# rampasek/GraphGPS

Measured on NVIDIA H100. Metric: graphs/sec GPSLayer fwd+bwd, higher is better.
Workload: dtype f32

## Files before the change

### graphgps_b200/csrc/attention.cu

```cuda
#include "kernels.cuh"

namespace gps {

namespace {

constexpr int kWarpsPerBlock = 4;

__device__ __forceinline__ int find_graph(const int* __restrict__ gptr, int B, int node) {
  int lo = 0, hi = B;
  while (hi - lo > 1) {
    int mid = (lo + hi) >> 1;
    if (gptr[mid] <= node) lo = mid; else hi = mid;
  }
  return lo;
}

template <int LPR>
__device__ __forceinline__ float group_sum(float v) {
#pragma unroll
  for (int o = LPR / 2; o > 0; o >>= 1) v += __shfl_xor_sync(0xffffffffu, v, o);
  return v;
}

__device__ __forceinline__ int warp_max_i(int v) {
// ... 19 lines not shown
  q.thr = (uint32_t)fminf(p * 4294967296.f, 4294967295.f);
  q.keep_scale = 1.f / (1.f - p);
}

template <int CH, int LPR>
__device__ __forceinline__ void load_slice(float4* dst, const float* row, int sub, int nch, bool ok) {
#pragma unroll
  for (int c = 0; c < CH; ++c) {
    int ch = sub + c * LPR;
    dst[c] = (ok && ch < nch) ? ld4(row + ch * 4) : f4zero();
  }
}
template <int CH, int LPR>
__device__ __forceinline__ void store_slice(const float4* src, float* row, int sub, int nch) {
#pragma unroll
  for (int c = 0; c < CH; ++c) {
    int ch = sub + c * LPR;
    if (ch < nch) st4(row + ch * 4, src[c]);
  }
}
template <int CH, int LPR>
__device__ __forceinline__ void store_slice_planes(const float4* src, const Planes& p, int64_t r, int64_t col0, int sub, int nch) {
  if (!p.hi) return;
#pragma unroll
  for (int c = 0; c < CH; ++c) {
    int ch = sub + c * LPR;
    if (ch < nch) planes_store4(p, r, col0 + ch * 4, src[c]);
  }
}
template <int CH>
__device__ __forceinline__ float dot_slice(const float4* a, const float4* b) {
  float s = 0.f;
#pragma unroll
  for (int c = 0; c < CH; ++c) s += a[c].x * b[c].x + a[c].y * b[c].y + a[c].z * b[c].z + a[c].w * b[c].w;
  return s;
}

struct AttnArgs {
  const int* gptr; int B; int N; int H; int hd;
  const float* Q; const float* K; const float* V; int64_t ld;
  float* O; const float* Oc; const float* dO; int64_t ldo;
  float* lse; const float* lsec; float* delta; const float* deltac;
  float* dQ; float* dK; float* dV; int64_t ldg;
  float scale; float p_drop; uint64_t seed, offset;
  const unsigned long long* offset_dev;
  Planes Op, dQp, dKp, dVp;
  int smem_rows;
};
__device__ __forceinline__ uint64_t eff_offset(const AttnArgs& a) {
  return a.offset + ((a.p_drop > 0.f && a.offset_dev) ? *a.offset_dev : 0ull);
}

struct StagedRows {
  const float* x; int64_t ldx;
  const float* y; int64_t ldy;
};
template <int RPB>
__device__ __forceinline__ StagedRows stage_rows(const AttnArgs& a, const float* X, int64_t ldX, const float* Y, int64_t ldY,
                                                 int h, float* sm) {
  const int64_t hoff = (int64_t)h * a.hd;
  StagedRows r{X + hoff, ldX, Y + hoff, ldY};
  const int r0 = blockIdx.x * RPB;
  if (a.smem_rows <= 0 || r0 >= a.N) return r;
  const int last = min(r0 + RPB, a.N) - 1;
  const int kmin = a.gptr[find_graph(a.gptr, a.B, r0)];
  const int R = a.gptr[find_graph(a.gptr, a.B, last) + 1] - kmin;
  if (R > a.smem_rows) return r;
  const int pitch = a.hd + 4, nch = a.hd >> 2;
  float* sx = sm;
  float* sy = sm + (int64_t)a.smem_rows * pitch;
  for (int idx = threadIdx.x; idx < R * nch; idx += blockDim.x) {
    const int row = idx / nch, c = idx - row * nch;
    st4(sx + row * pitch + c * 4, ld4(X + (int64_t)(kmin + row) * ldX + hoff + c * 4));
    st4(sy + row * pitch + c * 4, ld4(Y + (int64_t)(kmin + row) * ldY + hoff + c * 4));
  }
  __syncthreads();
  r.x = sx - (int64_t)kmin * pitch; r.ldx = pitch;
  r.y = sy - (int64_t)kmin * pitch; r.ldy = pitch;
  return r;
}

template <int CH, int LPR>
__global__ void __launch_bounds__(kWarpsPerBlock * 32) k_attn_fwd(AttnArgs a) {
  extern __shared__ float attn_sm[];
  constexpr int RPW = 32 / LPR;
  const int warp = threadIdx.x >> 5, lane = threadIdx.x & 31;
  const int sub = lane % LPR, rloc = lane / LPR;
  const int h = blockIdx.y;
  const int i = (blockIdx.x * kWarpsPerBlock + warp) * RPW + rloc;
  const bool row_ok = i < a.N;
  const int nch = a.hd / 4;
  const uint64_t offs = eff_offset(a);
  int gs = 0, n = 0;
  if (row_ok) {
    int g = find_graph(a.gptr, a.B, i);
    gs = a.gptr[g];
    n = a.gptr[g + 1] - gs;
  }
  const int nloop = warp_max_i(n);
  const int64_t hoff = (int64_t)h * a.hd;
  float4 q[CH], o[CH];
  load_slice<CH, LPR>(q, a.Q + (int64_t)(row_ok ? i : 0) * a.ld + hoff, sub, nch, row_ok);
#pragma unroll
  for (int c = 0; c < CH; ++c) {
    q[c] = f4scale(q[c], a.scale);
    o[c] = f4zero();
  }
  float m = -INFINITY, l = 0.f;
  const bool use_drop = a.p_drop > 0.f;
  DropQuad dq;
  drop_quad_init(dq, a.p_drop);
  const StagedRows kv = stage_rows<RPW * kWarpsPerBlock>(a, a.K, a.ld, a.V, a.ld, h, attn_sm);
  float4 kc[CH], vc[CH];
  load_slice<CH, LPR>(kc, kv.x + (int64_t)gs * kv.ldx, sub, nch, n > 0);
  load_slice<CH, LPR>(vc, kv.y + (int64_t)gs * kv.ldy, sub, nch, n > 0);
  for (int jl = 0; jl < nloop; ++jl) {
    if (use_drop && (jl & 3) == 0) drop_quad_refresh(dq, a.p_drop, a.seed, offs, h, i, jl);
    const bool valid = jl < n;
    const bool nvalid = jl + 1 < n;
    const int jn = gs + (nvalid ? jl + 1 : 0);
    float4 kn[CH], vn[CH];
    load_slice<CH, LPR>(kn, kv.x + (int64_t)jn * kv.ldx, sub, nch, nvalid);
    load_slice<CH, LPR>(vn, kv.y + (int64_t)jn * kv.ldy, sub, nch, nvalid);
    float s = group_sum<LPR>(dot_slice<CH>(q, kc));
    s = valid ? s : -INFINITY;
    const float m_new = fmaxf(m, s);
    const float corr = (m_new == -INFINITY) ? 1.f : __expf(m - m_new);
    const float p = valid ? __expf(s - m_new) : 0.f;
    l = l * corr + p;
    const float pd = use_drop ? p * drop_quad_scale(dq, jl) : p;
#pragma unroll
    for (int c = 0; c < CH; ++c) {
      o[c].x = o[c].x * corr + pd * vc[c].x;
      o[c].y = o[c].y * corr + pd * vc[c].y;
      o[c].z = o[c].z * corr + pd * vc[c].z;
      o[c].w = o[c].w * corr + pd * vc[c].w;
      kc[c] = kn[c];
      vc[c] = vn[c];
    }
    m = m_new;
  }
  if (row_ok) {
    const float inv = 1.f / l;
#pragma unroll
    for (int c = 0; c < CH; ++c) o[c] = f4scale(o[c], inv);
    store_slice<CH, LPR>(o, a.O + (int64_t)i * a.ldo + hoff, sub, nch);
    store_slice_planes<CH, LPR>(o, a.Op, i, hoff, sub, nch);
    if (sub == 0) a.lse[(int64_t)i * a.H + h] = m + __logf(l);
  }
}

__global__ void k_attn_delta(AttnArgs a) {
  const int64_t t = ((int64_t)blockIdx.x * blockDim.x + threadIdx.x) >> 3;
  const int sub = threadIdx.x & 7;
  const bool ok = t < (int64_t)a.N * a.H;
  const int64_t i = ok ? t / a.H : 0;
  const int h = ok ? (int)(t - i * a.H) : 0;
  const float4* go = reinterpret_cast<const float4*>(a.dO + i * a.ldo + (int64_t)h * a.hd);
  const float4* oo = reinterpret_cast<const float4*>(a.Oc + i * a.ldo + (int64_t)h * a.hd);
  float acc = 0.f;
  if (ok)
    for (int c = sub; c < a.hd / 4; c += 8) {
      const float4 x = __ldg(go + c), y = __ldg(oo + c);
      acc += x.x * y.x + x.y * y.y + x.z * y.z + x.w * y.w;
    }
  acc += __shfl_xor_sync(0xffffffffu, acc, 4);
  acc += __shfl_xor_sync(0xffffffffu, acc, 2);
  acc += __shfl_xor_sync(0xffffffffu, acc, 1);
  if (ok && sub == 0) a.delta[t] = acc;
}

template <int CH, int LPR>
__device__ __forceinline__ void attn_bwd_q_body(const AttnArgs& a, float* attn_sm) {
  constexpr int RPW = 32 / LPR;
  const int warp = threadIdx.x >> 5, lane = threadIdx.x & 31;
  const int sub = lane % LPR, rloc = lane / LPR;
  const int h = blockIdx.y;
  const int i = (blockIdx.x * kWarpsPerBlock + warp) * RPW + rloc;
  const bool row_ok = i < a.N;
  const int nch = a.hd / 4;
  const uint64_t offs = eff_offset(a);
  int gs = 0, n = 0;
  if (row_ok) {
    int g = find_graph(a.gptr, a.B, i);
    gs = a.gptr[g];
    n = a.gptr[g + 1] - gs;
  }
  const int nloop = warp_max_i(n);
  const int64_t hoff = (int64_t)h * a.hd;
  const int ir = row_ok ? i : 0;
  float4 q[CH], go[CH], gq[CH];
  load_slice<CH, LPR>(q, a.Q + (int64_t)ir * a.ld + hoff, sub, nch, row_ok);
  load_slice<CH, LPR>(go, a.dO + (int64_t)ir * a.ldo + hoff, sub, nch, row_ok);
  {
    const float dl = row_ok ? a.deltac[(int64_t)i * a.H + h] : 0.f;
#pragma unroll
    for (int c = 0; c < CH; ++c) gq[c] = f4zero();
    const float lse = row_ok ? a.lsec[(int64_t)i * a.H + h] : 0.f;
#pragma unroll
    for (int c = 0; c < CH; ++c) q[c] = f4scale(q[c], a.scale);
    const bool use_drop = a.p_drop > 0.f;
    DropQuad dq;
    drop_quad_init(dq, a.p_drop);
    const StagedRows kv = stage_rows<RPW * kWarpsPerBlock>(a, a.K, a.ld, a.V, a.ld, h, attn_sm);
    float4 kk[CH], vv[CH];
    load_slice<CH, LPR>(kk, kv.x + (int64_t)gs * kv.ldx, sub, nch, n > 0);
    load_slice<CH, LPR>(vv, kv.y + (int64_t)gs * kv.ldy, sub, nch, n > 0);
    for (int jl = 0; jl < nloop; ++jl) {
      if (use_drop && (jl & 3) == 0) drop_quad_refresh(dq, a.p_drop, a.seed, offs, h, i, jl);
      const bool valid = jl < n;
      const bool nvalid = jl + 1 < n;
      const int jn = gs + (nvalid ? jl + 1 : 0);
      float4 kn[CH], vn[CH];
      load_slice<CH, LPR>(kn, kv.x + (int64_t)jn * kv.ldx, sub, nch, nvalid);
      load_slice<CH, LPR>(vn, kv.y + (int64_t)jn * kv.ldy, sub, nch, nvalid);
      float s = dot_slice<CH>(q, kk), dp = dot_slice<CH>(go, vv);
#pragma unroll
      for (int ofs = LPR / 2; ofs > 0; ofs >>= 1) {
        s += __shfl_xor_sync(0xffffffffu, s, ofs);
        dp += __shfl_xor_sync(0xffffffffu, dp, ofs);
      }
      const float p = valid ? __expf(s - lse) : 0.f;
      const float ds = p * (dp * (use_drop ? drop_quad_scale(dq, jl) : 1.f) - dl);
#pragma unroll
      for (int c = 0; c < CH; ++c) {
        gq[c].x += ds * kk[c].x;
        gq[c].y += ds * kk[c].y;
        gq[c].z += ds * kk[c].z;
        gq[c].w += ds * kk[c].w;
        kk[c] = kn[c];
        vv[c] = vn[c];
      }
    }
  }
  if (row_ok) {
#pragma unroll
    for (int c = 0; c < CH; ++c) gq[c] = f4scale(gq[c], a.scale);
    store_slice<CH, LPR>(gq, a.dQ + (int64_t)i * a.ldg + hoff, sub, nch);
    store_slice_planes<CH, LPR>(gq, a.dQp, i, hoff, sub, nch);
  }
}

template <int CH, int LPR>
__device__ __forceinline__ void attn_bwd_kv_body(const AttnArgs& a, float* attn_sm) {
  constexpr int RPW = 32 / LPR;
  const int warp = threadIdx.x >> 5, lane = threadIdx.x & 31;
  const int sub = lane % LPR, rloc = lane / LPR;
  const int h = blockIdx.y;
  const int j = (blockIdx.x * kWarpsPerBlock + warp) * RPW + rloc;
  const bool row_ok = j < a.N;
  const int nch = a.hd / 4;
  const uint64_t offs = eff_offset(a);
  int gs = 0, n = 0;
  if (row_ok) {
    int g = find_graph(a.gptr, a.B, j);
    gs = a.gptr[g];
    n = a.gptr[g + 1] - gs;
  }
  const int nloop = warp_max_i(n);
  const int jl = j - gs;
  const int64_t hoff = (int64_t)h * a.hd;
  const int jr = row_ok ? j : 0;
  float4 kk[CH], vv[CH], gk[CH], gv[CH];
  load_slice<CH, LPR>(kk, a.K + (int64_t)jr * a.ld + hoff, sub, nch, row_ok);
  load_slice<CH, LPR>(vv, a.V + (int64_t)jr * a.ld + hoff, sub, nch, row_ok);
#pragma unroll
  for (int c = 0; c < CH; ++c) {
    gk[c] = f4zero();
    gv[c] = f4zero();
  }
  const StagedRows qd = stage_rows<RPW * kWarpsPerBlock>(a, a.Q, a.ld, a.dO, a.ldo, h, attn_sm);
  float4 q[CH], go[CH];
  load_slice<CH, LPR>(q, qd.x + (int64_t)gs * qd.ldx, sub, nch, n > 0);
  load_slice<CH, LPR>(go, qd.y + (int64_t)gs * qd.ldy, sub, nch, n > 0);
  for (int il = 0; il < nloop; ++il) {
    const bool valid = il < n;
    const int i = gs + (valid ? il : 0);
    const bool nvalid = il + 1 < n;
    const int in_ = gs + (nvalid ? il + 1 : 0);
    float4 qn[CH], gon[CH];
    load_slice<CH, LPR>(qn, qd.x + (int64_t)in_ * qd.ldx, sub, nch, nvalid);
    load_slice<CH, LPR>(gon, qd.y + (int64_t)in_ * qd.ldy, sub, nch, nvalid);
    float s = dot_slice<CH>(q, kk), dp = dot_slice<CH>(go, vv);
#pragma unroll
    for (int ofs = LPR / 2; ofs > 0; ofs >>= 1) {
      s += __shfl_xor_sync(0xffffffffu, s, ofs);
      dp += __shfl_xor_sync(0xffffffffu, dp, ofs);
    }
    const float lse = valid ? a.lsec[(int64_t)i * a.H + h] : 0.f;
    const float dl = valid ? a.deltac[(int64_t)i * a.H + h] : 0.f;
    const float p = valid ? __expf(s * a.scale - lse) : 0.f;
    float dsc = 1.f;
    if (a.p_drop > 0.f) {
      DropQuad dq;
      drop_quad_init(dq, a.p_drop);
      drop_quad_refresh(dq, a.p_drop, a.seed, offs, h, i, jl);
      dsc = drop_quad_scale(dq, jl);
    }
    const float pd = p * dsc;
    const float ds = p * (dp * dsc - dl) * a.scale;
#pragma unroll
    for (int c = 0; c < CH; ++c) {
      gk[c].x += ds * q[c].x; gk[c].y += ds * q[c].y; gk[c].z += ds * q[c].z; gk[c].w += ds * q[c].w;
      gv[c].x += pd * go[c].x; gv[c].y += pd * go[c].y; gv[c].z += pd * go[c].z; gv[c].w += pd * go[c].w;
      q[c] = qn[c];
      go[c] = gon[c];
    }
  }
  if (row_ok) {
    store_slice<CH, LPR>(gk, a.dK + (int64_t)j * a.ldg + hoff, sub, nch);
    store_slice<CH, LPR>(gv, a.dV + (int64_t)j * a.ldg + hoff, sub, nch);
    store_slice_planes<CH, LPR>(gk, a.dKp, j, hoff, sub, nch);
    store_slice_planes<CH, LPR>(gv, a.dVp, j, hoff, sub, nch);
  }
}

template <int CH, int LPR>
__global__ void __launch_bounds__(kWarpsPerBlock * 32) k_attn_bwd(AttnArgs a) {
  extern __shared__ float attn_sm[];
  if (blockIdx.z == 0) attn_bwd_kv_body<CH, LPR>(a, attn_sm);
  else attn_bwd_q_body<CH, LPR>(a, attn_sm);
}

enum { KFWD = 0, KBWD = 1 };

constexpr int kStageBytes = 72 * 1024;

template <int CH, int LPR>
static void launch_one(int which, const AttnArgs& a0, cudaStream_t stream) {
  constexpr int RPW = 32 / LPR;
  AttnArgs a = a0;
  static const bool stage_on = [] {
    const char* e = getenv("GPS_B200_ATTN_STAGE");
    return e && e[0] == '1';
  }();
  const int pitch = a.hd + 4;
  a.smem_rows = (stage_on && a.B > 0 && a.N < 64LL * a.B) ? kStageBytes / (2 * pitch * 4) : 0;
  const size_t smem = a.smem_rows > 0 ? (size_t)2 * a.smem_rows * pitch * 4 : 0;
  static bool attr_done[2] = {false, false};
  if (smem > 0 && !attr_done[which]) {
    if (which == KFWD) cudaFuncSetAttribute(k_attn_fwd<CH, LPR>, cudaFuncAttributeMaxDynamicSharedMemorySize, kStageBytes);
    else cudaFuncSetAttribute(k_attn_bwd<CH, LPR>, cudaFuncAttributeMaxDynamicSharedMemorySize, kStageBytes);
    attr_done[which] = true;
  }
  dim3 grid((unsigned)ceil_div(a.N, (int64_t)RPW * kWarpsPerBlock), (unsigned)a.H, which == KFWD ? 1 : 2);
  dim3 block(kWarpsPerBlock * 32);
  if (which == KFWD) k_attn_fwd<CH, LPR><<<grid, block, smem, stream>>>(a);
  else k_attn_bwd<CH, LPR><<<grid, block, smem, stream>>>(a);
}

static int dispatch(int which, const AttnArgs& a, cudaStream_t stream) {
  GPS_REQUIRE(a.hd > 0 && a.hd % 4 == 0, GPS_ERR_UNSUPPORTED, "attention: head dim %d must be a multiple of 4", a.hd);
  GPS_REQUIRE(a.ld % 4 == 0 && a.ldo % 4 == 0 && (which == KFWD || a.ldg % 4 == 0), GPS_ERR_UNSUPPORTED,
              "attention: leading dimensions must be multiples of 4");
  const int nch = a.hd / 4;
  GPS_REQUIRE(nch <= 48, GPS_ERR_UNSUPPORTED, "attention: head dim %d > 192 not supported", a.hd);
  if (a.N == 0) return GPS_OK;
  int lpr = 1;
  while ((nch + lpr - 1) / lpr > 6) lpr *= 2;
  const int ch = (nch + lpr - 1) / lpr;
#define GPS_ATTN_CASE(CHV, LPRV)                                  \
  if (ch == CHV && lpr == LPRV) {                                 \
    launch_one<CHV, LPRV>(which, a, stream);                      \
    GPS_LAUNCH_CHECK();                                           \
    return GPS_OK;                                                \
  }
  GPS_ATTN_CASE(1, 1) GPS_ATTN_CASE(2, 1) GPS_ATTN_CASE(3, 1) GPS_ATTN_CASE(4, 1) GPS_ATTN_CASE(5, 1)
  GPS_ATTN_CASE(6, 1) GPS_ATTN_CASE(4, 2) GPS_ATTN_CASE(5, 2) GPS_ATTN_CASE(6, 2) GPS_ATTN_CASE(4, 4)
  GPS_ATTN_CASE(5, 4) GPS_ATTN_CASE(6, 4) GPS_ATTN_CASE(4, 8) GPS_ATTN_CASE(5, 8) GPS_ATTN_CASE(6, 8)
#undef GPS_ATTN_CASE
  set_error("attention: no kernel for head dim %d", a.hd);
  return GPS_ERR_UNSUPPORTED;
}

}

int attention_fwd(const GpsGraph& g, int64_t heads, int64_t hd, const float* Q, const float* K, const float* V,
                  int64_t ld, float* O, int64_t ldo, float* lse, float p_drop, uint64_t seed, uint64_t offset,
                  cudaStream_t stream, const unsigned long long* offset_dev, Planes Op) {
  AttnArgs a{};
  a.offset_dev = offset_dev;
  a.Op = Op;
  a.gptr = g.graph_ptr; a.B = (int)g.B; a.N = (int)g.N; a.H = (int)heads; a.hd = (int)hd;
  a.Q = Q; a.K = K; a.V = V; a.ld = ld; a.O = O; a.ldo = ldo; a.lse = lse;
  a.scale = 1.f / sqrtf((float)hd); a.p_drop = p_drop; a.seed = seed; a.offset = offset;
  return dispatch(KFWD, a, stream);
}

int attention_bwd(const GpsGraph& g, int64_t heads, int64_t hd, const float* Q, const float* K, const float* V,
                  int64_t ld, const float* O, const float* dO, int64_t ldo, const float* lse, float* delta,
                  float* dQ, float* dK, float* dV, int64_t ldg, float p_drop, uint64_t seed, uint64_t offset,
                  cudaStream_t stream, const unsigned long long* offset_dev, Planes dQp, Planes dKp, Planes dVp) {
  AttnArgs a{};
  a.offset_dev = offset_dev;
  a.dQp = dQp; a.dKp = dKp; a.dVp = dVp;
  a.gptr = g.graph_ptr; a.B = (int)g.B; a.N = (int)g.N; a.H = (int)heads; a.hd = (int)hd;
  a.Q = Q; a.K = K; a.V = V; a.ld = ld; a.Oc = O; a.dO = dO; a.ldo = ldo; a.lsec = lse;
  a.delta = delta; a.deltac = delta; a.dQ = dQ; a.dK = dK; a.dV = dV; a.ldg = ldg;
  a.scale = 1.f / sqrtf((float)hd); a.p_drop = p_drop; a.seed = seed; a.offset = offset;
  if (a.N == 0) return GPS_OK;
  const int64_t nt = (int64_t)a.N * a.H * 8;
  k_attn_delta<<<(unsigned)ceil_div(nt, (int64_t)256), 256, 0, stream>>>(a);
  GPS_LAUNCH_CHECK();
  return dispatch(KBWD, a, stream);
}

}
```

### graphgps_b200/csrc/attention_tc.cu

```cuda
#include <cuda.h>
#include <cuda_bf16.h>

#include "gemm.cuh"
#include "kernels.cuh"
#include "tc_ptx.cuh"

namespace gps {

namespace {

using namespace tc;

constexpr int kTile = 128;
constexpr int kSoftWarps = 8;
constexpr int kThreadsA = 256;

struct AttnTcArgs {
  const int* gptr; int B; int N; int H; int hd; int hd_pad; int planes;
  float* O; int64_t ldo; Planes Op; float* lse;
  float scale; float p_drop; uint64_t seed, offset;
  const unsigned long long* offset_dev;
  float* dbg;
};

__device__ __forceinline__ int find_graph_tc(const int* __restrict__ gptr, int B, int node) {
  int lo = 0, hi = B;
  while (hi - lo > 1) {
    int mid = (lo + hi) >> 1;
    if (gptr[mid] <= node) lo = mid; else hi = mid;
  }
  return lo;
}

__device__ __forceinline__ uint32_t pack_bf16x2(float a, float b) {
  __nv_bfloat162 h = __floats2bfloat162_rn(a, b);
  return *reinterpret_cast<uint32_t*>(&h);
}

struct RowState {
  int i, gs, ge;
  float m, l;
  int rq_quad;
  Philox4 rq;
};

template <int NKB, bool SPLIT>
__global__ void __launch_bounds__(kThreadsA, 1)
k_attn_tc_fwd(const __grid_constant__ CUtensorMap tmQK, const __grid_constant__ CUtensorMap tmV, const AttnTcArgs a) {
  extern __shared__ __align__(1024) uint8_t smem_raw[];
  uint8_t* smem = reinterpret_cast<uint8_t*>((reinterpret_cast<uintptr_t>(smem_raw) + 1023) & ~(uintptr_t)1023);
  constexpr int planes = SPLIT ? 2 : 1;
  constexpr int q_bytes = NKB * 16384, k_bytes = NKB * 16384, v_bytes = 2 * NKB * 8192;
  uint8_t* sQ = smem;
  uint8_t* sK = sQ + planes * q_bytes;
  uint8_t* sV = sK + planes * k_bytes;
  uint64_t* bars = reinterpret_cast<uint64_t*>(sV + planes * v_bytes);
  int* range = reinterpret_cast<int*>(bars + 8);

  const int tid = threadIdx.x, warp = tid >> 5, lane = tid & 31;
  const int q0 = blockIdx.x * kTile, h = blockIdx.y;
  const uint32_t b_q = smem_u32(&bars[0]), b_kf = smem_u32(&bars[1]), b_vf = smem_u32(&bars[2]),
                 b_ke = smem_u32(&bars[3]), b_ve = smem_u32(&bars[4]);

  if (tid == 0) {
    mbar_init(b_q, 1); mbar_init(b_kf, 1); mbar_init(b_vf, 1); mbar_init(b_ke, kSoftWarps); mbar_init(b_ve, kSoftWarps);
    fence_barrier_init();
    const int last = min(q0 + kTile, a.N) - 1;
    const int g0 = find_graph_tc(a.gptr, a.B, q0), g1 = find_graph_tc(a.gptr, a.B, last);
    range[0] = a.gptr[g0];
    range[1] = a.gptr[g1 + 1];
  }
  __syncthreads();
  const int kmin = range[0], kmax = range[1];
  const int ntiles = max(1, (kmax - kmin + kTile - 1) / kTile);

  auto load_k = [&](int t) {
    if (t > 0) mbar_wait(b_ke, (uint32_t)(t - 1) & 1u);
    mbar_arrive_expect_tx(b_kf, (uint32_t)(planes * k_bytes));
    for (int pl = 0; pl < planes; ++pl)
      for (int kb = 0; kb < NKB; ++kb)
        tma_tile_3d(smem_u32(sK + pl * k_bytes + kb * 16384), &tmQK, (a.H + h) * a.hd_pad + 64 * kb, kmin + t * kTile, pl,
                    b_kf);
  };
  auto load_v = [&](int t) {
    if (t > 0) mbar_wait(b_ve, (uint32_t)(t - 1) & 1u);
    mbar_arrive_expect_tx(b_vf, (uint32_t)(planes * v_bytes));
    for (int pl = 0; pl < planes; ++pl)
      for (int kk = 0; kk < 2; ++kk)
        for (int nb = 0; nb < NKB; ++nb)
          tma_tile_3d(smem_u32(sV + pl * v_bytes + (kk * NKB + nb) * 8192), &tmV, (2 * a.H + h) * a.hd_pad + 64 * nb,
                      kmin + t * kTile + 64 * kk, pl, b_vf);
  };
  if (tid == 0) {
    tma_prefetch_desc(&tmQK);
    tma_prefetch_desc(&tmV);
    mbar_arrive_expect_tx(b_q, (uint32_t)(planes * q_bytes));
    for (int pl = 0; pl < planes; ++pl)
      for (int kb = 0; kb < NKB; ++kb)
        tma_tile_3d(smem_u32(sQ + pl * q_bytes + kb * 16384), &tmQK, h * a.hd_pad + 64 * kb, q0, pl, b_q);
    load_k(0);
    load_v(0);
  }

  const int wg = warp >> 2;
  const int rloc = wg * 64 + (warp & 3) * 16 + (lane >> 2);
  const int cq = 2 * (lane & 3);
  RowState rs[2];
#pragma unroll
  for (int u = 0; u < 2; ++u) {
    RowState& R = rs[u];
    R.i = q0 + rloc + 8 * u;
    R.gs = 0; R.ge = 0;
    if (R.i < a.N) {
      const int g = find_graph_tc(a.gptr, a.B, R.i);
      R.gs = a.gptr[g];
      R.ge = a.gptr[g + 1];
    }
    R.m = -INFINITY; R.l = 0.f; R.rq_quad = -1;
  }
  const uint64_t offs = a.offset + ((a.p_drop > 0.f && a.offset_dev) ? *a.offset_dev : 0ull);
  const bool use_drop = a.p_drop > 0.f;
  const uint32_t drop_thr = (uint32_t)fminf(a.p_drop * 4294967296.f, 4294967295.f);
  const float keep_scale = use_drop ? 1.f / (1.f - a.p_drop) : 1.f;
  const bool dump = a.dbg && blockIdx.x == 0 && blockIdx.y == 0;

  float o[NKB * 32];
#pragma unroll
  for (int e = 0; e < NKB * 32; ++e) o[e] = 0.f;
  const uint32_t aQ = smem_u32(sQ) + (uint32_t)wg * 8192u, aK = smem_u32(sK), aV = smem_u32(sV);
  const int qk_steps = a.hd_pad >> 4;
  if (lane == 0) mbar_wait(b_q, 0u);
  __syncwarp();
  for (int t = 0; t < ntiles; ++t) {
    const int key0 = kmin + t * kTile;
    float sacc[64];
#pragma unroll
    for (int e = 0; e < 64; ++e) sacc[e] = 0.f;
    if (lane == 0) mbar_wait(b_kf, (uint32_t)t & 1u);
    __syncwarp();
    wgmma_fence();
#pragma unroll
    for (int ks = 0; ks < NKB * 4; ++ks) {
      if (ks < qk_steps) {
        const uint32_t off = (ks >> 2) * 16384 + (ks & 3) * 32;
        const uint64_t dq_hi = make_desc(aQ + off, 16, 1024);
        const uint64_t dk_hi = make_desc(aK + off, 16, 1024);
        if (SPLIT) {
          const uint64_t dq_lo = make_desc(aQ + q_bytes + off, 16, 1024);
          const uint64_t dk_lo = make_desc(aK + k_bytes + off, 16, 1024);
// ... 53 lines not shown
                R.rq = philox4x32(a.seed, offs + (uint64_t)(GPS_SITE_ATTN_P + h), ((uint64_t)R.i << 20) | (uint64_t)R.rq_quad);
              }
              const int k4 = jl & 3;
              const uint32_t bits = k4 == 0 ? R.rq.v[0] : k4 == 1 ? R.rq.v[1] : k4 == 2 ? R.rq.v[2] : R.rq.v[3];
              pr = bits >= drop_thr ? pr * keep_scale : 0.f;
            }
          }
          v = pr;
          if (dump && t == 0) {
            const int r = rloc + 8 * u, c = 8 * j + cq + e;
            a.dbg[r * 128 + c] = sraw;
            a.dbg[16384 + r * 128 + c] = pr;
          }
        }
    }
    uint32_t ph[32], pl[SPLIT ? 32 : 1];
#pragma unroll
    for (int x = 0; x < 32; ++x) {
      const float p0 = sacc[2 * x], p1 = sacc[2 * x + 1];
      __nv_bfloat162 hb = __floats2bfloat162_rn(p0, p1);
      ph[x] = *reinterpret_cast<uint32_t*>(&hb);
      if (SPLIT) pl[x] = pack_bf16x2(p0 - __low2float(hb), p1 - __high2float(hb));
    }
    if (lane == 0) mbar_wait(b_vf, (uint32_t)t & 1u);
    __syncwarp();
    wgmma_fence();
#pragma unroll
    for (int ks = 0; ks < 8; ++ks) {
      const uint32_t voff = ((ks >> 2) * NKB) * 8192 + (ks & 3) * 2048;
      const uint64_t dv_hi = make_desc(aV + voff, 8192, 1024);
      if (SPLIT) {
        const uint64_t dv_lo = make_desc(aV + v_bytes + voff, 8192, 1024);
        wgmma_rs<NKB * 64, 1>(o, pl + 4 * ks, dv_hi, 1u);
        wgmma_rs<NKB * 64, 1>(o, ph + 4 * ks, dv_lo, 1u);
      }
      wgmma_rs<NKB * 64, 1>(o, ph + 4 * ks, dv_hi, 1u);
    }
    wgmma_commit();
    wgmma_wait<0>();
    reg_fence<NKB * 32>(o);
    __syncwarp();
    if (lane == 0) mbar_arrive(b_ve);
    if (tid == 0 && t + 1 < ntiles) load_v(t + 1);
  }
#pragma unroll
  for (int u = 0; u < 2; ++u) {
    RowState& R = rs[u];
    R.l += __shfl_xor_sync(0xffffffffu, R.l, 1);
    R.l += __shfl_xor_sync(0xffffffffu, R.l, 2);
    const float inv = R.l > 0.f ? 1.f / R.l : 0.f;
    const bool row_ok = R.i < a.N;
#pragma unroll
    for (int j = 0; j < NKB * 8; ++j) {
      const int col = 8 * j + cq;
      const float v0 = o[4 * j + 2 * u], v1 = o[4 * j + 2 * u + 1];
      if (dump) {
        a.dbg[32768 + (rloc + 8 * u) * 128 + col] = v0;
        a.dbg[32768 + (rloc + 8 * u) * 128 + col + 1] = v1;
      }
      if (!row_ok || col >= a.hd) continue;
      const float w0 = v0 * inv, w1 = v1 * inv;
      float* dst = a.O + (int64_t)R.i * a.ldo + (int64_t)h * a.hd + col;
      dst[0] = w0;
      dst[1] = w1;
      if (a.Op.hi) {
        const int64_t off = (int64_t)R.i * a.Op.ld + (int64_t)h * a.hd + col;
        __nv_bfloat162 hb = __floats2bfloat162_rn(w0, w1);
        *reinterpret_cast<__nv_bfloat162*>(a.Op.hi + off) = hb;
        if (a.Op.lo) *reinterpret_cast<uint32_t*>(a.Op.lo + off) = pack_bf16x2(w0 - __low2float(hb), w1 - __high2float(hb));
      }
    }
    if (row_ok && (lane & 3) == 0) a.lse[(int64_t)R.i * a.H + h] = R.m + __logf(R.l);
  }
}

template <int NKB, bool SPLIT>
int launch_attn(const CUtensorMap& tQK, const CUtensorMap& tV, const AttnTcArgs& a, dim3 grid, size_t smem,
                cudaStream_t stream) {
  static bool attr_done = false;
  if (!attr_done) {
    GPS_CUDA(cudaFuncSetAttribute(k_attn_tc_fwd<NKB, SPLIT>, cudaFuncAttributeMaxDynamicSharedMemorySize, 227 * 1024));
    attr_done = true;
  }
  k_attn_tc_fwd<NKB, SPLIT><<<grid, kThreadsA, smem, stream>>>(tQK, tV, a);
  GPS_LAUNCH_CHECK();
  return GPS_OK;
}

float* g_attn_dbg = nullptr;
}

void attention_tc_set_debug(float* buf) { g_attn_dbg = buf; }
bool attention_tc_supported(int64_t hd) { return hd > 0 && hd % 4 == 0 && hd <= 128; }
int64_t attention_tc_hd_pad(int64_t hd) { return round_up(hd, 16); }

int attention_tc_fwd(const GpsGraph& g, int64_t heads, int64_t hd, Planes qkv, float* O, int64_t ldo, Planes Op, float* lse,
                     float p_drop, uint64_t seed, uint64_t offset, const unsigned long long* offset_dev, int precision,
                     cudaStream_t stream) {
  if (g.N == 0) return GPS_OK;
  GPS_REQUIRE(attention_tc_supported(hd) && qkv.hi && (precision != GPS_PREC_FP32 || qkv.lo) && qkv.ld % 8 == 0, GPS_ERR_UNSUPPORTED,
              "attention_tc: head dim %lld / planes not supported", (long long)hd);
  AttnTcArgs a{};
  a.gptr = g.graph_ptr; a.B = (int)g.B; a.N = (int)g.N; a.H = (int)heads; a.hd = (int)hd;
  a.hd_pad = (int)attention_tc_hd_pad(hd);
  a.planes = precision == GPS_PREC_FP32 ? 2 : 1;
  a.O = O; a.ldo = ldo; a.Op = Op; a.lse = lse;
  a.scale = 1.f / sqrtf((float)hd); a.p_drop = p_drop; a.seed = seed; a.offset = offset; a.offset_dev = offset_dev;
  a.dbg = g_attn_dbg;
  const int64_t cols = 3 * heads * a.hd_pad;
  CUtensorMap tQK, tV;
  GPS_TRY(make_tensor_map(qkv.hi, qkv.lo, a.planes, g.N, cols, qkv.ld, 128, &tQK));
  GPS_TRY(make_tensor_map(qkv.hi, qkv.lo, a.planes, g.N, cols, qkv.ld, 64, &tV));
  const int nkb = (a.hd_pad + 63) >> 6;
  const size_t smem = (size_t)a.planes * nkb * (16384 + 16384 + 16384) + 1024 + 256;
  dim3 grid((unsigned)ceil_div(g.N, kTile), (unsigned)heads);
  if (nkb == 1) return a.planes == 2 ? launch_attn<1, true>(tQK, tV, a, grid, smem, stream)
                                     : launch_attn<1, false>(tQK, tV, a, grid, smem, stream);
  return a.planes == 2 ? launch_attn<2, true>(tQK, tV, a, grid, smem, stream)
                       : launch_attn<2, false>(tQK, tV, a, grid, smem, stream);
}

}
```

### graphgps_b200/csrc/common.cuh

```cuda
#pragma once

#include <cuda_bf16.h>
#include <cuda_runtime.h>
#include <stdint.h>
#include <stdio.h>
#include <string>

#include "../../include/gps_b200.h"

namespace gps {

void set_error(const char* fmt, ...);
int cuda_fail(cudaError_t e, const char* what, const char* file, int line);
void count_launch();

#define GPS_CUDA(expr)                                                             \
  do {                                                                             \
    cudaError_t _e = (expr);                                                       \
    if (_e != cudaSuccess) return ::gps::cuda_fail(_e, #expr, __FILE__, __LINE__); \
  } while (0)

#define GPS_LAUNCH_CHECK()            \
  do {                                \
    ::gps::count_launch();            \
    GPS_CUDA(cudaGetLastError());     \
  } while (0)

#define GPS_REQUIRE(cond, code, ...)   \
  do {                                 \
    if (!(cond)) {                     \
      ::gps::set_error(__VA_ARGS__);   \
      return (code);                   \
    }                                  \
  } while (0)

#define GPS_TRY(expr)            \
  do {                           \
    int _rc = (expr);            \
    if (_rc != GPS_OK) return _rc; \
  } while (0)

constexpr int kNumSMs = 132;
constexpr float kBnEps = 1e-5f;
constexpr float kBnMomentum = 0.1f;

static inline int64_t round_up(int64_t v, int64_t a) { return (v + a - 1) / a * a; }
static inline int64_t ceil_div(int64_t a, int64_t b) { return (a + b - 1) / b; }

struct Arena {
  char* base;
  int64_t cap;
  int64_t used = 0;
  bool overflow = false;
  Arena(void* b, int64_t c) : base(reinterpret_cast<char*>(b)), cap(c) {}
  template <typename T>
  T* alloc(int64_t n) {
    int64_t bytes = round_up(n * (int64_t)sizeof(T), 256);
    int64_t off = used;
    used += bytes;
    if (base == nullptr) return nullptr;
    if (used > cap) {
      overflow = true;
      return nullptr;
    }
    return reinterpret_cast<T*>(base + off);
  }
};

struct Planes {
  __nv_bfloat16* hi = nullptr;
  __nv_bfloat16* lo = nullptr;
  int64_t ld = 0;
  Planes cols(int64_t c0) const { Planes q = *this; if (q.hi) q.hi += c0; if (q.lo) q.lo += c0; return q; }
  Planes rows(int64_t r0) const { Planes q = *this; if (q.hi) q.hi += r0 * ld; if (q.lo) q.lo += r0 * ld; return q; }
};

#ifdef __CUDACC__

__device__ __forceinline__ void planes_store4(const Planes& p, int64_t r, int64_t c, float4 v) {
  __nv_bfloat162 h0 = __floats2bfloat162_rn(v.x, v.y), h1 = __floats2bfloat162_rn(v.z, v.w);
  uint2 hw = make_uint2(*reinterpret_cast<uint32_t*>(&h0), *reinterpret_cast<uint32_t*>(&h1));
  *reinterpret_cast<uint2*>(p.hi + r * p.ld + c) = hw;
  if (p.lo) {
    __nv_bfloat162 l0 = __floats2bfloat162_rn(v.x - __low2float(h0), v.y - __high2float(h0));
    __nv_bfloat162 l1 = __floats2bfloat162_rn(v.z - __low2float(h1), v.w - __high2float(h1));
    *reinterpret_cast<uint2*>(p.lo + r * p.ld + c) = make_uint2(*reinterpret_cast<uint32_t*>(&l0), *reinterpret_cast<uint32_t*>(&l1));
  }
}

__device__ __forceinline__ float4 ld4(const float* p) { return *reinterpret_cast<const float4*>(p); }
__device__ __forceinline__ void st4(float* p, float4 v) { *reinterpret_cast<float4*>(p) = v; }
__device__ __forceinline__ float4 f4zero() { return make_float4(0.f, 0.f, 0.f, 0.f); }
__device__ __forceinline__ float4 f4add(float4 a, float4 b) {
  return make_float4(a.x + b.x, a.y + b.y, a.z + b.z, a.w + b.w);
}
__device__ __forceinline__ float4 f4mul(float4 a, float4 b) {
  return make_float4(a.x * b.x, a.y * b.y, a.z * b.z, a.w * b.w);
}
__device__ __forceinline__ float4 f4fma(float4 a, float4 b, float4 c) {
  return make_float4(fmaf(a.x, b.x, c.x), fmaf(a.y, b.y, c.y), fmaf(a.z, b.z, c.z), fmaf(a.w, b.w, c.w));
}
__device__ __forceinline__ float4 f4scale(float4 a, float s) {
  return make_float4(a.x * s, a.y * s, a.z * s, a.w * s);
}

__device__ __forceinline__ float sigmoidf_(float v) { return 1.f / (1.f + __expf(-v)); }

template <int ACT>
__device__ __forceinline__ float act_fwd(float v) {
  if (ACT == GPS_ACT_RELU) return v > 0.f ? v : 0.f;
  return 0.5f * v * (1.f + erff(v * 0.70710678118654752f));
}
template <int ACT>
__device__ __forceinline__ float act_bwd(float v) {
  if (ACT == GPS_ACT_RELU) return v > 0.f ? 1.f : 0.f;
  float cdf = 0.5f * (1.f + erff(v * 0.70710678118654752f));
  float pdf = 0.3989422804014327f * __expf(-0.5f * v * v);
  return cdf + v * pdf;
}
__device__ __forceinline__ float act_fwd_rt(int act, float v) {
  return act == GPS_ACT_RELU ? act_fwd<GPS_ACT_RELU>(v) : act_fwd<GPS_ACT_GELU>(v);
}
__device__ __forceinline__ float act_bwd_rt(int act, float v) {
  return act == GPS_ACT_RELU ? act_bwd<GPS_ACT_RELU>(v) : act_bwd<GPS_ACT_GELU>(v);
}

struct Philox4 {
  uint32_t v[4];
};
__device__ __forceinline__ Philox4 philox4x32(uint64_t seed, uint64_t ctr_hi, uint64_t ctr_lo) {
  const uint32_t M0 = 0xD2511F53u, M1 = 0xCD9E8D57u, W0 = 0x9E3779B9u, W1 = 0xBB67AE85u;
  uint32_t c0 = (uint32_t)ctr_lo, c1 = (uint32_t)(ctr_lo >> 32), c2 = (uint32_t)ctr_hi,
           c3 = (uint32_t)(ctr_hi >> 32);
  uint32_t k0 = (uint32_t)seed, k1 = (uint32_t)(seed >> 32);
#pragma unroll
  for (int r = 0; r < 10; ++r) {
    uint32_t hi0 = __umulhi(M0, c0), lo0 = M0 * c0;
    uint32_t hi1 = __umulhi(M1, c2), lo1 = M1 * c2;
    uint32_t n0 = hi1 ^ c1 ^ k0, n1 = lo1, n2 = hi0 ^ c3 ^ k1, n3 = lo0;
    c0 = n0; c1 = n1; c2 = n2; c3 = n3;
    k0 += W0; k1 += W1;
  }
  Philox4 o;
  o.v[0] = c0; o.v[1] = c1; o.v[2] = c2; o.v[3] = c3;
  return o;
}
__device__ __forceinline__ float4 dropout_scale4(float p, uint64_t seed, uint64_t offset, int site,
                                                 uint64_t idx4) {
  Philox4 r = philox4x32(seed, offset + (uint64_t)site, idx4);
  uint32_t thr = (uint32_t)fminf(p * 4294967296.f, 4294967295.f);
  float s = 1.f / (1.f - p);
  return make_float4(r.v[0] >= thr ? s : 0.f, r.v[1] >= thr ? s : 0.f, r.v[2] >= thr ? s : 0.f,
                     r.v[3] >= thr ? s : 0.f);
}

enum {
  GPS_SITE_GCN_X = 1, GPS_SITE_GCN_E = 2, GPS_SITE_LOCAL = 3, GPS_SITE_ATTN_OUT = 4,
  GPS_SITE_FF1 = 5, GPS_SITE_FF2 = 6, GPS_SITE_PERF_OUT = 7, GPS_SITE_ATTN_P = 16
};

__device__ __forceinline__ float warp_sum(float v) {
// ... 11 lines not shown
```

### graphgps_b200/csrc/elementwise.cu

```cuda
#include <cooperative_groups.h>

#include "kernels.cuh"

namespace gps {

namespace {

struct RowGeom {
  dim3 block, grid;
  size_t smem;
};

static int row_geom(int64_t rows, int64_t d, int nstat, RowGeom* g) {
  GPS_REQUIRE(d > 0 && d % 4 == 0 && d / 4 <= 1024, GPS_ERR_UNSUPPORTED,
              "row-wise stage needs d %% 4 == 0 and d <= 4096 (got %lld)", (long long)d);
  int C4 = (int)(d / 4);
  int RY = C4 >= 256 ? 1 : 256 / C4;
  int64_t cap = kNumSMs * 8;
  if (nstat > 0) {
    RY = C4 >= 1024 ? 1 : 1024 / C4;
    if (RY > 16) RY = 16;
    const int smem_cap = (int)(48 * 1024 / ((size_t)nstat * C4 * sizeof(float4)));
    if (RY > smem_cap) RY = smem_cap < 1 ? 1 : smem_cap;
    cap = kNumSMs / 2;
  }
  int64_t blocks = ceil_div(rows > 0 ? rows : 1, (int64_t)RY * 4);
  if (blocks > cap) blocks = cap;
  g->block = dim3(C4, RY, 1);
  g->grid = dim3((unsigned)blocks, 1, 1);
  g->smem = RY > 1 ? (size_t)nstat * RY * C4 * sizeof(float4) : 0;
  return GPS_OK;
}

template <class Op>
__device__ __forceinline__ void rowwise_body(Op& op, int64_t rows, int vb, int vgrid, float4* sm) {
  const int c4 = threadIdx.x, ry = threadIdx.y, RY = blockDim.y, C4 = blockDim.x;
  constexpr int NS = Op::NS;
  float4 acc[NS > 0 ? NS : 1];
#pragma unroll
  for (int s = 0; s < (NS > 0 ? NS : 1); ++s) acc[s] = f4zero();
  op.prepare(c4);
#pragma unroll 4
  for (int64_t r = (int64_t)vb * RY + ry; r < rows; r += (int64_t)vgrid * RY) op.row(r, c4, acc);
  if (NS > 0) {
    if (RY > 1) {
#pragma unroll
      for (int s = 0; s < NS; ++s) sm[(s * RY + ry) * C4 + c4] = acc[s];
      __syncthreads();
      if (ry == 0) {
#pragma unroll
        for (int s = 0; s < NS; ++s)
          for (int y = 1; y < RY; ++y) acc[s] = f4add(acc[s], sm[(s * RY + y) * C4 + c4]);
      }
    }
    if (ry == 0) {
#pragma unroll
      for (int s = 0; s < NS; ++s) {
        double* p = op.stat_ptr(s);
        if (p) {
          atomic_add_f64(p + c4 * 4 + 0, (double)acc[s].x);
          atomic_add_f64(p + c4 * 4 + 1, (double)acc[s].y);
          atomic_add_f64(p + c4 * 4 + 2, (double)acc[s].z);
          atomic_add_f64(p + c4 * 4 + 3, (double)acc[s].w);
        }
      }
    }
  }
  op.finish(c4, ry);
}

template <class Op>
__global__ void __launch_bounds__(1024) k_rowwise(Op op, int64_t rows) {
  extern __shared__ float4 sm[];
  rowwise_body(op, rows, (int)blockIdx.x, (int)gridDim.x, sm);
}

template <class OpA, class OpB>
__global__ void __launch_bounds__(1024) k_rowwise2(OpA a, int64_t rowsA, int ga, OpB b, int64_t rowsB) {
  extern __shared__ float4 sm[];
  if ((int)blockIdx.x < ga) {
    a.vb = (int)blockIdx.x;
    rowwise_body(a, rowsA, (int)blockIdx.x, ga, sm);
  } else {
    b.vb = (int)blockIdx.x - ga;
    rowwise_body(b, rowsB, (int)blockIdx.x - ga, (int)gridDim.x - ga, sm);
  }
}

struct BnRegs {
  float4 mean, invstd, gamma, beta;
  __device__ void load(const BnView& v, int c4, int vb = -1) {
    gamma = ld4(v.gamma + c4 * 4);
    beta = ld4(v.beta + c4 * 4);
    if (v.mode == 0) {
      mean = ld4(v.mean + c4 * 4);
      invstd = ld4(v.invstd + c4 * 4);
    } else if (v.mode == 2) {
      mean = ld4(v.running_mean + c4 * 4);
      const float4 rv = ld4(v.running_var + c4 * 4);
      invstd = make_float4(rsqrtf(rv.x + kBnEps), rsqrtf(rv.y + kBnEps), rsqrtf(rv.z + kBnEps), rsqrtf(rv.w + kBnEps));
    } else {
      float m[4], is[4], var[4];
#pragma unroll
      for (int j = 0; j < 4; ++j) {
        const double mu = v.sums[c4 * 4 + j] * v.inv_n;
        double vv = v.sums[v.d + c4 * 4 + j] * v.inv_n - mu * mu;
        if (vv < 0.0) vv = 0.0;
        m[j] = (float)mu;
        var[j] = (float)(vv * v.unbias);
        is[j] = (float)(1.0 / sqrt(vv + (double)kBnEps));
      }
      mean = make_float4(m[0], m[1], m[2], m[3]);
      invstd = make_float4(is[0], is[1], is[2], is[3]);
      if ((vb < 0 ? (int)blockIdx.x : vb) == 0 && threadIdx.y == 0) {
        st4(v.save_mean + c4 * 4, mean);
        st4(v.save_invstd + c4 * 4, invstd);
        if (v.running_mean) {
          const float4 rm = ld4(v.running_mean + c4 * 4);
          st4(v.running_mean + c4 * 4, make_float4((1.f - kBnMomentum) * rm.x + kBnMomentum * m[0],
                                                   (1.f - kBnMomentum) * rm.y + kBnMomentum * m[1],
                                                   (1.f - kBnMomentum) * rm.z + kBnMomentum * m[2],
                                                   (1.f - kBnMomentum) * rm.w + kBnMomentum * m[3]));
        }
        if (v.running_var) {
          const float4 rv = ld4(v.running_var + c4 * 4);
          st4(v.running_var + c4 * 4, make_float4((1.f - kBnMomentum) * rv.x + kBnMomentum * var[0],
                                                  (1.f - kBnMomentum) * rv.y + kBnMomentum * var[1],
                                                  (1.f - kBnMomentum) * rv.z + kBnMomentum * var[2],
                                                  (1.f - kBnMomentum) * rv.w + kBnMomentum * var[3]));
        }
        if (c4 == 0 && v.nbt) *v.nbt += 1;
      }
    }
  }
  __device__ float4 zhat(float4 z) const {
    return make_float4((z.x - mean.x) * invstd.x, (z.y - mean.y) * invstd.y, (z.z - mean.z) * invstd.z,
                       (z.w - mean.w) * invstd.w);
  }
  __device__ float4 apply(float4 z) const { return f4fma(zhat(z), gamma, beta); }
};

__device__ __forceinline__ float4 act4(int act, float4 v) {
  if (act < 0) return v;
  return make_float4(act_fwd_rt(act, v.x), act_fwd_rt(act, v.y), act_fwd_rt(act, v.z), act_fwd_rt(act, v.w));
}
__device__ __forceinline__ float4 dact4(int act, float4 v) {
  return make_float4(act_bwd_rt(act, v.x), act_bwd_rt(act, v.y), act_bwd_rt(act, v.z), act_bwd_rt(act, v.w));
}

template <bool STATS>
struct OpBnActRes {
  static constexpr int NS = STATS ? 2 : 0;
  const float* z; int64_t ldz;
  const float* R; float* out; int64_t d;
  BnView bn; int act; DropCfg drop; double* stats; Planes outp;
  BnRegs reg;
  int vb = -1;
  __device__ void prepare(int c4) {
    reg.load(bn, c4, vb);
    if (drop.p > 0.f && drop.offset_dev) drop.offset += *drop.offset_dev;
  }
// ... 64 lines not shown
  static constexpr int NS = 0;
  const float* g; int64_t ldg; const float* z; int64_t ldz; int64_t d;
  BnView bn; int act; DropCfg drop; const double* sums; float inv_n;
  float* out; int64_t ldo; float* grad_gamma; float* grad_beta; int accumulate; Planes outp;
  BnRegs reg;
  float4 m1, m2, gs;
  float4 s1raw, s2raw;
  __device__ void prepare(int c4) {
    reg.load(bn, c4);
    if (drop.p > 0.f && drop.offset_dev) drop.offset += *drop.offset_dev;
    const double* a = sums + c4 * 4;
    const double* b = sums + d + c4 * 4;
    s1raw = make_float4((float)a[0], (float)a[1], (float)a[2], (float)a[3]);
    s2raw = make_float4((float)b[0], (float)b[1], (float)b[2], (float)b[3]);
    m1 = f4scale(s1raw, inv_n);
    m2 = f4scale(s2raw, inv_n);
    if (bn.mode == 2) m1 = m2 = f4zero();
    gs = f4mul(reg.gamma, reg.invstd);
  }
  __device__ void row(int64_t r, int c4, float4*) {
    float4 zh = reg.zhat(ld4(z + r * ldz + c4 * 4));
    float4 gp = bn_bwd_gprime(g, ldg, r, c4, zh, reg, act, drop, d);
    float4 v = make_float4(gs.x * (gp.x - m1.x - zh.x * m2.x), gs.y * (gp.y - m1.y - zh.y * m2.y),
                           gs.z * (gp.z - m1.z - zh.z * m2.z), gs.w * (gp.w - m1.w - zh.w * m2.w));
    st4(out + r * ldo + c4 * 4, v);
    if (outp.hi) planes_store4(outp, r, c4 * 4, v);
  }
  __device__ double* stat_ptr(int) { return nullptr; }
  __device__ void finish(int c4, int ry) {
    if (blockIdx.x == 0 && ry == 0) {
      if (grad_gamma) st4(grad_gamma + c4 * 4, accumulate ? f4add(ld4(grad_gamma + c4 * 4), s2raw) : s2raw);
      if (grad_beta) st4(grad_beta + c4 * 4, accumulate ? f4add(ld4(grad_beta + c4 * 4), s1raw) : s1raw);
    }
  }
};

struct OpBnBwdApplyChain {
  static constexpr int NS = 2;
  OpBnBwdApply a;
  const float* z2; int64_t ldz2; BnView bn2; int act2; DropCfg drop2; double* sums2;
  BnRegs reg2;
  __device__ void prepare(int c4) {
    a.prepare(c4);
    reg2.load(bn2, c4);
    if (drop2.p > 0.f && drop2.offset_dev) drop2.offset += *drop2.offset_dev;
  }
  __device__ void row(int64_t r, int c4, float4* acc) {
    float4 zh = a.reg.zhat(ld4(a.z + r * a.ldz + c4 * 4));
    float4 gp = bn_bwd_gprime(a.g, a.ldg, r, c4, zh, a.reg, a.act, a.drop, a.d);
    float4 v = make_float4(a.gs.x * (gp.x - a.m1.x - zh.x * a.m2.x), a.gs.y * (gp.y - a.m1.y - zh.y * a.m2.y),
                           a.gs.z * (gp.z - a.m1.z - zh.z * a.m2.z), a.gs.w * (gp.w - a.m1.w - zh.w * a.m2.w));
    st4(a.out + r * a.ldo + c4 * 4, v);
    if (a.outp.hi) planes_store4(a.outp, r, c4 * 4, v);
    float4 zh2 = reg2.zhat(ld4(z2 + r * ldz2 + c4 * 4));
    float4 g2 = v;
    if (drop2.p > 0.f)
      g2 = f4mul(g2, dropout_scale4(drop2.p, drop2.seed, drop2.offset, drop2.site, (uint64_t)r * (a.d >> 2) + c4));
    if (act2 >= 0) g2 = f4mul(g2, dact4(act2, f4fma(zh2, reg2.gamma, reg2.beta)));
    acc[0] = f4add(acc[0], g2);
    acc[1] = f4fma(g2, zh2, acc[1]);
  }
  __device__ double* stat_ptr(int s) { return sums2 + (int64_t)s * a.d; }
  __device__ void finish(int c4, int ry) { a.finish(c4, ry); }
};

struct OpAdd3 {
  static constexpr int NS = 0;
  const float* a; int64_t lda; const float* b; int64_t ldb; const float* c; int64_t ldc;
  float* out; int64_t ldo;
  __device__ void prepare(int) {}
  __device__ void row(int64_t r, int c4, float4*) {
    float4 v = ld4(a + r * lda + c4 * 4);
    if (b) v = f4add(v, ld4(b + r * ldb + c4 * 4));
    if (c) v = f4add(v, ld4(c + r * ldc + c4 * 4));
    st4(out + r * ldo + c4 * 4, v);
  }
  __device__ double* stat_ptr(int) { return nullptr; }
  __device__ void finish(int, int) {}
};

constexpr int kColsumCtas = 8;
__global__ void __launch_bounds__(1024) k_colsum(const float* __restrict__ a, int64_t lda, int64_t rows, int C4,
                                                 float* __restrict__ out) {
  extern __shared__ float4 sm[];
  const int ry = threadIdx.y, RY = blockDim.y, CB = blockDim.x;
  const int c4 = blockIdx.x * CB + threadIdx.x;
  const bool col_ok = c4 < C4;
  float4 acc = f4zero();
  if (col_ok)
    for (int64_t r = (int64_t)blockIdx.y * RY + ry; r < rows; r += (int64_t)gridDim.y * RY)
      acc = f4add(acc, ld4(a + r * lda + c4 * 4));
  if (RY > 1) {
    sm[ry * CB + threadIdx.x] = acc;
    __syncthreads();
    if (ry == 0)
      for (int y = 1; y < RY; ++y) acc = f4add(acc, sm[y * CB + threadIdx.x]);
  }
  if (ry == 0) sm[threadIdx.x] = acc;
  cooperative_groups::cluster_group cluster = cooperative_groups::this_cluster();
  cluster.sync();
  if (blockIdx.y == 0 && ry == 0 && col_ok) {
    float4 tot = f4zero();
    for (int k = 0; k < (int)gridDim.y; ++k) tot = f4add(tot, cluster.map_shared_rank(sm, k)[threadIdx.x]);
    atomicAdd(out + c4 * 4 + 0, tot.x);
    atomicAdd(out + c4 * 4 + 1, tot.y);
    atomicAdd(out + c4 * 4 + 2, tot.z);
    atomicAdd(out + c4 * 4 + 3, tot.w);
  }
  cluster.sync();
}

template <class Op>
static int launch_rowwise(Op op, int64_t rows, int64_t d, cudaStream_t stream) {
  if (rows == 0) return GPS_OK;
  RowGeom g;
  GPS_TRY(row_geom(rows, d, Op::NS, &g));
  k_rowwise<Op><<<g.grid, g.block, g.smem, stream>>>(op, rows);
  GPS_LAUNCH_CHECK();
  return GPS_OK;
}

}

int bn_act_residual(const float* z, int64_t ldz, const float* R, float* out, int64_t rows, int64_t d, BnView bn,
                    int act, DropCfg drop, double* stats, cudaStream_t stream, Planes outp) {
  if (stats) {
    OpBnActRes<true> op{z, ldz, R, out, d, bn, act, drop, stats, outp};
    return launch_rowwise(op, rows, d, stream);
  }
  OpBnActRes<false> op{z, ldz, R, out, d, bn, act, drop, nullptr, outp};
  return launch_rowwise(op, rows, d, stream);
}

int bn_act_residual2(const float* zx, const float* Rx, float* outx, int64_t N, BnView bnx, DropCfg dropx, double* statsx,
                     const float* ze, const float* Re, float* oute, int64_t E, BnView bne, DropCfg drope, Planes outep,
                     int64_t d, int act, cudaStream_t stream) {
  if (N == 0 || E == 0 || !statsx) {
    GPS_TRY(bn_act_residual(zx, d, Rx, outx, N, d, bnx, act, dropx, statsx, stream));
    return bn_act_residual(ze, d, Re, oute, E, d, bne, act, drope, nullptr, stream, outep);
  }
  RowGeom g;
  GPS_TRY(row_geom(N, d, 2, &g));
  const int RY = (int)g.block.y;
  int64_t gb = ceil_div(E, (int64_t)RY * 4);
  if (gb > kNumSMs * 2) gb = kNumSMs * 2;
  OpBnActRes<true> opx{zx, d, Rx, outx, d, bnx, act, dropx, statsx, Planes()};
  OpBnActRes<false> ope{ze, d, Re, oute, d, bne, act, drope, nullptr, outep};
  k_rowwise2<<<dim3((unsigned)(g.grid.x + gb)), g.block, g.smem, stream>>>(opx, N, (int)g.grid.x, ope, E);
  GPS_LAUNCH_CHECK();
  return GPS_OK;
}

int bn_bwd_apply_chain(const float* g, int64_t ldg, const float* z, int64_t ldz, int64_t rows, int64_t d, BnView bn,
                       const double* sums, float* out, int64_t ldo, float* grad_gamma, float* grad_beta, bool accumulate,
                       Planes outp, const float* z2, int64_t ldz2, BnView bn2, int act2, DropCfg drop2, double* sums2,
                       cudaStream_t stream) {
  GPS_REQUIRE(rows > 0, GPS_ERR_ARG, "bn_bwd_apply_chain: no rows");
  OpBnBwdApply a{g, ldg, z, ldz, d, bn, -1, DropCfg(), sums, 1.f / (float)rows, out, ldo, grad_gamma, grad_beta,
                 accumulate ? 1 : 0, outp};
  OpBnBwdApplyChain op{a, z2, ldz2, bn2, act2, drop2, sums2};
  return launch_rowwise(op, rows, d, stream);
}

int bn_combine(const float* a, BnView bna, const float* b, BnView bnb, float* out, int64_t rows, int64_t d,
               cudaStream_t stream, Planes outp) {
  OpCombine op{a, b, out, d, bna, bnb, outp};
  return launch_rowwise(op, rows, d, stream);
}

int bn_bwd_reduce(const float* g, int64_t ldg, const float* z, int64_t ldz, int64_t rows, int64_t d, BnView bn,
                  int act, DropCfg drop, double* sums, cudaStream_t stream) {
  OpBnBwdReduce op{g, ldg, z, ldz, d, bn, act, drop, sums};
  return launch_rowwise(op, rows, d, stream);
}

int bn_bwd_apply(const float* g, int64_t ldg, const float* z, int64_t ldz, int64_t rows, int64_t d, BnView bn,
                 int act, DropCfg drop, const double* sums, float* out, int64_t ldo, float* grad_gamma,
                 float* grad_beta, cudaStream_t stream, bool accumulate, Planes outp) {
  OpBnBwdApply op{g, ldg, z, ldz, d, bn, act, drop, sums, 1.f / (float)(rows > 0 ? rows : 1),
                  out, ldo, grad_gamma, grad_beta, accumulate ? 1 : 0, outp};
  if (rows == 0) {
    if (grad_gamma && !accumulate) GPS_CUDA(cudaMemsetAsync(grad_gamma, 0, d * sizeof(float), stream));
    if (grad_beta && !accumulate) GPS_CUDA(cudaMemsetAsync(grad_beta, 0, d * sizeof(float), stream));
    return GPS_OK;
  }
  return launch_rowwise(op, rows, d, stream);
}

int add3(const float* a, int64_t lda, const float* b, int64_t ldb, const float* c, int64_t ldc, float* out,
         int64_t ldo, int64_t rows, int64_t d, cudaStream_t stream) {
  OpAdd3 op{a, lda, b, ldb, c, ldc, out, ldo};
  return launch_rowwise(op, rows, d, stream);
}

int colsum(const float* a, int64_t lda, int64_t rows, int64_t d, float* out, cudaStream_t stream) {
  if (rows == 0) return GPS_OK;
  GPS_REQUIRE(d > 0 && d % 4 == 0, GPS_ERR_UNSUPPORTED, "colsum needs d %% 4 == 0 (got %lld)", (long long)d);
  const int C4 = (int)(d / 4);
  const int CB = C4 < 128 ? C4 : 128;
  const int RY = 1024 / CB < 16 ? 1024 / CB : 16;
  cudaLaunchConfig_t cfg = {};
  cfg.gridDim = dim3((unsigned)ceil_div(C4, CB), kColsumCtas);
  cfg.blockDim = dim3(CB, RY);
  cfg.dynamicSmemBytes = (size_t)RY * CB * sizeof(float4);
  cfg.stream = stream;
  cudaLaunchAttribute attr[1];
  attr[0].id = cudaLaunchAttributeClusterDimension;
  attr[0].val.clusterDim.x = 1;
  attr[0].val.clusterDim.y = kColsumCtas;
  attr[0].val.clusterDim.z = 1;
  cfg.attrs = attr;
  cfg.numAttrs = 1;
  GPS_CUDA(cudaLaunchKernelEx(&cfg, k_colsum, a, lda, rows, C4, out));
  GPS_LAUNCH_CHECK();
  return GPS_OK;
}

int copy2d(const float* src, int64_t lds, float* dst, int64_t ldd, int64_t rows, int64_t d, cudaStream_t stream) {
  if (rows == 0) return GPS_OK;
  GPS_CUDA(cudaMemcpy2DAsync(dst, ldd * sizeof(float), src, lds * sizeof(float), d * sizeof(float), rows,
                             cudaMemcpyDeviceToDevice, stream));
  return GPS_OK;
}

}
```

### graphgps_b200/csrc/eslap.cu

```cuda
#include "kernels.cuh"

namespace gps {

namespace {

constexpr int kWarpsPerBlock = 8;

__device__ __forceinline__ float pe_dist2(const float* __restrict__ pe, int64_t k, int64_t a, int64_t b, int lane) {
  float acc = 0.f;
  for (int64_t c = lane; c < k; c += 32) {
    const float t = pe[a * k + c] - pe[b * k + c];
    acc = fmaf(t, t, acc);
  }
  return warp_sum(acc);
}

template <int ACT>
__global__ void k_eslap_fwd(GpsGraph g, const float* __restrict__ pe, int64_t k, int d, const float* __restrict__ w1,
                            const float* __restrict__ b1, const float* __restrict__ w2, const float* __restrict__ b2,
                            float* __restrict__ r_out, float* __restrict__ rho_out) {
  const int lane = threadIdx.x & 31;
  const int64_t i = (int64_t)blockIdx.x * kWarpsPerBlock + (threadIdx.x >> 5);
  if (i >= g.N) return;
  const float bias2 = b2[0];
  for (int q = g.dst_ptr[i]; q < g.dst_ptr[i + 1]; ++q) {
    const int j = g.dst_src[q];
    const int64_t e = g.dst_eid[q];
    const float r = pe_dist2(pe, k, i, j, lane);
    float z = 0.f;
    for (int m = lane; m < d; m += 32) z = fmaf(w2[m], act_fwd<ACT>(fmaf(w1[m], r, b1[m])), z);
    z = warp_sum(z) + bias2;
    if (lane == 0) {
      r_out[e] = r;
      rho_out[e] = sigmoidf_(z);
    }
  }
}

template <int ACT>
__global__ void k_eslap_bwd_edge(GpsGraph g, int d, const float* __restrict__ g_num, const float* __restrict__ g_den,
                                 const float* __restrict__ Bx, int64_t ldy, const float* __restrict__ ehat,
                                 const float* __restrict__ r_in, const float* __restrict__ rho_in,
                                 const float* __restrict__ w1, const float* __restrict__ b1,
                                 const float* __restrict__ w2, float* __restrict__ gz_out, float* __restrict__ gr_out) {
  const int lane = threadIdx.x & 31;
  const int64_t i = (int64_t)blockIdx.x * kWarpsPerBlock + (threadIdx.x >> 5);
  if (i >= g.N) return;
  for (int q = g.dst_ptr[i]; q < g.dst_ptr[i + 1]; ++q) {
    const int64_t j = g.dst_src[q];
    const int64_t e = g.dst_eid[q];
    float acc = 0.f;
    for (int c = lane * 4; c < d; c += 128) {
      const float4 gn = ld4(g_num + i * d + c), gd = ld4(g_den + i * d + c), bx = ld4(Bx + j * ldy + c);
      const float4 eh = ld4(ehat + e * d + c);
      acc = fmaf(fmaf(gn.x, bx.x, gd.x), sigmoidf_(eh.x), acc);
      acc = fmaf(fmaf(gn.y, bx.y, gd.y), sigmoidf_(eh.y), acc);
      acc = fmaf(fmaf(gn.z, bx.z, gd.z), sigmoidf_(eh.z), acc);
      acc = fmaf(fmaf(gn.w, bx.w, gd.w), sigmoidf_(eh.w), acc);
    }
    const float g_rho = warp_sum(acc);
    const float rho = rho_in[e], r = r_in[e];
    const float gz = g_rho * rho * (1.f - rho);
    float s = 0.f;
    for (int m = lane; m < d; m += 32) s = fmaf(w2[m] * act_bwd<ACT>(fmaf(w1[m], r, b1[m])), w1[m], s);
    s = warp_sum(s);
    if (lane == 0) {
      gz_out[e] = gz;
      gr_out[e] = gz * s;
    }
  }
}

__global__ void k_eslap_bwd_pe(GpsGraph g, const float* __restrict__ pe, int64_t k, const float* __restrict__ gr,
                               float* __restrict__ grad_pe) {
  const int lane = threadIdx.x & 31;
  const int64_t n = (int64_t)blockIdx.x * kWarpsPerBlock + (threadIdx.x >> 5);
  if (n >= g.N) return;
  const int db = g.dst_ptr[n], de = g.dst_ptr[n + 1], sb = g.src_ptr[n], se = g.src_ptr[n + 1];
  for (int64_t c = lane; c < k; c += 32) {
    const float p = pe[n * k + c];
    float acc = 0.f;
    for (int q = db; q < de; ++q) acc = fmaf(2.f * gr[g.dst_eid[q]], p - pe[(int64_t)g.dst_src[q] * k + c], acc);
    for (int q = sb; q < se; ++q) acc = fmaf(2.f * gr[g.src_eid[q]], p - pe[(int64_t)g.src_dst[q] * k + c], acc);
    grad_pe[n * k + c] = acc;
  }
}

template <int ACT>
__global__ void k_eslap_wgrad_part(int64_t E, int64_t chunk, int d, const float* __restrict__ r_in,
                                   const float* __restrict__ gz_in, const float* __restrict__ w1,
                                   const float* __restrict__ b1, const float* __restrict__ w2, float* __restrict__ part) {
  const int64_t e0 = (int64_t)blockIdx.x * chunk;
  const int64_t e1 = e0 + chunk < E ? e0 + chunk : E;
  float* out = part + (int64_t)blockIdx.x * (3 * d + 1);
  for (int m = threadIdx.x; m < d; m += blockDim.x) {
    const float a = w1[m], b = b1[m], w = w2[m];
    float gw2 = 0.f, gw1 = 0.f, gb1 = 0.f;
    for (int64_t e = e0; e < e1; ++e) {
      const float r = r_in[e], gz = gz_in[e];
      const float pre = fmaf(a, r, b);
      gw2 = fmaf(gz, act_fwd<ACT>(pre), gw2);
      const float gpre = gz * w * act_bwd<ACT>(pre);
      gw1 = fmaf(gpre, r, gw1);
      gb1 += gpre;
    }
    out[m] = gw2;
    out[d + m] = gw1;
    out[2 * d + m] = gb1;
  }
  if (threadIdx.x == 0) {
    float gb2 = 0.f;
    for (int64_t e = e0; e < e1; ++e) gb2 += gz_in[e];
    out[3 * d] = gb2;
  }
}

__global__ void k_eslap_wgrad_sum(int64_t nparts, int d, const float* __restrict__ part, float* gw2, float* gw1,
                                  float* gb1, float* gb2, int accumulate) {
  const int col = blockIdx.x * blockDim.x + threadIdx.x;
  if (col > 3 * d) return;
  float s = 0.f;
#pragma unroll 8
  for (int64_t b = 0; b < nparts; ++b) s += part[b * (3 * d + 1) + col];
  float* base = col < d ? gw2 : (col < 2 * d ? gw1 : (col < 3 * d ? gb1 : gb2));
  if (!base) return;
  float* dst = base + (col < 3 * d ? col % d : 0);
  *dst = accumulate ? *dst + s : s;
}

}

int64_t eslap_wgrad_chunk(int64_t E) {
  const int64_t c = ceil_div(E, (int64_t)kNumSMs);
  return c > 32 ? c : 32;
}

int eslap_fwd(const GpsGraph& g, const float* pe, int64_t k, int64_t d, int act, const float* w1, const float* b1,
              const float* w2, const float* b2, float* r, float* rho, cudaStream_t stream) {
  if (g.N == 0 || g.E == 0) return GPS_OK;
  const unsigned blocks = (unsigned)ceil_div(g.N, (int64_t)kWarpsPerBlock);
  if (act == GPS_ACT_RELU)
    k_eslap_fwd<GPS_ACT_RELU><<<blocks, 32 * kWarpsPerBlock, 0, stream>>>(g, pe, k, (int)d, w1, b1, w2, b2, r, rho);
  else
    k_eslap_fwd<GPS_ACT_GELU><<<blocks, 32 * kWarpsPerBlock, 0, stream>>>(g, pe, k, (int)d, w1, b1, w2, b2, r, rho);
  GPS_LAUNCH_CHECK();
  return GPS_OK;
}

int eslap_bwd(const GpsGraph& g, const float* pe, int64_t k, int64_t d, int act, const float* g_num, const float* g_den,
              const float* Bx, int64_t ldy, const float* ehat, const float* r, const float* rho, const float* w1,
              const float* b1, const float* w2, float* gz, float* gr, float* part, float* grad_pe, float* gw1,
              float* gb1, float* gw2, float* gb2, bool accumulate, cudaStream_t stream) {
  const unsigned node_blocks = (unsigned)ceil_div(g.N, (int64_t)kWarpsPerBlock);
  const int64_t chunk = eslap_wgrad_chunk(g.E), nparts = ceil_div(g.E, chunk);
  if (g.E > 0) {
    if (act == GPS_ACT_RELU)
      k_eslap_bwd_edge<GPS_ACT_RELU><<<node_blocks, 32 * kWarpsPerBlock, 0, stream>>>(
          g, (int)d, g_num, g_den, Bx, ldy, ehat, r, rho, w1, b1, w2, gz, gr);
    else
      k_eslap_bwd_edge<GPS_ACT_GELU><<<node_blocks, 32 * kWarpsPerBlock, 0, stream>>>(
          g, (int)d, g_num, g_den, Bx, ldy, ehat, r, rho, w1, b1, w2, gz, gr);
    GPS_LAUNCH_CHECK();
    if (act == GPS_ACT_RELU)
      k_eslap_wgrad_part<GPS_ACT_RELU><<<(unsigned)nparts, 256, 0, stream>>>(g.E, chunk, (int)d, r, gz, w1, b1, w2, part);
    else
      k_eslap_wgrad_part<GPS_ACT_GELU><<<(unsigned)nparts, 256, 0, stream>>>(g.E, chunk, (int)d, r, gz, w1, b1, w2, part);
    GPS_LAUNCH_CHECK();
  }
  if (gw1 || gb1 || gw2 || gb2) {
    k_eslap_wgrad_sum<<<(unsigned)ceil_div(3 * d + 1, (int64_t)128), 128, 0, stream>>>(g.E > 0 ? nparts : 0, (int)d, part,
                                                                                     gw2, gw1, gb1, gb2, accumulate ? 1 : 0);
    GPS_LAUNCH_CHECK();
  }
  if (grad_pe && g.N > 0) {
    k_eslap_bwd_pe<<<node_blocks, 32 * kWarpsPerBlock, 0, stream>>>(g, pe, k, gr, grad_pe);
    GPS_LAUNCH_CHECK();
  }
  return GPS_OK;
}

}
```

### graphgps_b200/csrc/gemm_tma.cu

```cuda
#include <cooperative_groups.h>
#include <cuda.h>
#include <cuda_bf16.h>

#include <mutex>
#include <unordered_map>

#include "gemm.cuh"
#include "tc_ptx.cuh"

namespace gps {

namespace {

using namespace tc;
namespace cgrp = cooperative_groups;

constexpr int BM = 128;
constexpr int BK = 64;
constexpr int kEpiWarps = 8;
constexpr int kTmaWarp = 8;
constexpr int kThreads = 288;
constexpr int kATile = BM * BK * 2;
constexpr int kBlock = 64 * BK * 2;
constexpr int kMaxSplits = 8;

struct TmaArgs {
  GemmParams p;
  int BN, nb_blocks, stages, kb_per_split, planes;
  int debug;
  unsigned long long* trace;
};

__device__ __forceinline__ unsigned long long gtimer() {
  unsigned long long t;
  asm volatile("mov.u64 %0, %globaltimer;" : "=l"(t));
  return t;
}
#define GPS_TRACE(slot)                                                                         \
  do {                                                                                          \
    if (a.trace && cta_lin < 256) a.trace[cta_lin * 16 + (slot)] = gtimer();                    \
  } while (0)

template <bool A_MN, bool B_MN, int BN_T, bool SPLIT>
__global__ void __launch_bounds__(kThreads, BN_T == 64 ? 2 : 1)
k_gemm_tma(const __grid_constant__ CUtensorMap tmA, const __grid_constant__ CUtensorMap tmB, const TmaArgs a) {
  extern __shared__ __align__(1024) uint8_t smem_raw[];
  const GemmParams& p = a.p;
  uint8_t* smem = reinterpret_cast<uint8_t*>((reinterpret_cast<uintptr_t>(smem_raw) + 1023) & ~(uintptr_t)1023);
  const int planes = a.planes;
  const int b_tile = B_MN ? a.nb_blocks * kBlock : BN_T * 128;
  const int stage_bytes = planes * (kATile + b_tile);
  const int S = a.stages;
  uint64_t* bars = reinterpret_cast<uint64_t*>(smem + (size_t)S * stage_bytes);
  float* red = reinterpret_cast<float*>(bars + 2 * S + 2);
  float* ctot = red + 16 * 16 * 8;
  const int nsplit = (int)gridDim.z;

  const int tid = threadIdx.x, warp = tid >> 5, lane = tid & 31;
  const int m0 = blockIdx.y * BM, n0 = blockIdx.x * a.BN;
  const int nkb_total = (p.K + BK - 1) / BK;
  const int kb_begin = blockIdx.z * a.kb_per_split;
  const int kb_end = min(nkb_total, kb_begin + a.kb_per_split);
  const int nkb = kb_end - kb_begin;
  const bool do_colsum = A_MN && p.colsum_a != nullptr && blockIdx.x == 0;
  const int cta_lin = (blockIdx.z * gridDim.y + blockIdx.y) * gridDim.x + blockIdx.x;

  if (tid == 0) {
    GPS_TRACE(0);
    if (a.trace && cta_lin < 256) {
      unsigned smid;
      asm volatile("mov.u32 %0, %smid;" : "=r"(smid));
      a.trace[cta_lin * 16 + 8] = smid;
    }
    for (int s = 0; s < S; ++s) {
      mbar_init(smem_u32(&bars[s]), 1);
      mbar_init(smem_u32(&bars[S + s]), kEpiWarps);
    }
    fence_barrier_init();
  }
  if (warp == kTmaWarp && lane == 0) {
    tma_prefetch_desc(&tmA);
    tma_prefetch_desc(&tmB);
  }
  __syncthreads();
  if (tid == 0) GPS_TRACE(1);

  if (warp == kTmaWarp) {
    if (lane == 0 && nkb > 0) {
      int a_blocks = 2, b_blocks = a.nb_blocks;
      if (A_MN) a_blocks = min(2, (p.M - m0 + 63) / 64);
      if (B_MN) b_blocks = min(a.nb_blocks, (p.N - n0 + 63) / 64);
      const uint32_t tx = (uint32_t)planes * ((A_MN ? a_blocks * kBlock : kATile) +
                                              (B_MN ? b_blocks * kBlock : a.BN * 128));
      for (int i = 0; i < nkb; ++i) {
        const int s = i % S;
        if (i >= S) mbar_wait(smem_u32(&bars[S + s]), (uint32_t)((i / S) - 1) & 1u);
        const uint32_t full = smem_u32(&bars[s]);
        mbar_arrive_expect_tx(full, tx);
        const int k0 = (kb_begin + i) * BK;
        const uint32_t sa = smem_u32(smem + (size_t)s * stage_bytes);
        const uint32_t sb = sa + planes * kATile;
        for (int pl = 0; pl < planes; ++pl) {
          if (!A_MN) {
            tma_tile_3d(sa + pl * kATile, &tmA, k0, m0, pl, full);
          } else {
            for (int b = 0; b < a_blocks; ++b) tma_tile_3d(sa + pl * kATile + b * kBlock, &tmA, m0 + 64 * b, k0, pl, full);
          }
          if (!B_MN) {
            tma_tile_3d(sb + pl * b_tile, &tmB, k0, n0, pl, full);
          } else {
            for (int b = 0; b < b_blocks; ++b) tma_tile_3d(sb + pl * b_tile + b * kBlock, &tmB, n0 + 64 * b, k0, pl, full);
          }
        }
        if (i == 0) GPS_TRACE(2);
      }
      GPS_TRACE(9);
    }
    __syncwarp();
    if (nsplit > 1) {
      cgrp::this_cluster().sync();
      cgrp::this_cluster().sync();
    }
  } else {
    const int wg = warp >> 2;
    float acc[BN_T / 2];
#pragma unroll
    for (int e = 0; e < BN_T / 2; ++e) acc[e] = 0.f;
    float csum[8];
#pragma unroll
    for (int e = 0; e < 8; ++e) csum[e] = 0.f;
    const int cm = tid & 15, kq = tid >> 4;
    constexpr uint32_t a_lbo = A_MN ? kBlock : 16, b_lbo = B_MN ? kBlock : 16;
    constexpr uint32_t a_kstep = A_MN ? 2048 : 32, b_kstep = B_MN ? 2048 : 32;
    for (int i = 0; i < nkb; ++i) {
      const int s = i % S;
      if (lane == 0) mbar_wait(smem_u32(&bars[s]), (uint32_t)(i / S) & 1u);
      __syncwarp();
      if (i == 0 && tid == 0) GPS_TRACE(3);
      if (i == nkb - 1 && tid == 0) GPS_TRACE(10);
      const uint8_t* st = smem + (size_t)s * stage_bytes;
      const uint32_t sa_hi = smem_u32(st) + (uint32_t)wg * 8192u;
      const uint32_t sb_hi = smem_u32(st) + planes * kATile;
      const uint32_t sa_lo = sa_hi + kATile;
      const uint32_t sb_lo = sb_hi + b_tile;
      wgmma_fence();
#pragma unroll
      for (int kk = 0; kk < BK / 16; ++kk) {
        const uint64_t da_hi = make_desc(sa_hi + kk * a_kstep, a_lbo, 1024);
        const uint64_t db_hi = make_desc(sb_hi + kk * b_kstep, b_lbo, 1024);
        if (SPLIT) {
          const uint64_t da_lo = make_desc(sa_lo + kk * a_kstep, a_lbo, 1024);
          const uint64_t db_lo = make_desc(sb_lo + kk * b_kstep, b_lbo, 1024);
          wgmma_ss<BN_T, A_MN, B_MN>(acc, da_lo, db_hi, 1u);
          wgmma_ss<BN_T, A_MN, B_MN>(acc, da_hi, db_lo, 1u);
        }
        wgmma_ss<BN_T, A_MN, B_MN>(acc, da_hi, db_hi, 1u);
      }
      wgmma_commit();
      if (do_colsum) {
        const uint32_t blk_off = (uint32_t)(cm >> 3) * kBlock;
        const int cc = cm & 7;
        for (int pl = 0; pl < planes; ++pl) {
#pragma unroll
          for (int rr = 0; rr < 4; ++rr) {
            const int r = kq * 4 + rr;
            const uint4 q = *reinterpret_cast<const uint4*>(st + pl * kATile + blk_off + (r >> 3) * 1024 + (r & 7) * 128 +
                                                            ((cc ^ (r & 7)) << 4));
            const uint32_t w[4] = {q.x, q.y, q.z, q.w};
// ... 248 lines not shown
EncodeTiledFn encode_fn() {
  static EncodeTiledFn fn = [] {
    void* f = nullptr;
    cudaDriverEntryPointQueryResult q;
    if (cudaGetDriverEntryPoint("cuTensorMapEncodeTiled", &f, cudaEnableDefault, &q) != cudaSuccess ||
        q != cudaDriverEntryPointSuccess)
      f = nullptr;
    return reinterpret_cast<EncodeTiledFn>(f);
  }();
  return fn;
}

struct MapKey {
  const void* base; int64_t cols, rows, ld, plane_stride; int planes, box_rows;
  bool operator==(const MapKey& o) const {
    return base == o.base && cols == o.cols && rows == o.rows && ld == o.ld && plane_stride == o.plane_stride &&
           planes == o.planes && box_rows == o.box_rows;
  }
};
struct MapKeyHash {
  size_t operator()(const MapKey& k) const {
    size_t h = reinterpret_cast<size_t>(k.base);
    auto mix = [&](int64_t v) { h ^= (size_t)v + 0x9e3779b97f4a7c15ull + (h << 6) + (h >> 2); };
    mix(k.cols); mix(k.rows); mix(k.ld); mix(k.plane_stride); mix(k.planes); mix(k.box_rows);
    return h;
  }
};

int tensor_map(const __nv_bfloat16* hi, const __nv_bfloat16* lo, int planes, int64_t rows, int64_t cols, int64_t ld,
               int box_rows, CUtensorMap* out) {
  static std::mutex mu;
  static std::unordered_map<MapKey, CUtensorMap, MapKeyHash> cache;
  const int64_t plane_stride = planes == 2 ? (int64_t)(lo - hi) : rows * ld;
  GPS_REQUIRE(planes == 1 || plane_stride > 0, GPS_ERR_ARG, "gemm_tma: the lo plane must follow the hi plane in memory");
  MapKey key{hi, cols, rows, ld, plane_stride, planes, box_rows};
  {
    std::lock_guard<std::mutex> lk(mu);
    auto it = cache.find(key);
    if (it != cache.end()) {
      *out = it->second;
      return GPS_OK;
    }
  }
  EncodeTiledFn enc = encode_fn();
  GPS_REQUIRE(enc, GPS_ERR_UNSUPPORTED, "cuTensorMapEncodeTiled is not available from this driver");
  cuuint64_t dims[3] = {(cuuint64_t)cols, (cuuint64_t)rows, (cuuint64_t)planes};
  cuuint64_t strides[2] = {(cuuint64_t)ld * 2, (cuuint64_t)(plane_stride > 0 ? plane_stride : 8) * 2};
  cuuint32_t box[3] = {64, (cuuint32_t)box_rows, 1};
  cuuint32_t estr[3] = {1, 1, 1};
  CUtensorMap m;
  CUresult r = enc(&m, CU_TENSOR_MAP_DATA_TYPE_BFLOAT16, 3, const_cast<__nv_bfloat16*>(hi), dims, strides, box, estr,
                   CU_TENSOR_MAP_INTERLEAVE_NONE, CU_TENSOR_MAP_SWIZZLE_128B, CU_TENSOR_MAP_L2_PROMOTION_L2_256B,
                   CU_TENSOR_MAP_FLOAT_OOB_FILL_NONE);
  GPS_REQUIRE(r == CUDA_SUCCESS, GPS_ERR_CUDA, "cuTensorMapEncodeTiled failed (%d): rows %lld cols %lld ld %lld box %d",
              (int)r, (long long)rows, (long long)cols, (long long)ld, box_rows);
  {
    std::lock_guard<std::mutex> lk(mu);
    if (cache.size() > 4096) cache.clear();
    cache[key] = m;
  }
  *out = m;
  return GPS_OK;
}

}

int make_tensor_map(const __nv_bfloat16* hi, const __nv_bfloat16* lo, int planes, int64_t rows, int64_t cols, int64_t ld,
                    int box_rows, CUtensorMap* out) {
  return tensor_map(hi, lo, planes, rows, cols, ld, box_rows, out);
}

namespace {

inline bool aligned16(const void* q) { return (reinterpret_cast<uintptr_t>(q) & 15) == 0; }

template <bool A_MN, bool B_MN, int BN_T, bool SPLIT>
int launch1(const CUtensorMap& tA, const CUtensorMap& tB, const TmaArgs& a, dim3 grid, size_t smem, cudaStream_t stream) {
  static bool attr_done = false;
  if (!attr_done) {
    GPS_CUDA(cudaFuncSetAttribute(k_gemm_tma<A_MN, B_MN, BN_T, SPLIT>, cudaFuncAttributeMaxDynamicSharedMemorySize,
                                  227 * 1024));
    attr_done = true;
  }
  if (grid.z == 1) {
    k_gemm_tma<A_MN, B_MN, BN_T, SPLIT><<<grid, kThreads, smem, stream>>>(tA, tB, a);
  } else {
    cudaLaunchConfig_t cfg = {};
    cfg.gridDim = grid;
    cfg.blockDim = dim3(kThreads);
    cfg.dynamicSmemBytes = smem;
    cfg.stream = stream;
    cudaLaunchAttribute attr[1];
    attr[0].id = cudaLaunchAttributeClusterDimension;
    attr[0].val.clusterDim.x = 1;
    attr[0].val.clusterDim.y = 1;
    attr[0].val.clusterDim.z = grid.z;
    cfg.attrs = attr;
    cfg.numAttrs = 1;
    GPS_CUDA(cudaLaunchKernelEx(&cfg, k_gemm_tma<A_MN, B_MN, BN_T, SPLIT>, tA, tB, a));
  }
  GPS_LAUNCH_CHECK();
  return GPS_OK;
}
template <bool A_MN, bool B_MN, int BN_T>
int launch(const CUtensorMap& tA, const CUtensorMap& tB, const TmaArgs& a, dim3 grid, size_t smem, cudaStream_t stream) {
  return a.planes == 2 ? launch1<A_MN, B_MN, BN_T, true>(tA, tB, a, grid, smem, stream)
                       : launch1<A_MN, B_MN, BN_T, false>(tA, tB, a, grid, smem, stream);
}

int g_tma_force_bn = 0;
unsigned long long* g_tma_trace = nullptr;
int g_tma_debug = 0;

}

void gemm_tma_set_force_bn(int bn) { g_tma_force_bn = bn & 0xFFFF; g_tma_debug = bn >> 16; }
void gemm_tma_set_trace(unsigned long long* buf) { g_tma_trace = buf; }

int gemm_tma(const GemmParams& p, cudaStream_t stream) {
  if (p.M <= 0 || p.N <= 0) return GPS_OK;
  if (p.K <= 0 || !p.Ap.hi || !p.Bp.hi) return GPS_ERR_UNSUPPORTED;
  const bool split = p.precision == GPS_PREC_FP32;
  const int planes = split ? 2 : 1;
  if (split && (!p.Ap.lo || !p.Bp.lo)) return GPS_ERR_UNSUPPORTED;
  if (!aligned16(p.Ap.hi) || !aligned16(p.Bp.hi) || p.Ap.ld % 8 || p.Bp.ld % 8 || p.N % 4) return GPS_ERR_UNSUPPORTED;
  if (split && (!aligned16(p.Ap.lo) || !aligned16(p.Bp.lo))) return GPS_ERR_UNSUPPORTED;
  if ((p.C && (!aligned16(p.C) || p.ldc % 4)) || (!p.C && !p.Cp.hi)) return GPS_ERR_UNSUPPORTED;
  if (p.Cp.hi && (p.Cp.ld % 4 || (reinterpret_cast<uintptr_t>(p.Cp.hi) & 7) || (p.Cp.lo && (reinterpret_cast<uintptr_t>(p.Cp.lo) & 7))))
    return GPS_ERR_UNSUPPORTED;
  if ((p.bias && !aligned16(p.bias)) || (p.R1 && (!aligned16(p.R1) || p.ldr1 % 4)) ||
      (p.R2 && (!aligned16(p.R2) || p.ldr2 % 4)) || (p.mask_src && (!aligned16(p.mask_src) || p.ldmask % 4)) ||
      (p.C_pre && (!aligned16(p.C_pre) || p.ldpre % 4)))
    return GPS_ERR_UNSUPPORTED;
  if (p.splitk > 1 && (p.bias || p.act >= 0 || p.mask_src || p.stats || p.C_pre || p.p_drop != 0.f || p.p_drop2 != 0.f ||
                       p.Cp.hi || !p.C)) {
    set_error("gemm: split-K supports the plain fp32 product (+ residuals) only");
    return GPS_ERR_ARG;
  }
  if (p.colsum_a && !p.ta) {
    set_error("gemm: colsum_a needs ta == 1");
    return GPS_ERR_ARG;
  }
  if ((p.bnred[0].sums || p.bnred[1].sums) &&
      (p.splitk > 1 || p.C_pre || (p.mask_src && !p.mask_is_post) || p.p_drop != 0.f || p.p_drop2 != 0.f ||
       (p.act >= 0 && p.act != GPS_ACT_RELU))) {
    set_error("gemm: fused BatchNorm-backward reductions need the plain epilogue (no split-K / dropout / GELU)");
    return GPS_ERR_ARG;
  }
  const int mt = (int)ceil_div(p.M, BM);
  const int nkb = (int)ceil_div(p.K, BK);
  const int splits_hint = p.splitk > 1 ? min(kMaxSplits, min(p.splitk, nkb)) : 1;
  const auto width_ok = [&](int bn) {
    return bn == 64 || bn == 128 || (bn == 152 && !p.tb) || (bn == 256 && !p.ta);
  };
  int bestBN = 0;
  long bestCost = 0;
  for (const int bn : {64, 128, 152, 256}) {
    if (!width_ok(bn)) continue;
    const long tiles = (long)mt * ceil_div(p.N, bn) * splits_hint;
    const long cost = bn != 64 ? ceil_div(tiles, (long)kNumSMs) * bn : tiles <= kNumSMs ? 64 : ceil_div(tiles, 2L * kNumSMs) * 160;
    if (!bestBN || cost <= bestCost) { bestCost = cost; bestBN = bn; }
  }
  if (g_tma_force_bn) {
    if (!width_ok(g_tma_force_bn)) return GPS_ERR_UNSUPPORTED;
    bestBN = g_tma_force_bn;
  }
  TmaArgs a;
  a.p = p;
  a.BN = bestBN;
  a.nb_blocks = a.BN / 64;
  a.planes = planes;
  const bool narrow = a.nb_blocks == 1;
  const int stage_bytes = planes * (kATile + (p.tb ? a.nb_blocks * kBlock : a.BN * 128));
  const int fixed = 1024  + 1024  + 16 * 16 * 8 * 4 + 128 * 4;
  int stages = ((narrow ? 112 : 226) * 1024 - fixed) / stage_bytes;
  if (stages > 8) stages = 8;
  if (stages < 2) return GPS_ERR_UNSUPPORTED;
  GPS_REQUIRE((size_t)stages * stage_bytes >= (size_t)BM * (a.BN + 4) * 4, GPS_ERR_ARG,
              "gemm_tma: BN %d: the staging tile does not fit the operand stages", a.BN);
  a.stages = stages;
  int splitk = p.splitk > 1 ? p.splitk : 1;
  if (splitk > kMaxSplits) splitk = kMaxSplits;
  if (splitk > nkb) splitk = nkb;
  a.kb_per_split = (int)ceil_div(nkb, splitk);
  splitk = (int)ceil_div(nkb, a.kb_per_split);
  a.p.splitk = p.splitk > 1 ? 2 : 1;
  a.trace = g_tma_trace;
  a.debug = g_tma_debug;
  const bool amn = p.ta != 0, bmn = p.tb != 0;
  CUtensorMap tA, tB;
  GPS_TRY(tensor_map(p.Ap.hi, p.Ap.lo, planes, amn ? p.K : p.M, amn ? p.M : p.K, p.Ap.ld, amn ? 64 : BM, &tA));
  GPS_TRY(tensor_map(p.Bp.hi, p.Bp.lo, planes, bmn ? p.K : p.N, bmn ? p.N : p.K, p.Bp.ld, bmn ? 64 : a.BN, &tB));
  const size_t smem = (size_t)stages * stage_bytes + fixed;
  dim3 grid((unsigned)ceil_div(p.N, a.BN), (unsigned)mt, (unsigned)splitk);
#define GPS_TMA_CASE(AM, BMN)                                                                              \
  if (amn == AM && bmn == BMN) {                                                                           \
    if (a.BN == 64) return launch<AM, BMN, 64>(tA, tB, a, grid, smem, stream);                            \
    if (a.BN == 128) return launch<AM, BMN, 128>(tA, tB, a, grid, smem, stream);                          \
  }
  GPS_TMA_CASE(false, false)
  GPS_TMA_CASE(false, true)
  GPS_TMA_CASE(true, false)
  GPS_TMA_CASE(true, true)
#undef GPS_TMA_CASE
  if (a.BN == 152 && !bmn)
    return amn ? launch<true, false, 152>(tA, tB, a, grid, smem, stream) : launch<false, false, 152>(tA, tB, a, grid, smem, stream);
  if (a.BN == 256 && !amn)
    return bmn ? launch<false, true, 256>(tA, tB, a, grid, smem, stream) : launch<false, false, 256>(tA, tB, a, grid, smem, stream);
  return GPS_ERR_UNSUPPORTED;
}

namespace {
struct ToPlanesDesc {
  ToPlanesItem it[16];
  int start[17];
  int n;
};
__global__ void k_to_planes(ToPlanesDesc d) {
  int item = 0;
  while (item + 1 < d.n && (int)blockIdx.x >= d.start[item + 1]) ++item;
  const ToPlanesItem& it = d.it[item];
  const int cpr = (it.cols + 7) >> 3;
  const int64_t total = (int64_t)it.rows * cpr;
  const int64_t idx = ((int64_t)blockIdx.x - d.start[item]) * blockDim.x + threadIdx.x;
  if (idx >= total) return;
  const int64_t r = idx / cpr;
  const int c = (int)(idx - r * cpr) * 8;
  const float* src = it.src + r * it.ld + c;
  float v[8];
  if (c + 8 <= it.cols) {
    const float4 x = ld4(src), y = ld4(src + 4);
    v[0] = x.x; v[1] = x.y; v[2] = x.z; v[3] = x.w; v[4] = y.x; v[5] = y.y; v[6] = y.z; v[7] = y.w;
  } else {
#pragma unroll
    for (int i = 0; i < 8; ++i) v[i] = c + i < it.cols ? src[i] : 0.f;
  }
  uint4 hi, lo;
  tc::split8(v, hi, lo);
  *reinterpret_cast<uint4*>(it.dst.hi + r * it.dst.ld + c) = hi;
  if (it.dst.lo) *reinterpret_cast<uint4*>(it.dst.lo + r * it.dst.ld + c) = lo;
}
}

int to_planes(const ToPlanesItem* items, int n, cudaStream_t stream) {
  if (n <= 0) return GPS_OK;
  GPS_REQUIRE(n <= 16, GPS_ERR_ARG, "to_planes: at most 16 matrices per call");
  ToPlanesDesc d;
  d.n = 0;
  int total = 0;
  for (int i = 0; i < n; ++i) {
    const ToPlanesItem& it = items[i];
    if (it.rows <= 0 || it.cols <= 0) continue;
    GPS_REQUIRE(it.src && it.dst.hi && it.ld % 4 == 0 && it.dst.ld % 8 == 0 && it.dst.ld >= round_up(it.cols, 8) &&
                    (reinterpret_cast<uintptr_t>(it.src) & 15) == 0 && (reinterpret_cast<uintptr_t>(it.dst.hi) & 15) == 0 &&
                    (!it.dst.lo || (reinterpret_cast<uintptr_t>(it.dst.lo) & 15) == 0),
                GPS_ERR_ARG, "to_planes: operands must be 16-byte aligned, ld %% 4 == 0, plane ld %% 8 == 0");
    d.it[d.n] = it;
    d.start[d.n] = total;
    total += (int)ceil_div((int64_t)it.rows * ((it.cols + 7) >> 3), 256);
    ++d.n;
  }
  d.start[d.n] = total;
  if (total == 0) return GPS_OK;
  k_to_planes<<<(unsigned)total, 256, 0, stream>>>(d);
  GPS_LAUNCH_CHECK();
  return GPS_OK;
}

}
```

### graphgps_b200/csrc/layer.cu

```cuda
#include <stdarg.h>
#include <string.h>

#include <algorithm>
#include <atomic>

#include "gemm.cuh"
#include "kernels.cuh"

namespace gps {

int perf_supported(int64_t dim_head, int64_t features);
int64_t perf_mp();
int perf_prep(const float* P, int64_t m, float* Pn, const GpsGraph& g, int64_t H, int* nmax, float* gmax, int* argk,
              cudaStream_t st);
int perf_features_fwd(float* fq, float* fk, const float* Q, const float* K, const GpsGraph& g, int64_t H, int64_t m,
                      float* gmax, int* argq, int* argk, cudaStream_t st);
int perf_linattn_fwd(const GpsGraph& g, int64_t H, int64_t m, const int* nmax, const float* qf, const float* kf,
                     const float* V, const float* gmax, float* O, cudaStream_t st);
int perf_linattn_bwd(const GpsGraph& g, int64_t H, int64_t m, const int* nmax, const float* qf, const float* kf,
                     const float* V, const float* gmax, const float* gO, float* g_qf, float* g_kf, float* gV,
                     float* ggmax, cudaStream_t st);
int perf_features_bwd(float* g_fq, float* g_fk, const float* fq, const float* fk, const float* Q, const float* K,
                      float* gQ, float* gK, const GpsGraph& g, int64_t H, int64_t m, const int* argq, const int* argk,
                      float* ggmax, cudaStream_t st);
// ... 30 lines not shown
    int rc = gemm_tma(p, stream);
    if (rc != GPS_ERR_UNSUPPORTED) return rc;
  }
  GPS_REQUIRE(p.A && p.B && p.C, GPS_ERR_UNSUPPORTED, "gemm: plane operands rejected and no fp32 operands to fall back to");
  GPS_REQUIRE(!p.bnred[0].sums && !p.bnred[1].sums, GPS_ERR_UNSUPPORTED,
              "gemm: fused BatchNorm-backward reductions exist in the TMA kernel only");
  GemmParams q = p;
  if (q.Cp.hi) {
    q.Cp = Planes();
  }
  int rc = gemm_tc(q, stream);
  if (rc == GPS_ERR_UNSUPPORTED) {
    g_fallbacks.fetch_add(1, std::memory_order_relaxed);
    GPS_REQUIRE(!strict, GPS_ERR_UNSUPPORTED,
                "GPS_B200_STRICT: dense product M=%d N=%d K=%d (ta=%d tb=%d) would fall back to the CUDA-core kernel",
                p.M, p.N, p.K, p.ta, p.tb);
    rc = gemm_simt(q, stream);
  }
  if (rc == GPS_OK && p.Cp.hi) {
    ToPlanesItem it{p.C, p.ldc, p.M, p.N, p.Cp};
    rc = to_planes(&it, 1, stream);
  }
  return rc;
}

namespace {

struct Side {
  cudaStream_t s = nullptr;
  cudaStream_t s3 = nullptr;
  cudaStream_t s4 = nullptr;
  cudaEvent_t ev[32];
  int next = 0;
  bool ok = false;
  int init() {
    if (ok) return GPS_OK;
    GPS_CUDA(cudaStreamCreateWithFlags(&s, cudaStreamNonBlocking));
    GPS_CUDA(cudaStreamCreateWithFlags(&s3, cudaStreamNonBlocking));
    GPS_CUDA(cudaStreamCreateWithFlags(&s4, cudaStreamNonBlocking));
    for (int i = 0; i < 32; ++i) GPS_CUDA(cudaEventCreateWithFlags(&ev[i], cudaEventDisableTiming));
    ok = true;
    return GPS_OK;
  }
  int order(cudaStream_t from, cudaStream_t to) {
    cudaEvent_t e = ev[next++ & 31];
    GPS_CUDA(cudaEventRecord(e, from));
    GPS_CUDA(cudaStreamWaitEvent(to, e, 0));
    return GPS_OK;
  }
  int fork(cudaStream_t main) { return order(main, s); }
  int join(cudaStream_t main) { return order(s, main); }
};

static int opt_flags() {
  static const int v = [] {
    const char* e = getenv("GPS_B200_OPT");
    return e ? atoi(e) : 0;
  }();
  return v;
}

static Side* side_stream() {
  static const bool enabled = [] {
    const char* e = getenv("GPS_B200_STREAMS");
    return !(e && e[0] == '0');
  }();
  if (!enabled) return nullptr;
  static thread_local Side sides[64];
  int dev = 0;
  if (cudaGetDevice(&dev) != cudaSuccess || dev < 0 || dev >= 64) return nullptr;
  if (sides[dev].init() != GPS_OK) return nullptr;
  return &sides[dev];
}

struct PackSeg {
  const float* w; const float* b; float* gw; float* gb; int rows;
};
struct PackDesc {
  PackSeg seg[5];
  int nseg; int d; int total_rows;
};

__global__ void k_pack(PackDesc pd, float* __restrict__ Wcat, float* __restrict__ bcat) {
  const int r = blockIdx.x;
  int row0 = 0, s = 0;
  while (s < pd.nseg - 1 && r >= row0 + pd.seg[s].rows) row0 += pd.seg[s++].rows;
  const float* src = pd.seg[s].w + (int64_t)(r - row0) * pd.d;
  float* dst = Wcat + (int64_t)r * pd.d;
  for (int c = threadIdx.x * 4; c < pd.d; c += blockDim.x * 4) st4(dst + c, ld4(src + c));
  if (threadIdx.x == 0) bcat[r] = pd.seg[s].b ? pd.seg[s].b[r - row0] : 0.f;
}
__global__ void k_unpack(PackDesc pd, const float* __restrict__ gWcat, const float* __restrict__ gbcat, int accumulate) {
  const int r = blockIdx.x;
  int row0 = 0, s = 0;
  while (s < pd.nseg - 1 && r >= row0 + pd.seg[s].rows) row0 += pd.seg[s++].rows;
  if (pd.seg[s].gw) {
    float* dst = pd.seg[s].gw + (int64_t)(r - row0) * pd.d;
    const float* src = gWcat + (int64_t)r * pd.d;
    for (int c = threadIdx.x * 4; c < pd.d; c += blockDim.x * 4)
      st4(dst + c, accumulate ? f4add(ld4(dst + c), ld4(src + c)) : ld4(src + c));
  }
  if (threadIdx.x == 0 && pd.seg[s].gb) pd.seg[s].gb[r - row0] = (accumulate ? pd.seg[s].gb[r - row0] : 0.f) + gbcat[r];
}

enum { BN_X = 0, BN_E = 1, BN_L = 2, BN_A = 3, BN_2 = 4, BN_COUNT = 5 };

struct Plan {
  int64_t N, E, d, H, hd, Wy, qkv_off;
  bool gated, gine, gcn, attn, perf;
  int64_t inner, mp, m;
  float *pQ, *pK, *pV, *pfq, *pfk, *pPn, *pgmax;
  int *pargq, *pargk, *pnmax;
  float *pden, *g_pden;
  bool perf_pairwise;
  float *g_pfq, *g_pfk, *g_pQ, *g_pK, *g_pV, *g_pgmax, *g_xp;
  float *Wcat, *bcat, *Y1, *ehat, *xt, *xloc, *O, *lse, *hA, *s, *hid, *hid_pre, *t, *bnbuf;
  float *agg, *h1, *h1_pre;
  float* dinv;
  bool eslap;
  float *pe_r, *pe_rho, *g_den, *pe_gz, *pe_gr, *pe_part;
  bool use_planes;
  Planes x_p, e_p, O_p, s_p, hid_p, agg_p, h1_p, Wcat_p, C_p, out_p, ff1_p, ff2_p, g0_p, g1_p, pq_p, pk_p, pv_p;
  Planes gt_p, ghid_p, ghA_p, ge_p, gY1_p, gtmp_p, gtmp2_p, gtmp3_p, gl1_p, gh1_p;
  Planes qkv_p;
  bool attn_tc;
  int64_t saved_bytes;
  int64_t wplanes_bytes;
  double* fstats;
  int64_t fwd_bytes;
  double* bsums;
  float *g_t, *g_hid, *g_s, *g_xloc, *g_hA, *g_O, *gY1, *g_e, *g_num, *delta, *g_tmp, *g_tmp2, *g_tmp3, *g_h1, *g_agg, *gWcat,
      *gbcat, *g_xl;
  int64_t bwd_bytes;
  int64_t fwd_launches, bwd_launches;
};

static bool attn_tc_enabled(int64_t N, int64_t B) {
  static const int mode = [] {
    const char* e = getenv("GPS_B200_ATTN");
    return e && strcmp(e, "simt") == 0 ? 0 : (e && strcmp(e, "tc") == 0 ? 2 : 1);
  }();
  if (mode != 1) return mode == 2;
  return B > 0 && N >= 64 * B;
}

static int make_plan(const GpsLayerArgs* a, Plan* P, bool bind) {
  memset(P, 0, sizeof(*P));
  GPS_REQUIRE(a, GPS_ERR_ARG, "null args");
  P->N = a->graph.N;
  P->E = a->graph.E;
  P->d = a->d;
  P->H = a->heads;
  GPS_REQUIRE(a->d > 0 && a->d % 4 == 0, GPS_ERR_UNSUPPORTED, "dim_h must be a positive multiple of 4 (got %lld)",
              (long long)a->d);
  P->gated = a->local_type == GPS_LOCAL_GATEDGCN;
  P->gine = a->local_type == GPS_LOCAL_GINE;
  P->gcn = a->local_type == GPS_LOCAL_GCN;
  GPS_REQUIRE(a->local_type == GPS_LOCAL_NONE || P->gated || P->gine || P->gcn, GPS_ERR_ARG, "unknown local_type %d",
              a->local_type);
  P->eslap = a->pe != nullptr;
  GPS_REQUIRE(!P->eslap || P->gated, GPS_ERR_ARG, "pe (EquivStableLapPE) is read by the GatedGCN local model only");
  GPS_REQUIRE(!P->eslap || a->pe_dim >= 1, GPS_ERR_ARG, "pe_dim must be >= 1 (got %lld)", (long long)a->pe_dim);
  GPS_REQUIRE(a->global_type == GPS_GLOBAL_NONE || a->global_type == GPS_GLOBAL_TRANSFORMER ||
                  a->global_type == GPS_GLOBAL_PERFORMER,
              GPS_ERR_ARG, "unknown global_type %d", a->global_type);
  P->attn = a->global_type == GPS_GLOBAL_TRANSFORMER;
  P->perf = a->global_type == GPS_GLOBAL_PERFORMER;
  if (P->perf) {
    GPS_TRY(perf_supported(a->perf_dim_head, a->perf_features));
    GPS_REQUIRE(a->heads > 0, GPS_ERR_ARG, "num_heads must be positive");
    P->inner = a->heads * a->perf_dim_head;
    P->mp = perf_mp();
    P->m = a->perf_features;
  }
  GPS_REQUIRE(a->local_type != GPS_LOCAL_NONE || P->attn || P->perf, GPS_ERR_ARG,
// ... 295 lines not shown
  GPS_TRY(check_bn(a->norm2, "norm2"));
  return GPS_OK;
}

static thread_local bool g_grads_prezeroed = false;
static thread_local bool g_grads_accumulate = false;

static int splitk_for(int64_t rows, int64_t out = 304, int64_t in = 304) {
  const int64_t tiles = ceil_div(out, 128) * ceil_div(in, in >= 160 ? 160 : 64);
  int64_t s = ceil_div(300, tiles > 0 ? tiles : 1);
  const int64_t max_s = rows / 256;
  if (s > max_s) s = max_s;
  if (s < 1) s = 1;
  if (s > 64) s = 64;
  return (int)s;
}

static int linear_wgrad(const float* G, int64_t ldg, const float* X, int64_t ldx, int64_t rows, int64_t out,
                        int64_t in, float* dW, float* db, int precision, cudaStream_t st, Planes Gp = Planes(),
                        Planes Xp = Planes()) {
  if (!dW) return GPS_OK;
  if (!g_grads_prezeroed) {
    GPS_CUDA(cudaMemsetAsync(dW, 0, (size_t)(out * in) * sizeof(float), st));
    if (db) GPS_CUDA(cudaMemsetAsync(db, 0, (size_t)out * sizeof(float), st));
  }
  if (rows == 0) return GPS_OK;
  GemmParams p;
  p.M = (int)out; p.N = (int)in; p.K = (int)rows;
  p.A = G; p.lda = (int)ldg; p.ta = 1;
  p.B = X; p.ldb = (int)ldx; p.tb = 1;
  p.C = dW; p.ldc = (int)in;
  p.splitk = splitk_for(rows, out, in);
  if (p.splitk == 1) p.splitk = 2;
  p.colsum_a = db;
  p.precision = precision;
  p.Ap = Gp; p.Bp = Xp;
  if (precision == GPS_PREC_BF16 && Gp.hi && db) {
    p.colsum_a = nullptr;
    GPS_TRY(colsum(G, ldg, rows, out, db, st));
  }
  return gemm(p, st);
}

}

static int layer_forward(const GpsLayerArgs* a, cudaStream_t st) {
  Plan P;
  GPS_TRY(make_plan(a, &P, true));
  GPS_REQUIRE(a->saved && a->workspace, GPS_ERR_ARG, "saved/workspace buffers are required");
  GPS_REQUIRE(a->workspace_bytes >= P.fwd_bytes, GPS_ERR_ARG, "workspace too small (%lld < %lld)",
              (long long)a->workspace_bytes, (long long)P.fwd_bytes);
  GPS_TRY(check_params(a, P));
  GPS_REQUIRE(a->x_out, GPS_ERR_ARG, "x_out is null");
  const int64_t N = P.N, E = P.E, d = P.d;
  const int act = a->act;
  const bool train = a->training != 0;
  const float pd = train ? a->dropout : 0.f;
  const float pa = train ? a->attn_dropout : 0.f;
  auto drop = [&](int site) {
    DropCfg c;
    c.p = pd; c.seed = a->seed; c.offset = a->offset; c.site = site;
    c.offset_dev = (const unsigned long long*)a->offset_dev;
    return c;
  };
  auto stats = [&](int which) -> double* { return train ? P.fstats + (int64_t)which * 2 * d : nullptr; };
  auto out_planes = [&](const GpsPlanes& g) {
    Planes q;
    if (P.use_planes && g.hi && g.ld >= d && g.ld % 8 == 0) {
      q.hi = (__nv_bfloat16*)g.hi;
      q.lo = a->precision == GPS_PREC_FP32 ? (__nv_bfloat16*)g.lo : nullptr;
      q.ld = g.ld;
      if (a->precision == GPS_PREC_FP32 && !q.lo) q = Planes();
    }
    return q;
  };

  if (train) GPS_CUDA(cudaMemsetAsync(P.fstats, 0, (size_t)BN_COUNT * 2 * d * sizeof(double), st));
  Side* sd = side_stream();
  cudaStream_t s2 = sd ? sd->s : st;
  const bool two_branches = (P.gated || P.gine || P.gcn) && (P.attn || P.perf);

  if (P.Wy) {
    PackDesc pdsc0 = pack_desc(a, P);
    k_pack<<<(unsigned)pdsc0.total_rows, 128, 0, st>>>(pdsc0, P.Wcat, P.bcat);
    GPS_LAUNCH_CHECK();
  }
  if (P.use_planes) {
    ToPlanesItem it[16];
    int ni = 0;
    auto add = [&](const float* src, int64_t ld, int64_t rows, int64_t cols, Planes dst) {
      if (src && dst.hi && rows > 0) it[ni++] = ToPlanesItem{src, ld, (int)rows, (int)cols, dst};
    };
    const int64_t kout = P.perf ? P.inner : d;
    if (P.x_p.hi != (__nv_bfloat16*)a->x_planes_in.hi) add(a->x, d, N, d, P.x_p);
    if ((P.gated || P.gine) && P.e_p.hi != (__nv_bfloat16*)a->e_planes_in.hi) add(a->edge_attr, d, E, d, P.e_p);
    const bool wvalid = a->wplanes && a->wplanes_valid;
    if (wvalid) goto weights_done;
    if (P.gated) {
      add(a->gcn_A.weight, d, d, d, P.Wcat_p.rows(0));
      add(a->gcn_B.weight, d, d, d, P.Wcat_p.rows(d));
      add(a->gcn_D.weight, d, d, d, P.Wcat_p.rows(2 * d));
      add(a->gcn_E.weight, d, d, d, P.Wcat_p.rows(3 * d));
      add(a->gcn_C.weight, d, d, d, P.C_p);
    }
    if (P.gcn) add(a->gcn_conv.weight, d, d, d, P.Wcat_p.rows(0));
    if (P.attn) add(a->attn_in.weight, d, 3 * d, d, P.Wcat_p.rows(P.qkv_off));
    if (P.gine) {
      add(a->gine_lin0.weight, d, d, d, P.g0_p);
      add(a->gine_lin1.weight, d, d, d, P.g1_p);
    }
    if (P.attn || P.perf) add(a->attn_out.weight, kout, d, kout, P.out_p);
    add(a->ff1.weight, d, 2 * d, d, P.ff1_p);
    add(a->ff2.weight, 2 * d, d, 2 * d, P.ff2_p);
    if (P.perf) {
      add(a->perf_q.weight, d, P.inner, d, P.pq_p);
      add(a->perf_k.weight, d, P.inner, d, P.pk_p);
      add(a->perf_v.weight, d, P.inner, d, P.pv_p);
    }
  weights_done:
    GPS_TRY(to_planes(it, ni, st));
  }
  if (P.gated) {
    GPS_REQUIRE(a->edge_out, GPS_ERR_ARG, "edge_out is null");
    if (sd) GPS_TRY(sd->fork(st));
    GemmParams g;
    g.M = (int)E; g.N = (int)d; g.K = (int)d;
    g.A = a->edge_attr; g.lda = (int)d; g.B = a->gcn_C.weight; g.ldb = (int)d; g.C = P.ehat; g.ldc = (int)d;
    g.bias = a->gcn_C.bias; g.precision = a->precision;
    g.Ap = P.e_p; g.Bp = P.C_p;
    GPS_TRY(gemm(g, s2));
    if (P.eslap)
      GPS_TRY(eslap_fwd(a->graph, a->pe, a->pe_dim, d, act, a->pe_mlp0.weight, a->pe_mlp0.bias, a->pe_mlp1.weight,
                        a->pe_mlp1.bias, P.pe_r, P.pe_rho, s2));
  }

  cudaStream_t sg = st;
  if (two_branches && sd) {
    GPS_TRY(sd->order(st, sd->s3));
    sg = sd->s3;
  }
  if (P.Wy) {
    const int64_t wl = P.qkv_off, wg = P.Wy - P.qkv_off;
    if (wg > 0) {
      GemmParams g;
      g.M = (int)N; g.N = (int)wg; g.K = (int)d;
      g.A = a->x; g.lda = (int)d; g.B = P.Wcat + wl * d; g.ldb = (int)d; g.C = P.Y1 + wl; g.ldc = (int)P.Wy;
      g.bias = P.bcat + wl; g.precision = a->precision;
      g.Ap = P.x_p; g.Bp = P.Wcat_p.rows(wl);
      if (P.attn_tc) {
        g.Cp = P.qkv_p; g.cp_hd = (int)P.hd; g.cp_hd_pad = (int)attention_tc_hd_pad(P.hd); g.cp_col0 = 0;
      }
      GPS_TRY(gemm(g, sg));
    }
    if (wl > 0) {
      GemmParams g;
      g.M = (int)N; g.N = (int)wl; g.K = (int)d;
      g.A = a->x; g.lda = (int)d; g.B = P.Wcat; g.ldb = (int)d; g.C = P.Y1; g.ldc = (int)P.Wy;
      g.bias = P.bcat; g.precision = a->precision;
      g.Ap = P.x_p; g.Bp = P.Wcat_p;
      GPS_TRY(gemm(g, st));
    }
  }

  if (P.gated && sd) GPS_TRY(sd->join(st));

  if (P.gated) {
    GPS_TRY(gatedgcn_fwd(a->graph, d, P.Y1, P.Y1 + d, P.Y1 + 2 * d, P.Y1 + 3 * d, P.Wy, P.ehat, P.xt,
// ... 344 lines not shown
    if (P.eslap) {
      if (sp != st) GPS_TRY(sd->order(st, sp));
      GPS_TRY(eslap_bwd(a->graph, a->pe, a->pe_dim, d, act, P.g_num, P.g_den, P.Y1 + d, P.Wy, P.ehat, P.pe_r, P.pe_rho,
                        a->pe_mlp0.weight, a->pe_mlp0.bias, a->pe_mlp1.weight, P.pe_gz, P.pe_gr, P.pe_part, a->grad_pe,
                        a->pe_mlp0.grad_weight, a->pe_mlp0.grad_bias, a->pe_mlp1.grad_weight, a->pe_mlp1.grad_bias,
                        g_grads_accumulate, sp));
    }
    GPS_TRY(gatedgcn_bwd_src(a->graph, d, P.g_e, P.ehat, P.g_num, P.gY1 + 3 * d, P.gY1 + d, P.Wy, st, P.gY1_p.cols(3 * d),
                             P.gY1_p.cols(d), P.pe_rho));
    GPS_TRY(wfork(st));
    GPS_TRY(linear_wgrad(P.g_e, d, a->edge_attr, d, E, d, d, a->gcn_C.grad_weight, a->gcn_C.grad_bias, prec, s2, P.ge_p, P.e_p));
    if (sp != st) GPS_TRY(sd->order(sp, s2));
    GPS_TRY(mid_done());
    if (a->grad_edge_attr && E > 0) {
      GemmParams g;
      g.M = (int)E; g.N = (int)d; g.K = (int)d;
      g.A = P.g_e; g.lda = (int)d; g.B = a->gcn_C.weight; g.ldb = (int)d; g.tb = 1; g.C = a->grad_edge_attr; g.ldc = (int)d;
      g.R1 = a->grad_edge_out; g.ldr1 = (int)d; g.precision = prec;
      g.Ap = P.ge_p; g.Bp = P.C_p;
      GPS_TRY(gemm(g, st));
    }
    g_x_local = P.g_xloc;
  } else if (P.gine) {
    const float* g_l1 = P.g_xloc;
    Planes g_l1_p = P.gl1_p;
    if (pd > 0.f) {
      GPS_TRY(dropmul(P.g_xloc, P.g_tmp3, N, d, P, a, GPS_SITE_LOCAL, st, 0.f, 0, P.gtmp3_p));
      g_l1 = P.g_tmp3;
      g_l1_p = P.gtmp3_p;
    }
    GemmParams g;
    g.M = (int)N; g.N = (int)d; g.K = (int)d;
    g.A = g_l1; g.lda = (int)d; g.B = a->gine_lin1.weight; g.ldb = (int)d; g.tb = 1; g.C = P.g_h1; g.ldc = (int)d;
    if (relu) { g.mask_src = P.h1; g.mask_is_post = 1; } else { g.mask_src = P.h1_pre; g.mask_act = act; }
    g.ldmask = (int)d; g.precision = prec;
    g.Ap = g_l1_p; g.Bp = P.g1_p; g.Cp = P.gh1_p;
    GPS_TRY(gemm(g, st));
    GPS_TRY(wfork(st));
    GPS_TRY(linear_wgrad(g_l1, d, P.h1, d, N, d, d, a->gine_lin1.grad_weight, a->gine_lin1.grad_bias, prec, s2, g_l1_p, P.h1_p));
    GPS_TRY(linear_wgrad(P.g_h1, d, P.agg, d, N, d, d, a->gine_lin0.grad_weight, a->gine_lin0.grad_bias, prec, s2, P.gh1_p, P.agg_p));
    GPS_TRY(mid_done());
    GemmParams g2;
    g2.M = (int)N; g2.N = (int)d; g2.K = (int)d;
    g2.A = P.g_h1; g2.lda = (int)d; g2.B = a->gine_lin0.weight; g2.ldb = (int)d; g2.tb = 1; g2.C = P.g_agg; g2.ldc = (int)d;
    g2.precision = prec;
    g2.Ap = P.gh1_p; g2.Bp = P.g0_p;
    GPS_TRY(gemm(g2, st));
    GPS_REQUIRE(a->grad_edge_attr || E == 0, GPS_ERR_ARG, "grad_edge_attr is required for GINE");
    GPS_TRY(gine_bwd_dst(a->graph, d, a->x, a->edge_attr, P.g_agg, a->grad_edge_attr, st));
    GPS_TRY(gine_bwd_src(a->graph, d, a->grad_edge_attr, P.g_agg, a->gine_eps, P.g_xloc, P.g_xl, st));
    g_x_local = P.g_xl;
  } else if (P.gcn) {
    const float* g_h = P.g_xloc;
    if (pd > 0.f) {
      GPS_TRY(dropmul(P.g_xloc, P.g_tmp3, N, d, P, a, GPS_SITE_LOCAL, st));
      g_h = P.g_tmp3;
    }
    if (a->gcn_conv.grad_bias) {
      if (!g_grads_prezeroed) GPS_CUDA(cudaMemsetAsync(a->gcn_conv.grad_bias, 0, (size_t)d * sizeof(float), st));
      GPS_TRY(colsum(g_h, d, N, d, a->gcn_conv.grad_bias, st));
    }
    GPS_TRY(gcn_bwd(a->graph, d, g_h, P.dinv, P.gY1, P.Wy, st, P.gY1_p));
    GPS_TRY(wfork(st));
    GPS_TRY(mid_done());
    g_x_local = P.g_xloc;
  }

  if (two_branches && sd) GPS_TRY(sd->order(sa, st));

  if (P.Wy) {
    GPS_TRY(wfork(st));
    GemmParams w;
    w.M = (int)P.Wy; w.N = (int)d; w.K = (int)N;
    w.A = P.gY1; w.lda = (int)P.Wy; w.ta = 1; w.B = a->x; w.ldb = (int)d; w.tb = 1; w.C = P.gWcat; w.ldc = (int)d;
    w.splitk = splitk_for(N, P.Wy, d) < 2 ? 2 : splitk_for(N, P.Wy, d);
    w.colsum_a = P.gbcat; w.precision = prec;
    w.Ap = P.gY1_p; w.Bp = P.x_p;
    if (prec == GPS_PREC_BF16 && w.Ap.hi && N > 0) {
      w.colsum_a = nullptr;
      GPS_TRY(colsum(P.gY1, P.Wy, N, P.Wy, P.gbcat, s2));
    }
    if (N > 0) GPS_TRY(gemm(w, s2));
    PackDesc pdsc = pack_desc(a, P);
    k_unpack<<<(unsigned)P.Wy, 128, 0, s2>>>(pdsc, P.gWcat, P.gbcat, g_grads_accumulate ? 1 : 0);
    GPS_LAUNCH_CHECK();
    GemmParams g;
    g.M = (int)N; g.N = (int)d; g.K = (int)P.Wy;
    g.A = P.gY1; g.lda = (int)P.Wy; g.B = P.Wcat; g.ldb = (int)d; g.tb = 1; g.C = a->grad_x; g.ldc = (int)d;
    g.R1 = g_x_local; g.ldr1 = (int)d;
    g.R2 = P.attn ? P.g_hA : (P.perf ? P.g_xp : nullptr); g.ldr2 = (int)d;
    g.precision = prec;
    if (gx_splitk) g.splitk = 4;
    g.Ap = P.gY1_p; g.Bp = P.Wcat_p;
    GPS_TRY(gemm(g, st));
  } else if (g_x_local) {
    GPS_TRY(add3(g_x_local, d, P.perf ? P.g_xp : nullptr, d, nullptr, 0, a->grad_x, d, N, d, st));
  } else {
    GPS_TRY(add3(P.g_xp, d, nullptr, 0, nullptr, 0, a->grad_x, d, N, d, st));
  }
  if (sd) GPS_TRY(sd->join(st));
  GPS_TRY(record_ev(a->ev_grads_done, st));
  return GPS_OK;
}

namespace {
__global__ void k_dropmul(const float* __restrict__ src, float* __restrict__ dst, int64_t n4, int64_t c4n, float p,
                          uint64_t seed, uint64_t offset, int site, const unsigned long long* offset_dev, float p2,
                          int site2, Planes dstp) {
  if (offset_dev) offset += *offset_dev;
  for (int64_t i = blockIdx.x * (int64_t)blockDim.x + threadIdx.x; i < n4; i += (int64_t)gridDim.x * blockDim.x) {
    float4 v = ld4(src + i * 4);
    if (p > 0.f) v = f4mul(v, dropout_scale4(p, seed, offset, site, (uint64_t)i));
    if (p2 > 0.f) v = f4mul(v, dropout_scale4(p2, seed, offset, site2, (uint64_t)i));
    st4(dst + i * 4, v);
    if (dstp.hi) planes_store4(dstp, i / c4n, (i % c4n) * 4, v);
  }
}
__global__ void k_dropmask(float* __restrict__ dst, int64_t n4, float p, uint64_t seed, uint64_t offset, int site) {
  for (int64_t i = blockIdx.x * (int64_t)blockDim.x + threadIdx.x; i < n4; i += (int64_t)gridDim.x * blockDim.x) {
    float4 s = dropout_scale4(p, seed, offset, site, (uint64_t)i);
    st4(dst + i * 4, make_float4(s.x > 0.f ? 1.f : 0.f, s.y > 0.f ? 1.f : 0.f, s.z > 0.f ? 1.f : 0.f,
                                 s.w > 0.f ? 1.f : 0.f));
  }
}
}

static int dropmul(const float* src, float* dst, int64_t rows, int64_t d, const Plan&, const GpsLayerArgs* a, int site,
                   cudaStream_t st, float p2, int site2, Planes dstp) {
  int64_t n4 = rows * d / 4;
  if (n4 == 0) return GPS_OK;
  k_dropmul<<<(unsigned)std::min<int64_t>(ceil_div(n4, 256), kNumSMs * 8), 256, 0, st>>>(src, dst, n4, d / 4, a->dropout,
                                                                                        a->seed, a->offset, site,
                                                                                        (const unsigned long long*)a->offset_dev,
                                                                                        p2, site2, dstp);
  GPS_LAUNCH_CHECK();
  return GPS_OK;
}

}

using namespace gps;

extern "C" const char* gps_last_error(void) { return g_err; }
extern "C" int gps_abi_version(void) { return GPS_ABI_VERSION; }
extern "C" const char* gps_build_arch(void) { return "sm_90a"; }
extern "C" unsigned long long gps_launch_count(void) { return g_launches.load(); }
extern "C" unsigned long long gps_fallback_count(void) { return g_fallbacks.load(); }

extern "C" int gps_to_planes(const float* src, int64_t ld, int64_t rows, int64_t cols, void* hi, void* lo, int64_t ldp,
                             void* stream) {
  GPS_REQUIRE(src && hi, GPS_ERR_ARG, "gps_to_planes: null argument");
  ToPlanesItem it{src, ld, (int)rows, (int)cols, Planes{(__nv_bfloat16*)hi, (__nv_bfloat16*)lo, ldp}};
  return to_planes(&it, 1, (cudaStream_t)stream);
}

extern "C" int gps_gemm_planes(const void* A_hi, const void* A_lo, int64_t lda, int32_t ta, const void* B_hi,
                               const void* B_lo, int64_t ldb, int32_t tb, float* C, int64_t ldc, void* C_hi, void* C_lo,
                               int64_t ldcp, int64_t M, int64_t N, int64_t K, int32_t splitk, int32_t precision,
                               float* colsum_a, void* stream) {
  GemmParams g;
  g.M = (int)M; g.N = (int)N; g.K = (int)K;
  g.ta = ta; g.tb = tb; g.C = C; g.ldc = (int)ldc;
  g.Ap = Planes{(__nv_bfloat16*)A_hi, (__nv_bfloat16*)A_lo, lda};
  g.Bp = Planes{(__nv_bfloat16*)B_hi, (__nv_bfloat16*)B_lo, ldb};
  g.Cp = Planes{(__nv_bfloat16*)C_hi, (__nv_bfloat16*)C_lo, ldcp};
  g.splitk = splitk < 1 ? 1 : splitk; g.precision = precision; g.colsum_a = colsum_a;
  int rc = gemm_tma(g, (cudaStream_t)stream);
  if (rc == GPS_ERR_UNSUPPORTED) set_error("gps_gemm_planes: the TMA kernel does not take this shape/alignment");
  return rc;
}
extern "C" void gps_debug_set(int v) { gemm_tc_set_debug(v); }
extern "C" void gps_debug_tma(int force_bn, void* trace) {
  gemm_tma_set_force_bn(force_bn);
  gemm_tma_set_trace((unsigned long long*)trace);
}
extern "C" void gps_debug_attn(void* buf) { attention_tc_set_debug((float*)buf); }

extern "C" int gps_layer_plan(const GpsLayerArgs* args, GpsLayerPlan* plan) {
  GPS_REQUIRE(args && plan, GPS_ERR_ARG, "gps_layer_plan: null argument");
  Plan P;
  GPS_TRY(make_plan(args, &P, false));
  plan->saved_bytes = P.saved_bytes;
  plan->fwd_workspace_bytes = P.fwd_bytes;
  plan->bwd_workspace_bytes = P.bwd_bytes;
  plan->fwd_launches = 0;
  plan->bwd_launches = 0;
  plan->wplanes_bytes = P.wplanes_bytes;
  return GPS_OK;
}

extern "C" int gps_layer_forward(const GpsLayerArgs* args, void* stream) {
  GPS_REQUIRE(args, GPS_ERR_ARG, "gps_layer_forward: null args");
  return layer_forward(args, (cudaStream_t)stream);
}

extern "C" int gps_layer_backward(const GpsLayerArgs* args, void* stream) {
  GPS_REQUIRE(args, GPS_ERR_ARG, "gps_layer_backward: null args");
  return layer_backward(args, (cudaStream_t)stream);
}

extern "C" int gps_linear_forward(const float* A, int64_t lda, const float* W, int64_t ldw, const float* bias,
                                  float* C, int64_t ldc, int64_t M, int64_t N, int64_t K, int32_t act,
                                  int32_t precision, void* stream) {
  GemmParams g;
  g.M = (int)M; g.N = (int)N; g.K = (int)K;
  g.A = A; g.lda = (int)lda; g.B = W; g.ldb = (int)ldw; g.C = C; g.ldc = (int)ldc; g.bias = bias; g.act = act;
  g.precision = precision;
  return gemm(g, (cudaStream_t)stream);
}

extern "C" int gps_gemm(const float* A, int64_t lda, int32_t ta, const float* B, int64_t ldb, int32_t tb, float* C,
                        int64_t ldc, int64_t M, int64_t N, int64_t K, int32_t splitk, int32_t precision, int32_t impl,
                        void* stream) {
  GemmParams g;
  g.M = (int)M; g.N = (int)N; g.K = (int)K;
  g.A = A; g.lda = (int)lda; g.ta = ta; g.B = B; g.ldb = (int)ldb; g.tb = tb; g.C = C; g.ldc = (int)ldc;
  g.splitk = splitk < 1 ? 1 : splitk; g.precision = precision;
  if (impl == 1) return gemm_simt(g, (cudaStream_t)stream);
  if (impl == 2) {
    int rc = gemm_tc(g, (cudaStream_t)stream);
    if (rc == GPS_ERR_UNSUPPORTED) set_error("gps_gemm: the tensor-core kernel does not take this shape/alignment");
    return rc;
  }
  return gemm(g, (cudaStream_t)stream);
}

extern "C" int gps_gatedgcn_aggregate_forward(const GpsGraph* g, int64_t d, const float* Ax, const float* Bx,
                                              const float* Dx, const float* Ex, int64_t ldy, float* Ce, float* xt,
                                              double* stats_x, double* stats_e, void* stream) {
  GPS_REQUIRE(g && Ax && Bx && Dx && Ex && (Ce || g->E == 0) && xt, GPS_ERR_ARG, "gatedgcn_aggregate: null argument");
  return gatedgcn_fwd(*g, d, Ax, Bx, Dx, Ex, ldy, Ce, xt, stats_x, stats_e, (cudaStream_t)stream);
}

extern "C" int gps_gine_aggregate_forward(const GpsGraph* g, int64_t d, const float* x, const float* e, float eps,
                                          float* out, void* stream) {
  GPS_REQUIRE(g && x && out, GPS_ERR_ARG, "gine_aggregate: null argument");
  return gine_fwd(*g, d, x, e, eps, out, (cudaStream_t)stream);
}

extern "C" int gps_attention_forward(const GpsGraph* g, int64_t heads, int64_t hd, const float* Q, const float* K,
                                     const float* V, int64_t ld, float* O, int64_t ldo, float* lse, float p_drop,
                                     uint64_t seed, uint64_t offset, void* stream) {
  GPS_REQUIRE(g && Q && K && V && O && lse, GPS_ERR_ARG, "attention_forward: null argument");
  return attention_fwd(*g, heads, hd, Q, K, V, ld, O, ldo, lse, p_drop, seed, offset, (cudaStream_t)stream);
}

extern "C" int gps_attention_forward_tc(const GpsGraph* g, int64_t heads, int64_t hd, const void* qkv_hi, const void* qkv_lo,
                                        int64_t ld, float* O, int64_t ldo, float* lse, float p_drop, uint64_t seed,
                                        uint64_t offset, int32_t precision, void* stream) {
  GPS_REQUIRE(g && qkv_hi && O && lse, GPS_ERR_ARG, "attention_forward_tc: null argument");
  Planes q{(__nv_bfloat16*)qkv_hi, (__nv_bfloat16*)qkv_lo, ld};
  return attention_tc_fwd(*g, heads, hd, q, O, ldo, Planes(), lse, p_drop, seed, offset, nullptr, precision,
                          (cudaStream_t)stream);
}

extern "C" int gps_attention_backward(const GpsGraph* g, int64_t heads, int64_t hd, const float* Q, const float* K,
                                      const float* V, int64_t ld, const float* O, const float* dO, int64_t ldo,
                                      const float* lse, float* delta, float* dQ, float* dK, float* dV, int64_t ldg,
                                      float p_drop, uint64_t seed, uint64_t offset, void* stream) {
  GPS_REQUIRE(g && Q && K && V && O && dO && lse && delta && dQ && dK && dV, GPS_ERR_ARG,
              "attention_backward: null argument");
  return attention_bwd(*g, heads, hd, Q, K, V, ld, O, dO, ldo, lse, delta, dQ, dK, dV, ldg, p_drop, seed, offset,
                       (cudaStream_t)stream);
}

extern "C" int gps_dropout_mask(float* mask, int64_t rows, int64_t cols, float p, uint64_t seed, uint64_t offset,
                                int32_t site, void* stream) {
  GPS_REQUIRE(mask && cols % 4 == 0, GPS_ERR_ARG, "dropout_mask: cols must be a multiple of 4");
  int64_t n4 = rows * cols / 4;
  if (n4 == 0) return GPS_OK;
  k_dropmask<<<(unsigned)std::min<int64_t>(ceil_div(n4, 256), kNumSMs * 8), 256, 0, (cudaStream_t)stream>>>(
      mask, n4, p, seed, offset, site);
  GPS_LAUNCH_CHECK();
  return GPS_OK;
}
```

### graphgps_b200/csrc/scatter.cu

```cuda
#include "kernels.cuh"

namespace gps {

namespace {

struct NodeGeom {
  dim3 block, grid;
  size_t smem;
};
static int node_geom(int64_t N, int64_t d, int nstat, NodeGeom* g) {
  GPS_REQUIRE(d > 0 && d % 4 == 0 && d / 4 <= 1024, GPS_ERR_UNSUPPORTED,
              "sparse stage needs d %% 4 == 0 and d <= 4096 (got %lld)", (long long)d);
  int C4 = (int)(d / 4);
  int RY = C4 >= 256 ? 1 : 256 / C4;
  int64_t cap = kNumSMs * 16;
  if (nstat > 0) {
    RY = C4 >= 1024 ? 1 : 1024 / C4;
    if (RY > 16) RY = 16;
    const int smem_cap = (int)(48 * 1024 / ((size_t)nstat * C4 * sizeof(float4)));
    if (RY > smem_cap) RY = smem_cap < 1 ? 1 : smem_cap;
    cap = kNumSMs;
  }
  int64_t blocks = ceil_div(N > 0 ? N : 1, (int64_t)RY * 2);
  if (blocks > cap) blocks = cap;
  g->block = dim3(C4, RY, 1);
  g->grid = dim3((unsigned)blocks, 1, 1);
  g->smem = RY > 1 ? (size_t)nstat * RY * C4 * sizeof(float4) : 0;
  return GPS_OK;
}

__device__ __forceinline__ float4 sigmoid4(float4 v) {
  return make_float4(sigmoidf_(v.x), sigmoidf_(v.y), sigmoidf_(v.z), sigmoidf_(v.w));
}

template <int NS>
__device__ __forceinline__ void block_stats(float4* acc, double* const* ptrs, float4* sm) {
  const int c4 = threadIdx.x, ry = threadIdx.y, RY = blockDim.y, C4 = blockDim.x;
  if (RY > 1) {
#pragma unroll
    for (int s = 0; s < NS; ++s) sm[(s * RY + ry) * C4 + c4] = acc[s];
    __syncthreads();
    if (ry == 0) {
#pragma unroll
      for (int s = 0; s < NS; ++s)
        for (int y = 1; y < RY; ++y) acc[s] = f4add(acc[s], sm[(s * RY + y) * C4 + c4]);
    }
  }
  if (ry == 0) {
#pragma unroll
    for (int s = 0; s < NS; ++s) {
      double* p = ptrs[s];
      if (!p) continue;
      atomic_add_f64(p + c4 * 4 + 0, (double)acc[s].x);
      atomic_add_f64(p + c4 * 4 + 1, (double)acc[s].y);
      atomic_add_f64(p + c4 * 4 + 2, (double)acc[s].z);
      atomic_add_f64(p + c4 * 4 + 3, (double)acc[s].w);
    }
  }
}

template <bool STATS, bool PE>
__global__ void __launch_bounds__(1024) k_gatedgcn_fwd(GpsGraph g, int d, const float* __restrict__ Ax, const float* __restrict__ Bx,
                               const float* __restrict__ Dx, const float* __restrict__ Ex, int64_t ldy,
                               float* __restrict__ Ce, float* __restrict__ xt, double* stats_x,
                               double* stats_e, const float* __restrict__ rho) {
  extern __shared__ float4 sm[];
  const int c = threadIdx.x * 4, ry = threadIdx.y, RY = blockDim.y;
  float4 acc[4] = {f4zero(), f4zero(), f4zero(), f4zero()};
  for (int64_t i = (int64_t)blockIdx.x * RY + ry; i < g.N; i += (int64_t)gridDim.x * RY) {
    const float4 dx = ld4(Dx + i * ldy + c);
    float4 num = f4zero(), den = f4zero();
    const int kb = g.dst_ptr[i], ke = g.dst_ptr[i + 1];
    for (int k = kb; k < ke; k += 2) {
      const bool two = k + 1 < ke;
      const int j0 = g.dst_src[k], j1 = two ? g.dst_src[k + 1] : j0;
      const int64_t e0 = g.dst_eid[k], e1 = two ? g.dst_eid[k + 1] : e0;
      const float4 ex0 = ld4(Ex + (int64_t)j0 * ldy + c), bx0 = ld4(Bx + (int64_t)j0 * ldy + c);
      float4 c0 = ld4(Ce + e0 * d + c);
      const float4 ex1 = ld4(Ex + (int64_t)j1 * ldy + c), bx1 = ld4(Bx + (int64_t)j1 * ldy + c);
      float4 c1 = ld4(Ce + e1 * d + c);
      c0 = f4add(c0, f4add(dx, ex0));
      st4(Ce + e0 * d + c, c0);
      const float4 s0 = PE ? f4scale(sigmoid4(c0), rho[e0]) : sigmoid4(c0);
      num = f4fma(s0, bx0, num);
      den = f4add(den, s0);
      if (STATS) {
        acc[2] = f4add(acc[2], c0);
        acc[3] = f4fma(c0, c0, acc[3]);
      }
      if (two) {
        c1 = f4add(c1, f4add(dx, ex1));
        st4(Ce + e1 * d + c, c1);
        const float4 s1 = PE ? f4scale(sigmoid4(c1), rho[e1]) : sigmoid4(c1);
        num = f4fma(s1, bx1, num);
        den = f4add(den, s1);
        if (STATS) {
          acc[2] = f4add(acc[2], c1);
          acc[3] = f4fma(c1, c1, acc[3]);
        }
      }
    }
    const float4 ax = ld4(Ax + i * ldy + c);
    float4 v = make_float4(ax.x + num.x / (den.x + 1e-6f), ax.y + num.y / (den.y + 1e-6f),
                           ax.z + num.z / (den.z + 1e-6f), ax.w + num.w / (den.w + 1e-6f));
    st4(xt + i * d + c, v);
    if (STATS) {
      acc[0] = f4add(acc[0], v);
      acc[1] = f4fma(v, v, acc[1]);
    }
  }
  if (STATS) {
    double* ptrs[4] = {stats_x, stats_x ? stats_x + d : nullptr, stats_e, stats_e ? stats_e + d : nullptr};
    block_stats<4>(acc, ptrs, sm);
  }
}

template <bool PE>
__global__ void k_gatedgcn_bwd_dst(GpsGraph g, int d, const float* __restrict__ g_xt, int64_t ldg,
                                   const float* __restrict__ ehat, const float* __restrict__ Bx, int64_t ldy,
                                   float* __restrict__ g_e, float* __restrict__ g_num,
                                   float* __restrict__ g_Dx, Planes g_e_p, Planes g_Dx_p,
                                   const float* __restrict__ rho, float* __restrict__ g_den) {
  const int c = threadIdx.x * 4, ry = threadIdx.y, RY = blockDim.y;
  for (int64_t i = (int64_t)blockIdx.x * RY + ry; i < g.N; i += (int64_t)gridDim.x * RY) {
    const int kb = g.dst_ptr[i], ke = g.dst_ptr[i + 1];
    float4 num = f4zero(), den = f4zero();
    for (int k = kb; k < ke; ++k) {
      const int j = g.dst_src[k];
      const int64_t eid = g.dst_eid[k];
      const float4 s = PE ? f4scale(sigmoid4(ld4(ehat + eid * d + c)), rho[eid]) : sigmoid4(ld4(ehat + eid * d + c));
      num = f4fma(s, ld4(Bx + (int64_t)j * ldy + c), num);
      den = f4add(den, s);
    }
    const float4 inv = make_float4(1.f / (den.x + 1e-6f), 1.f / (den.y + 1e-6f), 1.f / (den.z + 1e-6f),
                                   1.f / (den.w + 1e-6f));
    const float4 agg = f4mul(num, inv);
    const float4 gx = ld4(g_xt + i * ldg + c);
    const float4 gn = f4mul(gx, inv);
    const float4 gd = make_float4(-gn.x * agg.x, -gn.y * agg.y, -gn.z * agg.z, -gn.w * agg.w);
    st4(g_num + i * d + c, gn);
    if (PE) st4(g_den + i * d + c, gd);
    float4 gdx = f4zero();
    for (int k = kb; k < ke; ++k) {
      const int j = g.dst_src[k];
      const int64_t eid = g.dst_eid[k];
      const float4 s = sigmoid4(ld4(ehat + eid * d + c));
      const float4 bx = ld4(Bx + (int64_t)j * ldy + c);
      const float4 gs = PE ? f4scale(f4fma(gn, bx, gd), rho[eid]) : f4fma(gn, bx, gd);
      float4 ge = ld4(g_e + eid * d + c);
      ge.x += gs.x * s.x * (1.f - s.x);
      ge.y += gs.y * s.y * (1.f - s.y);
      ge.z += gs.z * s.z * (1.f - s.z);
      ge.w += gs.w * s.w * (1.f - s.w);
      st4(g_e + eid * d + c, ge);
      if (g_e_p.hi) planes_store4(g_e_p, eid, c, ge);
      gdx = f4add(gdx, ge);
    }
    st4(g_Dx + i * ldg + c, gdx);
    if (g_Dx_p.hi) planes_store4(g_Dx_p, i, c, gdx);
  }
}

template <bool PE>
__global__ void k_gatedgcn_bwd_src(GpsGraph g, int d, const float* __restrict__ g_e,
                                   const float* __restrict__ ehat, const float* __restrict__ g_num,
                                   float* __restrict__ g_Ex, float* __restrict__ g_Bx, int64_t ldg, Planes g_Ex_p,
                                   Planes g_Bx_p, const float* __restrict__ rho) {
  const int c = threadIdx.x * 4, ry = threadIdx.y, RY = blockDim.y;
  for (int64_t j = (int64_t)blockIdx.x * RY + ry; j < g.N; j += (int64_t)gridDim.x * RY) {
    float4 gex = f4zero(), gbx = f4zero();
    const int kb = g.src_ptr[j], ke = g.src_ptr[j + 1];
    for (int k = kb; k < ke; ++k) {
      const int i = g.src_dst[k];
      const int64_t eid = g.src_eid[k];
      gex = f4add(gex, ld4(g_e + eid * d + c));
      const float4 s = PE ? f4scale(sigmoid4(ld4(ehat + eid * d + c)), rho[eid]) : sigmoid4(ld4(ehat + eid * d + c));
      gbx = f4fma(ld4(g_num + (int64_t)i * d + c), s, gbx);
    }
    st4(g_Ex + j * ldg + c, gex);
    st4(g_Bx + j * ldg + c, gbx);
    if (g_Ex_p.hi) planes_store4(g_Ex_p, j, c, gex);
    if (g_Bx_p.hi) planes_store4(g_Bx_p, j, c, gbx);
  }
}

__global__ void k_gine_fwd(GpsGraph g, int d, const float* __restrict__ x, const float* __restrict__ e,
                           float eps, float* __restrict__ out, Planes outp) {
  const int c = threadIdx.x * 4, ry = threadIdx.y, RY = blockDim.y;
  for (int64_t i = (int64_t)blockIdx.x * RY + ry; i < g.N; i += (int64_t)gridDim.x * RY) {
    float4 acc = f4scale(ld4(x + i * d + c), 1.f + eps);
    const int kb = g.dst_ptr[i], ke = g.dst_ptr[i + 1];
    for (int k = kb; k < ke; ++k) {
      const int j = g.dst_src[k];
      const int64_t eid = g.dst_eid[k];
      const float4 m = f4add(ld4(x + (int64_t)j * d + c), ld4(e + eid * d + c));
      acc.x += fmaxf(m.x, 0.f);
      acc.y += fmaxf(m.y, 0.f);
      acc.z += fmaxf(m.z, 0.f);
      acc.w += fmaxf(m.w, 0.f);
    }
    st4(out + i * d + c, acc);
    if (outp.hi) planes_store4(outp, i, c, acc);
  }
}

__global__ void k_gine_bwd_dst(GpsGraph g, int d, const float* __restrict__ x, const float* __restrict__ e,
                               const float* __restrict__ g_o, float* __restrict__ g_e) {
  const int c = threadIdx.x * 4, ry = threadIdx.y, RY = blockDim.y;
  for (int64_t i = (int64_t)blockIdx.x * RY + ry; i < g.N; i += (int64_t)gridDim.x * RY) {
    const float4 go = ld4(g_o + i * d + c);
    const int kb = g.dst_ptr[i], ke = g.dst_ptr[i + 1];
    for (int k = kb; k < ke; ++k) {
      const int j = g.dst_src[k];
      const int64_t eid = g.dst_eid[k];
      const float4 m = f4add(ld4(x + (int64_t)j * d + c), ld4(e + eid * d + c));
      st4(g_e + eid * d + c, make_float4(m.x > 0.f ? go.x : 0.f, m.y > 0.f ? go.y : 0.f,
                                         m.z > 0.f ? go.z : 0.f, m.w > 0.f ? go.w : 0.f));
    }
  }
}

__global__ void k_gine_bwd_src(GpsGraph g, int d, const float* __restrict__ g_e, const float* __restrict__ g_o,
                               float eps, const float* __restrict__ add, float* __restrict__ g_x) {
  const int c = threadIdx.x * 4, ry = threadIdx.y, RY = blockDim.y;
  for (int64_t j = (int64_t)blockIdx.x * RY + ry; j < g.N; j += (int64_t)gridDim.x * RY) {
    float4 acc = f4scale(ld4(g_o + j * d + c), 1.f + eps);
    if (add) acc = f4add(acc, ld4(add + j * d + c));
    const int kb = g.src_ptr[j], ke = g.src_ptr[j + 1];
    for (int k = kb; k < ke; ++k) acc = f4add(acc, ld4(g_e + (int64_t)g.src_eid[k] * d + c));
    st4(g_x + j * d + c, acc);
  }
}

__global__ void k_gcn_dinv(GpsGraph g, float* __restrict__ dinv) {
  const int64_t i = (int64_t)blockIdx.x * blockDim.x + threadIdx.x;
  if (i >= g.N) return;
  int deg = 1;
  for (int k = g.dst_ptr[i]; k < g.dst_ptr[i + 1]; ++k) deg += g.dst_src[k] != (int)i;
  dinv[i] = rsqrtf((float)deg);
}

template <bool STATS>
__global__ void __launch_bounds__(1024) k_gcn_fwd(GpsGraph g, int d, const float* __restrict__ Y, int64_t ldy,
                                                  const float* __restrict__ dinv, const float* __restrict__ bias,
                                                  const float* __restrict__ x, float* __restrict__ xloc, DropCfg drop,
                                                  double* stats) {
  extern __shared__ float4 sm[];
  const int c = threadIdx.x * 4, ry = threadIdx.y, RY = blockDim.y;
  const uint64_t offs = drop.offset + ((drop.p > 0.f && drop.offset_dev) ? *drop.offset_dev : 0ull);
  const float4 b4 = ld4(bias + c);
  float4 acc[2] = {f4zero(), f4zero()};
  for (int64_t i = (int64_t)blockIdx.x * RY + ry; i < g.N; i += (int64_t)gridDim.x * RY) {
    const float di = dinv[i];
    float4 a = f4scale(ld4(Y + i * ldy + c), di);
    for (int k = g.dst_ptr[i]; k < g.dst_ptr[i + 1]; ++k) {
      const int j = g.dst_src[k];
      if (j == (int)i) continue;
      a = f4fma(make_float4(dinv[j], dinv[j], dinv[j], dinv[j]), ld4(Y + (int64_t)j * ldy + c), a);
    }
    float4 h = f4add(f4scale(a, di), b4);
    if (drop.p > 0.f) h = f4mul(h, dropout_scale4(drop.p, drop.seed, offs, drop.site, ((uint64_t)i * (uint64_t)d + c) >> 2));
    const float4 v = f4add(ld4(x + i * d + c), h);
    st4(xloc + i * d + c, v);
    if (STATS) {
      acc[0] = f4add(acc[0], v);
      acc[1] = f4fma(v, v, acc[1]);
    }
  }
  if (STATS) {
    double* ptrs[2] = {stats, stats + d};
    block_stats<2>(acc, ptrs, sm);
  }
}

__global__ void k_gcn_bwd(GpsGraph g, int d, const float* __restrict__ g_h, const float* __restrict__ dinv,
                          float* __restrict__ gY, int64_t ldg, Planes gYp) {
  const int c = threadIdx.x * 4, ry = threadIdx.y, RY = blockDim.y;
  for (int64_t j = (int64_t)blockIdx.x * RY + ry; j < g.N; j += (int64_t)gridDim.x * RY) {
    const float dj = dinv[j];
    float4 a = f4scale(ld4(g_h + j * d + c), dj);
    for (int k = g.src_ptr[j]; k < g.src_ptr[j + 1]; ++k) {
      const int i = g.src_dst[k];
      if (i == (int)j) continue;
      a = f4fma(make_float4(dinv[i], dinv[i], dinv[i], dinv[i]), ld4(g_h + (int64_t)i * d + c), a);
    }
    st4(gY + j * ldg + c, f4scale(a, dj));
    if (gYp.hi) planes_store4(gYp, j, c, f4scale(a, dj));
  }
}

}

int gcn_dinv(const GpsGraph& g, float* dinv, cudaStream_t stream) {
  if (g.N == 0) return GPS_OK;
  k_gcn_dinv<<<(unsigned)ceil_div(g.N, (int64_t)256), 256, 0, stream>>>(g, dinv);
  GPS_LAUNCH_CHECK();
  return GPS_OK;
}

int gcn_fwd(const GpsGraph& g, int64_t d, const float* Y, int64_t ldy, const float* dinv, const float* bias,
            const float* x, float* xloc, DropCfg drop, double* stats, cudaStream_t stream) {
  if (g.N == 0) return GPS_OK;
  NodeGeom ng;
  GPS_TRY(node_geom(g.N, d, stats ? 2 : 0, &ng));
  if (stats)
    k_gcn_fwd<true><<<ng.grid, ng.block, ng.smem, stream>>>(g, (int)d, Y, ldy, dinv, bias, x, xloc, drop, stats);
  else
    k_gcn_fwd<false><<<ng.grid, ng.block, 0, stream>>>(g, (int)d, Y, ldy, dinv, bias, x, xloc, drop, nullptr);
  GPS_LAUNCH_CHECK();
  return GPS_OK;
}

int gcn_bwd(const GpsGraph& g, int64_t d, const float* g_h, const float* dinv, float* gY, int64_t ldg,
            cudaStream_t stream, Planes gYp) {
  if (g.N == 0) return GPS_OK;
  NodeGeom ng;
  GPS_TRY(node_geom(g.N, d, 0, &ng));
  k_gcn_bwd<<<ng.grid, ng.block, 0, stream>>>(g, (int)d, g_h, dinv, gY, ldg, gYp);
  GPS_LAUNCH_CHECK();
  return GPS_OK;
}

int gatedgcn_fwd(const GpsGraph& g, int64_t d, const float* Ax, const float* Bx, const float* Dx, const float* Ex,
                 int64_t ldy, float* Ce, float* xt, double* stats_x, double* stats_e, cudaStream_t stream,
                 const float* rho) {
  if (g.N == 0) return GPS_OK;
  NodeGeom ng;
  const bool stats = stats_x || stats_e;
  GPS_TRY(node_geom(g.N, d, stats ? 4 : 0, &ng));
  if (stats && rho)
    k_gatedgcn_fwd<true, true><<<ng.grid, ng.block, ng.smem, stream>>>(g, (int)d, Ax, Bx, Dx, Ex, ldy, Ce, xt, stats_x,
                                                                         stats_e, rho);
  else if (rho)
    k_gatedgcn_fwd<false, true><<<ng.grid, ng.block, 0, stream>>>(g, (int)d, Ax, Bx, Dx, Ex, ldy, Ce, xt, nullptr, nullptr,
                                                                  rho);
  else if (stats)
    k_gatedgcn_fwd<true, false><<<ng.grid, ng.block, ng.smem, stream>>>(g, (int)d, Ax, Bx, Dx, Ex, ldy, Ce, xt, stats_x,
                                                                          stats_e, nullptr);
  else
    k_gatedgcn_fwd<false, false><<<ng.grid, ng.block, 0, stream>>>(g, (int)d, Ax, Bx, Dx, Ex, ldy, Ce, xt, nullptr, nullptr,
                                                                   nullptr);
  GPS_LAUNCH_CHECK();
  return GPS_OK;
}

int gatedgcn_bwd_dst(const GpsGraph& g, int64_t d, const float* g_xt, int64_t ldg, const float* ehat, const float* Bx,
                     int64_t ldy, float* g_e, float* g_num, float* g_Dx, cudaStream_t stream, Planes g_e_p, Planes g_Dx_p,
                     const float* rho, float* g_den) {
  if (g.N == 0) return GPS_OK;
  NodeGeom ng;
  GPS_TRY(node_geom(g.N, d, 0, &ng));
  if (rho)
    k_gatedgcn_bwd_dst<true><<<ng.grid, ng.block, 0, stream>>>(g, (int)d, g_xt, ldg, ehat, Bx, ldy, g_e, g_num, g_Dx, g_e_p,
                                                               g_Dx_p, rho, g_den);
  else
    k_gatedgcn_bwd_dst<false><<<ng.grid, ng.block, 0, stream>>>(g, (int)d, g_xt, ldg, ehat, Bx, ldy, g_e, g_num, g_Dx, g_e_p,
                                                                g_Dx_p, nullptr, nullptr);
  GPS_LAUNCH_CHECK();
  return GPS_OK;
}

int gatedgcn_bwd_src(const GpsGraph& g, int64_t d, const float* g_e, const float* ehat, const float* g_num,
                     float* g_Ex, float* g_Bx, int64_t ldg, cudaStream_t stream, Planes g_Ex_p, Planes g_Bx_p,
                     const float* rho) {
  if (g.N == 0) return GPS_OK;
  NodeGeom ng;
  GPS_TRY(node_geom(g.N, d, 0, &ng));
  if (rho)
    k_gatedgcn_bwd_src<true><<<ng.grid, ng.block, 0, stream>>>(g, (int)d, g_e, ehat, g_num, g_Ex, g_Bx, ldg, g_Ex_p, g_Bx_p,
                                                               rho);
  else
    k_gatedgcn_bwd_src<false><<<ng.grid, ng.block, 0, stream>>>(g, (int)d, g_e, ehat, g_num, g_Ex, g_Bx, ldg, g_Ex_p,
                                                                g_Bx_p, nullptr);
  GPS_LAUNCH_CHECK();
  return GPS_OK;
}

int gine_fwd(const GpsGraph& g, int64_t d, const float* x, const float* e, float eps, float* out,
             cudaStream_t stream, Planes outp) {
  if (g.N == 0) return GPS_OK;
  NodeGeom ng;
  GPS_TRY(node_geom(g.N, d, 0, &ng));
  k_gine_fwd<<<ng.grid, ng.block, 0, stream>>>(g, (int)d, x, e, eps, out, outp);
  GPS_LAUNCH_CHECK();
  return GPS_OK;
}

int gine_bwd_dst(const GpsGraph& g, int64_t d, const float* x, const float* e, const float* g_o, float* g_e,
                 cudaStream_t stream) {
  if (g.N == 0) return GPS_OK;
  NodeGeom ng;
  GPS_TRY(node_geom(g.N, d, 0, &ng));
  k_gine_bwd_dst<<<ng.grid, ng.block, 0, stream>>>(g, (int)d, x, e, g_o, g_e);
  GPS_LAUNCH_CHECK();
  return GPS_OK;
}

int gine_bwd_src(const GpsGraph& g, int64_t d, const float* g_e, const float* g_o, float eps, const float* add,
                 float* g_x, cudaStream_t stream) {
  if (g.N == 0) return GPS_OK;
  NodeGeom ng;
  GPS_TRY(node_geom(g.N, d, 0, &ng));
  k_gine_bwd_src<<<ng.grid, ng.block, 0, stream>>>(g, (int)d, g_e, g_o, eps, add, g_x);
  GPS_LAUNCH_CHECK();
  return GPS_OK;
}

}
```

Measured before the change: 339,500.

## Enable programmatic dependent launch across all kernels with griddepcontrol.wait

Launches every kernel with the programmatic stream serialization attribute and adds a griddepcontrol.wait at kernel entry, so each kernel's launch and prologue (barrier init, TMA descriptor prefetch) can overlap the tail of the previous kernel. The intent is to hide launch latency across the many small kernels in a GPSLayer forward and backward pass. No kernel issues an explicit launch_dependents trigger, so the overlap window is limited to the implicit trigger at grid completion. The waits sit at kernel entry, which keeps data dependencies correct.

```diff
diff --git a/graphgps_b200/csrc/attention.cu b/graphgps_b200/csrc/attention.cu
--- a/graphgps_b200/csrc/attention.cu
+++ b/graphgps_b200/csrc/attention.cu
@@ -125,6 +125,7 @@
 
 template <int CH, int LPR>
 __global__ void __launch_bounds__(kWarpsPerBlock * 32) k_attn_fwd(AttnArgs a) {
+  pdl_wait();
   extern __shared__ float attn_sm[];
   constexpr int RPW = 32 / LPR;
   const int warp = threadIdx.x >> 5, lane = threadIdx.x & 31;
@@ -194,6 +195,7 @@
 }
 
 __global__ void k_attn_delta(AttnArgs a) {
+  pdl_wait();
   const int64_t t = ((int64_t)blockIdx.x * blockDim.x + threadIdx.x) >> 3;
   const int sub = threadIdx.x & 7;
   const bool ok = t < (int64_t)a.N * a.H;
@@ -360,6 +362,7 @@
 
 template <int CH, int LPR>
 __global__ void __launch_bounds__(kWarpsPerBlock * 32) k_attn_bwd(AttnArgs a) {
+  pdl_wait();
   extern __shared__ float attn_sm[];
   if (blockIdx.z == 0) attn_bwd_kv_body<CH, LPR>(a, attn_sm);
   else attn_bwd_q_body<CH, LPR>(a, attn_sm);
@@ -370,7 +373,7 @@
 constexpr int kStageBytes = 72 * 1024;
 
 template <int CH, int LPR>
-static void launch_one(int which, const AttnArgs& a0, cudaStream_t stream) {
+static int launch_one(int which, const AttnArgs& a0, cudaStream_t stream) {
   constexpr int RPW = 32 / LPR;
   AttnArgs a = a0;
   static const bool stage_on = [] {
@@ -388,8 +391,9 @@
   }
   dim3 grid((unsigned)ceil_div(a.N, (int64_t)RPW * kWarpsPerBlock), (unsigned)a.H, which == KFWD ? 1 : 2);
   dim3 block(kWarpsPerBlock * 32);
-  if (which == KFWD) k_attn_fwd<CH, LPR><<<grid, block, smem, stream>>>(a);
-  else k_attn_bwd<CH, LPR><<<grid, block, smem, stream>>>(a);
+  if (which == KFWD) GPS_CUDA(launch_pdl(k_attn_fwd<CH, LPR>, grid, block, smem, stream, a));
+  else GPS_CUDA(launch_pdl(k_attn_bwd<CH, LPR>, grid, block, smem, stream, a));
+  return GPS_OK;
 }
 
 static int dispatch(int which, const AttnArgs& a, cudaStream_t stream) {
@@ -404,7 +408,7 @@
   const int ch = (nch + lpr - 1) / lpr;
 #define GPS_ATTN_CASE(CHV, LPRV)                                  \
   if (ch == CHV && lpr == LPRV) {                                 \
-    launch_one<CHV, LPRV>(which, a, stream);                      \
+    GPS_TRY((launch_one<CHV, LPRV>(which, a, stream)));           \
     GPS_LAUNCH_CHECK();                                           \
     return GPS_OK;                                                \
   }
@@ -443,7 +447,7 @@
   a.scale = 1.f / sqrtf((float)hd); a.p_drop = p_drop; a.seed = seed; a.offset = offset;
   if (a.N == 0) return GPS_OK;
   const int64_t nt = (int64_t)a.N * a.H * 8;
-  k_attn_delta<<<(unsigned)ceil_div(nt, (int64_t)256), 256, 0, stream>>>(a);
+  GPS_CUDA(launch_pdl(k_attn_delta, (unsigned)ceil_div(nt, (int64_t)256), 256, 0, stream, a));
   GPS_LAUNCH_CHECK();
   return dispatch(KBWD, a, stream);
 }
diff --git a/graphgps_b200/csrc/attention_tc.cu b/graphgps_b200/csrc/attention_tc.cu
--- a/graphgps_b200/csrc/attention_tc.cu
+++ b/graphgps_b200/csrc/attention_tc.cu
@@ -65,6 +65,9 @@
   if (tid == 0) {
     mbar_init(b_q, 1); mbar_init(b_kf, 1); mbar_init(b_vf, 1); mbar_init(b_ke, kSoftWarps); mbar_init(b_ve, kSoftWarps);
     fence_barrier_init();
+  }
+  pdl_wait();
+  if (tid == 0) {
     const int last = min(q0 + kTile, a.N) - 1;
     const int g0 = find_graph_tc(a.gptr, a.B, q0), g1 = find_graph_tc(a.gptr, a.B, last);
     range[0] = a.gptr[g0];
@@ -284,7 +287,7 @@
     GPS_CUDA(cudaFuncSetAttribute(k_attn_tc_fwd<NKB, SPLIT>, cudaFuncAttributeMaxDynamicSharedMemorySize, 227 * 1024));
     attr_done = true;
   }
-  k_attn_tc_fwd<NKB, SPLIT><<<grid, kThreadsA, smem, stream>>>(tQK, tV, a);
+  GPS_CUDA(launch_pdl(k_attn_tc_fwd<NKB, SPLIT>, grid, kThreadsA, smem, stream, tQK, tV, a));
   GPS_LAUNCH_CHECK();
   return GPS_OK;
 }
diff --git a/graphgps_b200/csrc/common.cuh b/graphgps_b200/csrc/common.cuh
--- a/graphgps_b200/csrc/common.cuh
+++ b/graphgps_b200/csrc/common.cuh
@@ -5,6 +5,7 @@
 #include <stdint.h>
 #include <stdio.h>
 #include <string>
+#include <utility>
 
 #include "../../include/gps_b200.h"
 
@@ -39,6 +40,34 @@
     int _rc = (expr);            \
     if (_rc != GPS_OK) return _rc; \
   } while (0)
+
+template <typename... KArgs, typename... Args>
+cudaError_t launch_pdl_cluster(void (*kernel)(KArgs...), dim3 cluster, dim3 grid, dim3 block, size_t smem,
+                               cudaStream_t stream, Args&&... args) {
+  cudaLaunchAttribute attr[2];
+  int n = 0;
+  attr[n].id = cudaLaunchAttributeProgrammaticStreamSerialization;
+  attr[n++].val.programmaticStreamSerializationAllowed = 1;
+  if (cluster.x * cluster.y * cluster.z > 1) {
+    attr[n].id = cudaLaunchAttributeClusterDimension;
+    attr[n].val.clusterDim.x = cluster.x;
+    attr[n].val.clusterDim.y = cluster.y;
+    attr[n++].val.clusterDim.z = cluster.z;
+  }
+  cudaLaunchConfig_t cfg = {};
+  cfg.gridDim = grid;
+  cfg.blockDim = block;
+  cfg.dynamicSmemBytes = smem;
+  cfg.stream = stream;
+  cfg.attrs = attr;
+  cfg.numAttrs = n;
+  return cudaLaunchKernelEx(&cfg, kernel, std::forward<Args>(args)...);
+}
+template <typename... KArgs, typename... Args>
+cudaError_t launch_pdl(void (*kernel)(KArgs...), dim3 grid, dim3 block, size_t smem, cudaStream_t stream,
+                       Args&&... args) {
+  return launch_pdl_cluster(kernel, dim3(1, 1, 1), grid, block, smem, stream, std::forward<Args>(args)...);
+}
 
 constexpr int kNumSMs = 132;
 constexpr float kBnEps = 1e-5f;
@@ -77,6 +106,8 @@
 
 #ifdef __CUDACC__
 
+__device__ __forceinline__ void pdl_wait() { asm volatile("griddepcontrol.wait;" ::: "memory"); }
+
 __device__ __forceinline__ void planes_store4(const Planes& p, int64_t r, int64_t c, float4 v) {
   __nv_bfloat162 h0 = __floats2bfloat162_rn(v.x, v.y), h1 = __floats2bfloat162_rn(v.z, v.w);
   uint2 hw = make_uint2(*reinterpret_cast<uint32_t*>(&h0), *reinterpret_cast<uint32_t*>(&h1));
diff --git a/graphgps_b200/csrc/elementwise.cu b/graphgps_b200/csrc/elementwise.cu
--- a/graphgps_b200/csrc/elementwise.cu
+++ b/graphgps_b200/csrc/elementwise.cu
@@ -71,12 +71,14 @@
 
 template <class Op>
 __global__ void __launch_bounds__(1024) k_rowwise(Op op, int64_t rows) {
+  pdl_wait();
   extern __shared__ float4 sm[];
   rowwise_body(op, rows, (int)blockIdx.x, (int)gridDim.x, sm);
 }
 
 template <class OpA, class OpB>
 __global__ void __launch_bounds__(1024) k_rowwise2(OpA a, int64_t rowsA, int ga, OpB b, int64_t rowsB) {
+  pdl_wait();
   extern __shared__ float4 sm[];
   if ((int)blockIdx.x < ga) {
     a.vb = (int)blockIdx.x;
@@ -307,6 +309,7 @@
 constexpr int kColsumCtas = 8;
 __global__ void __launch_bounds__(1024) k_colsum(const float* __restrict__ a, int64_t lda, int64_t rows, int C4,
                                                  float* __restrict__ out) {
+  pdl_wait();
   extern __shared__ float4 sm[];
   const int ry = threadIdx.y, RY = blockDim.y, CB = blockDim.x;
   const int c4 = blockIdx.x * CB + threadIdx.x;
@@ -340,7 +343,7 @@
   if (rows == 0) return GPS_OK;
   RowGeom g;
   GPS_TRY(row_geom(rows, d, Op::NS, &g));
-  k_rowwise<Op><<<g.grid, g.block, g.smem, stream>>>(op, rows);
+  GPS_CUDA(launch_pdl(k_rowwise<Op>, g.grid, g.block, g.smem, stream, op, rows));
   GPS_LAUNCH_CHECK();
   return GPS_OK;
 }
@@ -371,7 +374,8 @@
   if (gb > kNumSMs * 2) gb = kNumSMs * 2;
   OpBnActRes<true> opx{zx, d, Rx, outx, d, bnx, act, dropx, statsx, Planes()};
   OpBnActRes<false> ope{ze, d, Re, oute, d, bne, act, drope, nullptr, outep};
-  k_rowwise2<<<dim3((unsigned)(g.grid.x + gb)), g.block, g.smem, stream>>>(opx, N, (int)g.grid.x, ope, E);
+  GPS_CUDA(launch_pdl(k_rowwise2<OpBnActRes<true>, OpBnActRes<false>>, dim3((unsigned)(g.grid.x + gb)), g.block, g.smem,
+                      stream, opx, N, (int)g.grid.x, ope, E));
   GPS_LAUNCH_CHECK();
   return GPS_OK;
 }
@@ -424,19 +428,8 @@
   const int C4 = (int)(d / 4);
   const int CB = C4 < 128 ? C4 : 128;
   const int RY = 1024 / CB < 16 ? 1024 / CB : 16;
-  cudaLaunchConfig_t cfg = {};
-  cfg.gridDim = dim3((unsigned)ceil_div(C4, CB), kColsumCtas);
-  cfg.blockDim = dim3(CB, RY);
-  cfg.dynamicSmemBytes = (size_t)RY * CB * sizeof(float4);
-  cfg.stream = stream;
-  cudaLaunchAttribute attr[1];
-  attr[0].id = cudaLaunchAttributeClusterDimension;
-  attr[0].val.clusterDim.x = 1;
-  attr[0].val.clusterDim.y = kColsumCtas;
-  attr[0].val.clusterDim.z = 1;
-  cfg.attrs = attr;
-  cfg.numAttrs = 1;
-  GPS_CUDA(cudaLaunchKernelEx(&cfg, k_colsum, a, lda, rows, C4, out));
+  GPS_CUDA(launch_pdl_cluster(k_colsum, dim3(1, kColsumCtas, 1), dim3((unsigned)ceil_div(C4, CB), kColsumCtas),
+                              dim3(CB, RY), (size_t)RY * CB * sizeof(float4), stream, a, lda, rows, C4, out));
   GPS_LAUNCH_CHECK();
   return GPS_OK;
 }
diff --git a/graphgps_b200/csrc/eslap.cu b/graphgps_b200/csrc/eslap.cu
--- a/graphgps_b200/csrc/eslap.cu
+++ b/graphgps_b200/csrc/eslap.cu
@@ -19,6 +19,7 @@
 __global__ void k_eslap_fwd(GpsGraph g, const float* __restrict__ pe, int64_t k, int d, const float* __restrict__ w1,
                             const float* __restrict__ b1, const float* __restrict__ w2, const float* __restrict__ b2,
                             float* __restrict__ r_out, float* __restrict__ rho_out) {
+  pdl_wait();
   const int lane = threadIdx.x & 31;
   const int64_t i = (int64_t)blockIdx.x * kWarpsPerBlock + (threadIdx.x >> 5);
   if (i >= g.N) return;
@@ -43,6 +44,7 @@
                                  const float* __restrict__ r_in, const float* __restrict__ rho_in,
                                  const float* __restrict__ w1, const float* __restrict__ b1,
                                  const float* __restrict__ w2, float* __restrict__ gz_out, float* __restrict__ gr_out) {
+  pdl_wait();
   const int lane = threadIdx.x & 31;
   const int64_t i = (int64_t)blockIdx.x * kWarpsPerBlock + (threadIdx.x >> 5);
   if (i >= g.N) return;
@@ -73,6 +75,7 @@
 
 __global__ void k_eslap_bwd_pe(GpsGraph g, const float* __restrict__ pe, int64_t k, const float* __restrict__ gr,
                                float* __restrict__ grad_pe) {
+  pdl_wait();
   const int lane = threadIdx.x & 31;
   const int64_t n = (int64_t)blockIdx.x * kWarpsPerBlock + (threadIdx.x >> 5);
   if (n >= g.N) return;
@@ -90,6 +93,7 @@
 __global__ void k_eslap_wgrad_part(int64_t E, int64_t chunk, int d, const float* __restrict__ r_in,
                                    const float* __restrict__ gz_in, const float* __restrict__ w1,
                                    const float* __restrict__ b1, const float* __restrict__ w2, float* __restrict__ part) {
+  pdl_wait();
   const int64_t e0 = (int64_t)blockIdx.x * chunk;
   const int64_t e1 = e0 + chunk < E ? e0 + chunk : E;
   float* out = part + (int64_t)blockIdx.x * (3 * d + 1);
@@ -117,6 +121,7 @@
 
 __global__ void k_eslap_wgrad_sum(int64_t nparts, int d, const float* __restrict__ part, float* gw2, float* gw1,
                                   float* gb1, float* gb2, int accumulate) {
+  pdl_wait();
   const int col = blockIdx.x * blockDim.x + threadIdx.x;
   if (col > 3 * d) return;
   float s = 0.f;
@@ -140,9 +145,11 @@
   if (g.N == 0 || g.E == 0) return GPS_OK;
   const unsigned blocks = (unsigned)ceil_div(g.N, (int64_t)kWarpsPerBlock);
   if (act == GPS_ACT_RELU)
-    k_eslap_fwd<GPS_ACT_RELU><<<blocks, 32 * kWarpsPerBlock, 0, stream>>>(g, pe, k, (int)d, w1, b1, w2, b2, r, rho);
+    GPS_CUDA(launch_pdl(k_eslap_fwd<GPS_ACT_RELU>, blocks, 32 * kWarpsPerBlock, 0, stream, g, pe, k, (int)d, w1, b1, w2,
+                        b2, r, rho));
   else
-    k_eslap_fwd<GPS_ACT_GELU><<<blocks, 32 * kWarpsPerBlock, 0, stream>>>(g, pe, k, (int)d, w1, b1, w2, b2, r, rho);
+    GPS_CUDA(launch_pdl(k_eslap_fwd<GPS_ACT_GELU>, blocks, 32 * kWarpsPerBlock, 0, stream, g, pe, k, (int)d, w1, b1, w2,
+                        b2, r, rho));
   GPS_LAUNCH_CHECK();
   return GPS_OK;
 }
@@ -155,25 +162,27 @@
   const int64_t chunk = eslap_wgrad_chunk(g.E), nparts = ceil_div(g.E, chunk);
   if (g.E > 0) {
     if (act == GPS_ACT_RELU)
-      k_eslap_bwd_edge<GPS_ACT_RELU><<<node_blocks, 32 * kWarpsPerBlock, 0, stream>>>(
-          g, (int)d, g_num, g_den, Bx, ldy, ehat, r, rho, w1, b1, w2, gz, gr);
+      GPS_CUDA(launch_pdl(k_eslap_bwd_edge<GPS_ACT_RELU>, node_blocks, 32 * kWarpsPerBlock, 0, stream, g, (int)d, g_num,
+                          g_den, Bx, ldy, ehat, r, rho, w1, b1, w2, gz, gr));
     else
-      k_eslap_bwd_edge<GPS_ACT_GELU><<<node_blocks, 32 * kWarpsPerBlock, 0, stream>>>(
-          g, (int)d, g_num, g_den, Bx, ldy, ehat, r, rho, w1, b1, w2, gz, gr);
+      GPS_CUDA(launch_pdl(k_eslap_bwd_edge<GPS_ACT_GELU>, node_blocks, 32 * kWarpsPerBlock, 0, stream, g, (int)d, g_num,
+                          g_den, Bx, ldy, ehat, r, rho, w1, b1, w2, gz, gr));
     GPS_LAUNCH_CHECK();
     if (act == GPS_ACT_RELU)
-      k_eslap_wgrad_part<GPS_ACT_RELU><<<(unsigned)nparts, 256, 0, stream>>>(g.E, chunk, (int)d, r, gz, w1, b1, w2, part);
+      GPS_CUDA(launch_pdl(k_eslap_wgrad_part<GPS_ACT_RELU>, (unsigned)nparts, 256, 0, stream, g.E, chunk, (int)d, r, gz,
+                          w1, b1, w2, part));
     else
-      k_eslap_wgrad_part<GPS_ACT_GELU><<<(unsigned)nparts, 256, 0, stream>>>(g.E, chunk, (int)d, r, gz, w1, b1, w2, part);
+      GPS_CUDA(launch_pdl(k_eslap_wgrad_part<GPS_ACT_GELU>, (unsigned)nparts, 256, 0, stream, g.E, chunk, (int)d, r, gz,
+                          w1, b1, w2, part));
     GPS_LAUNCH_CHECK();
   }
   if (gw1 || gb1 || gw2 || gb2) {
-    k_eslap_wgrad_sum<<<(unsigned)ceil_div(3 * d + 1, (int64_t)128), 128, 0, stream>>>(g.E > 0 ? nparts : 0, (int)d, part,
-                                                                                     gw2, gw1, gb1, gb2, accumulate ? 1 : 0);
+    GPS_CUDA(launch_pdl(k_eslap_wgrad_sum, (unsigned)ceil_div(3 * d + 1, (int64_t)128), 128, 0, stream,
+                        g.E > 0 ? nparts : 0, (int)d, part, gw2, gw1, gb1, gb2, accumulate ? 1 : 0));
     GPS_LAUNCH_CHECK();
   }
   if (grad_pe && g.N > 0) {
-    k_eslap_bwd_pe<<<node_blocks, 32 * kWarpsPerBlock, 0, stream>>>(g, pe, k, gr, grad_pe);
+    GPS_CUDA(launch_pdl(k_eslap_bwd_pe, node_blocks, 32 * kWarpsPerBlock, 0, stream, g, pe, k, gr, grad_pe));
     GPS_LAUNCH_CHECK();
   }
   return GPS_OK;
diff --git a/graphgps_b200/csrc/gemm_tma.cu b/graphgps_b200/csrc/gemm_tma.cu
--- a/graphgps_b200/csrc/gemm_tma.cu
+++ b/graphgps_b200/csrc/gemm_tma.cu
@@ -66,24 +66,27 @@
   const int cta_lin = (blockIdx.z * gridDim.y + blockIdx.y) * gridDim.x + blockIdx.x;
 
   if (tid == 0) {
+    for (int s = 0; s < S; ++s) {
+      mbar_init(smem_u32(&bars[s]), 1);
+      mbar_init(smem_u32(&bars[S + s]), kEpiWarps);
+    }
+    fence_barrier_init();
+  }
+  if (warp == kTmaWarp && lane == 0) {
+    tma_prefetch_desc(&tmA);
+    tma_prefetch_desc(&tmB);
+  }
+  __syncthreads();
+  pdl_wait();
+  if (tid == 0) {
     GPS_TRACE(0);
     if (a.trace && cta_lin < 256) {
       unsigned smid;
       asm volatile("mov.u32 %0, %smid;" : "=r"(smid));
       a.trace[cta_lin * 16 + 8] = smid;
     }
-    for (int s = 0; s < S; ++s) {
-      mbar_init(smem_u32(&bars[s]), 1);
-      mbar_init(smem_u32(&bars[S + s]), kEpiWarps);
-    }
-    fence_barrier_init();
-  }
-  if (warp == kTmaWarp && lane == 0) {
-    tma_prefetch_desc(&tmA);
-    tma_prefetch_desc(&tmB);
-  }
-  __syncthreads();
-  if (tid == 0) GPS_TRACE(1);
+    GPS_TRACE(1);
+  }
 
   if (warp == kTmaWarp) {
     if (lane == 0 && nkb > 0) {
@@ -498,23 +501,8 @@
                                   227 * 1024));
     attr_done = true;
   }
-  if (grid.z == 1) {
-    k_gemm_tma<A_MN, B_MN, BN_T, SPLIT><<<grid, kThreads, smem, stream>>>(tA, tB, a);
-  } else {
-    cudaLaunchConfig_t cfg = {};
-    cfg.gridDim = grid;
-    cfg.blockDim = dim3(kThreads);
-    cfg.dynamicSmemBytes = smem;
-    cfg.stream = stream;
-    cudaLaunchAttribute attr[1];
-    attr[0].id = cudaLaunchAttributeClusterDimension;
-    attr[0].val.clusterDim.x = 1;
-    attr[0].val.clusterDim.y = 1;
-    attr[0].val.clusterDim.z = grid.z;
-    cfg.attrs = attr;
-    cfg.numAttrs = 1;
-    GPS_CUDA(cudaLaunchKernelEx(&cfg, k_gemm_tma<A_MN, B_MN, BN_T, SPLIT>, tA, tB, a));
-  }
+  GPS_CUDA(launch_pdl_cluster(k_gemm_tma<A_MN, B_MN, BN_T, SPLIT>, dim3(1, 1, grid.z), grid, kThreads, smem, stream, tA,
+                              tB, a));
   GPS_LAUNCH_CHECK();
   return GPS_OK;
 }
@@ -633,6 +621,7 @@
   int n;
 };
 __global__ void k_to_planes(ToPlanesDesc d) {
+  pdl_wait();
   int item = 0;
   while (item + 1 < d.n && (int)blockIdx.x >= d.start[item + 1]) ++item;
   const ToPlanesItem& it = d.it[item];
@@ -678,7 +667,7 @@
   }
   d.start[d.n] = total;
   if (total == 0) return GPS_OK;
-  k_to_planes<<<(unsigned)total, 256, 0, stream>>>(d);
+  GPS_CUDA(launch_pdl(k_to_planes, (unsigned)total, 256, 0, stream, d));
   GPS_LAUNCH_CHECK();
   return GPS_OK;
 }
diff --git a/graphgps_b200/csrc/layer.cu b/graphgps_b200/csrc/layer.cu
--- a/graphgps_b200/csrc/layer.cu
+++ b/graphgps_b200/csrc/layer.cu
@@ -136,6 +136,7 @@
 };
 
 __global__ void k_pack(PackDesc pd, float* __restrict__ Wcat, float* __restrict__ bcat) {
+  pdl_wait();
   const int r = blockIdx.x;
   int row0 = 0, s = 0;
   while (s < pd.nseg - 1 && r >= row0 + pd.seg[s].rows) row0 += pd.seg[s++].rows;
@@ -145,6 +146,7 @@
   if (threadIdx.x == 0) bcat[r] = pd.seg[s].b ? pd.seg[s].b[r - row0] : 0.f;
 }
 __global__ void k_unpack(PackDesc pd, const float* __restrict__ gWcat, const float* __restrict__ gbcat, int accumulate) {
+  pdl_wait();
   const int r = blockIdx.x;
   int row0 = 0, s = 0;
   while (s < pd.nseg - 1 && r >= row0 + pd.seg[s].rows) row0 += pd.seg[s++].rows;
@@ -606,7 +608,7 @@
 
   if (P.Wy) {
     PackDesc pdsc0 = pack_desc(a, P);
-    k_pack<<<(unsigned)pdsc0.total_rows, 128, 0, st>>>(pdsc0, P.Wcat, P.bcat);
+    GPS_CUDA(launch_pdl(k_pack, (unsigned)pdsc0.total_rows, 128, 0, st, pdsc0, P.Wcat, P.bcat));
     GPS_LAUNCH_CHECK();
   }
   if (P.use_planes) {
@@ -1117,7 +1119,7 @@
     }
     if (N > 0) GPS_TRY(gemm(w, s2));
     PackDesc pdsc = pack_desc(a, P);
-    k_unpack<<<(unsigned)P.Wy, 128, 0, s2>>>(pdsc, P.gWcat, P.gbcat, g_grads_accumulate ? 1 : 0);
+    GPS_CUDA(launch_pdl(k_unpack, (unsigned)P.Wy, 128, 0, s2, pdsc, P.gWcat, P.gbcat, g_grads_accumulate ? 1 : 0));
     GPS_LAUNCH_CHECK();
     GemmParams g;
     g.M = (int)N; g.N = (int)d; g.K = (int)P.Wy;
@@ -1142,6 +1144,7 @@
 __global__ void k_dropmul(const float* __restrict__ src, float* __restrict__ dst, int64_t n4, int64_t c4n, float p,
                           uint64_t seed, uint64_t offset, int site, const unsigned long long* offset_dev, float p2,
                           int site2, Planes dstp) {
+  pdl_wait();
   if (offset_dev) offset += *offset_dev;
   for (int64_t i = blockIdx.x * (int64_t)blockDim.x + threadIdx.x; i < n4; i += (int64_t)gridDim.x * blockDim.x) {
     float4 v = ld4(src + i * 4);
@@ -1152,6 +1155,7 @@
   }
 }
 __global__ void k_dropmask(float* __restrict__ dst, int64_t n4, float p, uint64_t seed, uint64_t offset, int site) {
+  pdl_wait();
   for (int64_t i = blockIdx.x * (int64_t)blockDim.x + threadIdx.x; i < n4; i += (int64_t)gridDim.x * blockDim.x) {
     float4 s = dropout_scale4(p, seed, offset, site, (uint64_t)i);
     st4(dst + i * 4, make_float4(s.x > 0.f ? 1.f : 0.f, s.y > 0.f ? 1.f : 0.f, s.z > 0.f ? 1.f : 0.f,
@@ -1164,10 +1168,9 @@
                    cudaStream_t st, float p2, int site2, Planes dstp) {
   int64_t n4 = rows * d / 4;
   if (n4 == 0) return GPS_OK;
-  k_dropmul<<<(unsigned)std::min<int64_t>(ceil_div(n4, 256), kNumSMs * 8), 256, 0, st>>>(src, dst, n4, d / 4, a->dropout,
-                                                                                        a->seed, a->offset, site,
-                                                                                        (const unsigned long long*)a->offset_dev,
-                                                                                        p2, site2, dstp);
+  GPS_CUDA(launch_pdl(k_dropmul, (unsigned)std::min<int64_t>(ceil_div(n4, 256), kNumSMs * 8), 256, 0, st, src, dst, n4,
+                      d / 4, a->dropout, a->seed, a->offset, site, (const unsigned long long*)a->offset_dev, p2, site2,
+                      dstp));
   GPS_LAUNCH_CHECK();
   return GPS_OK;
 }
@@ -1304,8 +1307,8 @@
   GPS_REQUIRE(mask && cols % 4 == 0, GPS_ERR_ARG, "dropout_mask: cols must be a multiple of 4");
   int64_t n4 = rows * cols / 4;
   if (n4 == 0) return GPS_OK;
-  k_dropmask<<<(unsigned)std::min<int64_t>(ceil_div(n4, 256), kNumSMs * 8), 256, 0, (cudaStream_t)stream>>>(
-      mask, n4, p, seed, offset, site);
+  GPS_CUDA(launch_pdl(k_dropmask, (unsigned)std::min<int64_t>(ceil_div(n4, 256), kNumSMs * 8), 256, 0,
+                      (cudaStream_t)stream, mask, n4, p, seed, offset, site));
   GPS_LAUNCH_CHECK();
   return GPS_OK;
 }
diff --git a/graphgps_b200/csrc/scatter.cu b/graphgps_b200/csrc/scatter.cu
--- a/graphgps_b200/csrc/scatter.cu
+++ b/graphgps_b200/csrc/scatter.cu
@@ -64,6 +64,7 @@
                                const float* __restrict__ Dx, const float* __restrict__ Ex, int64_t ldy,
                                float* __restrict__ Ce, float* __restrict__ xt, double* stats_x,
                                double* stats_e, const float* __restrict__ rho) {
+  pdl_wait();
   extern __shared__ float4 sm[];
   const int c = threadIdx.x * 4, ry = threadIdx.y, RY = blockDim.y;
   float4 acc[4] = {f4zero(), f4zero(), f4zero(), f4zero()};
@@ -121,6 +122,7 @@
                                    float* __restrict__ g_e, float* __restrict__ g_num,
                                    float* __restrict__ g_Dx, Planes g_e_p, Planes g_Dx_p,
                                    const float* __restrict__ rho, float* __restrict__ g_den) {
+  pdl_wait();
   const int c = threadIdx.x * 4, ry = threadIdx.y, RY = blockDim.y;
   for (int64_t i = (int64_t)blockIdx.x * RY + ry; i < g.N; i += (int64_t)gridDim.x * RY) {
     const int kb = g.dst_ptr[i], ke = g.dst_ptr[i + 1];
@@ -166,6 +168,7 @@
                                    const float* __restrict__ ehat, const float* __restrict__ g_num,
                                    float* __restrict__ g_Ex, float* __restrict__ g_Bx, int64_t ldg, Planes g_Ex_p,
                                    Planes g_Bx_p, const float* __restrict__ rho) {
+  pdl_wait();
   const int c = threadIdx.x * 4, ry = threadIdx.y, RY = blockDim.y;
   for (int64_t j = (int64_t)blockIdx.x * RY + ry; j < g.N; j += (int64_t)gridDim.x * RY) {
     float4 gex = f4zero(), gbx = f4zero();
@@ -186,6 +189,7 @@
 
 __global__ void k_gine_fwd(GpsGraph g, int d, const float* __restrict__ x, const float* __restrict__ e,
                            float eps, float* __restrict__ out, Planes outp) {
+  pdl_wait();
   const int c = threadIdx.x * 4, ry = threadIdx.y, RY = blockDim.y;
   for (int64_t i = (int64_t)blockIdx.x * RY + ry; i < g.N; i += (int64_t)gridDim.x * RY) {
     float4 acc = f4scale(ld4(x + i * d + c), 1.f + eps);
@@ -206,6 +210,7 @@
 
 __global__ void k_gine_bwd_dst(GpsGraph g, int d, const float* __restrict__ x, const float* __restrict__ e,
                                const float* __restrict__ g_o, float* __restrict__ g_e) {
+  pdl_wait();
   const int c = threadIdx.x * 4, ry = threadIdx.y, RY = blockDim.y;
   for (int64_t i = (int64_t)blockIdx.x * RY + ry; i < g.N; i += (int64_t)gridDim.x * RY) {
     const float4 go = ld4(g_o + i * d + c);
@@ -222,6 +227,7 @@
 
 __global__ void k_gine_bwd_src(GpsGraph g, int d, const float* __restrict__ g_e, const float* __restrict__ g_o,
                                float eps, const float* __restrict__ add, float* __restrict__ g_x) {
+  pdl_wait();
   const int c = threadIdx.x * 4, ry = threadIdx.y, RY = blockDim.y;
   for (int64_t j = (int64_t)blockIdx.x * RY + ry; j < g.N; j += (int64_t)gridDim.x * RY) {
     float4 acc = f4scale(ld4(g_o + j * d + c), 1.f + eps);
@@ -233,6 +239,7 @@
 }
 
 __global__ void k_gcn_dinv(GpsGraph g, float* __restrict__ dinv) {
+  pdl_wait();
   const int64_t i = (int64_t)blockIdx.x * blockDim.x + threadIdx.x;
   if (i >= g.N) return;
   int deg = 1;
@@ -245,6 +252,7 @@
                                                   const float* __restrict__ dinv, const float* __restrict__ bias,
                                                   const float* __restrict__ x, float* __restrict__ xloc, DropCfg drop,
                                                   double* stats) {
+  pdl_wait();
   extern __shared__ float4 sm[];
   const int c = threadIdx.x * 4, ry = threadIdx.y, RY = blockDim.y;
   const uint64_t offs = drop.offset + ((drop.p > 0.f && drop.offset_dev) ? *drop.offset_dev : 0ull);
@@ -275,6 +283,7 @@
 
 __global__ void k_gcn_bwd(GpsGraph g, int d, const float* __restrict__ g_h, const float* __restrict__ dinv,
                           float* __restrict__ gY, int64_t ldg, Planes gYp) {
+  pdl_wait();
   const int c = threadIdx.x * 4, ry = threadIdx.y, RY = blockDim.y;
   for (int64_t j = (int64_t)blockIdx.x * RY + ry; j < g.N; j += (int64_t)gridDim.x * RY) {
     const float dj = dinv[j];
@@ -293,7 +302,7 @@
 
 int gcn_dinv(const GpsGraph& g, float* dinv, cudaStream_t stream) {
   if (g.N == 0) return GPS_OK;
-  k_gcn_dinv<<<(unsigned)ceil_div(g.N, (int64_t)256), 256, 0, stream>>>(g, dinv);
+  GPS_CUDA(launch_pdl(k_gcn_dinv, (unsigned)ceil_div(g.N, (int64_t)256), 256, 0, stream, g, dinv));
   GPS_LAUNCH_CHECK();
   return GPS_OK;
 }
@@ -304,9 +313,11 @@
   NodeGeom ng;
   GPS_TRY(node_geom(g.N, d, stats ? 2 : 0, &ng));
   if (stats)
-    k_gcn_fwd<true><<<ng.grid, ng.block, ng.smem, stream>>>(g, (int)d, Y, ldy, dinv, bias, x, xloc, drop, stats);
+    GPS_CUDA(launch_pdl(k_gcn_fwd<true>, ng.grid, ng.block, ng.smem, stream, g, (int)d, Y, ldy, dinv, bias, x, xloc,
+                        drop, stats));
   else
-    k_gcn_fwd<false><<<ng.grid, ng.block, 0, stream>>>(g, (int)d, Y, ldy, dinv, bias, x, xloc, drop, nullptr);
+    GPS_CUDA(launch_pdl(k_gcn_fwd<false>, ng.grid, ng.block, 0, stream, g, (int)d, Y, ldy, dinv, bias, x, xloc, drop,
+                        nullptr));
   GPS_LAUNCH_CHECK();
   return GPS_OK;
 }
@@ -316,7 +327,7 @@
   if (g.N == 0) return GPS_OK;
   NodeGeom ng;
   GPS_TRY(node_geom(g.N, d, 0, &ng));
-  k_gcn_bwd<<<ng.grid, ng.block, 0, stream>>>(g, (int)d, g_h, dinv, gY, ldg, gYp);
+  GPS_CUDA(launch_pdl(k_gcn_bwd, ng.grid, ng.block, 0, stream, g, (int)d, g_h, dinv, gY, ldg, gYp));
   GPS_LAUNCH_CHECK();
   return GPS_OK;
 }
@@ -329,17 +340,17 @@
   const bool stats = stats_x || stats_e;
   GPS_TRY(node_geom(g.N, d, stats ? 4 : 0, &ng));
   if (stats && rho)
-    k_gatedgcn_fwd<true, true><<<ng.grid, ng.block, ng.smem, stream>>>(g, (int)d, Ax, Bx, Dx, Ex, ldy, Ce, xt, stats_x,
-                                                                         stats_e, rho);
+    GPS_CUDA(launch_pdl(k_gatedgcn_fwd<true, true>, ng.grid, ng.block, ng.smem, stream, g, (int)d, Ax, Bx, Dx, Ex, ldy,
+                        Ce, xt, stats_x, stats_e, rho));
   else if (rho)
-    k_gatedgcn_fwd<false, true><<<ng.grid, ng.block, 0, stream>>>(g, (int)d, Ax, Bx, Dx, Ex, ldy, Ce, xt, nullptr, nullptr,
-                                                                  rho);
+    GPS_CUDA(launch_pdl(k_gatedgcn_fwd<false, true>, ng.grid, ng.block, 0, stream, g, (int)d, Ax, Bx, Dx, Ex, ldy, Ce,
+                        xt, nullptr, nullptr, rho));
   else if (stats)
-    k_gatedgcn_fwd<true, false><<<ng.grid, ng.block, ng.smem, stream>>>(g, (int)d, Ax, Bx, Dx, Ex, ldy, Ce, xt, stats_x,
-                                                                          stats_e, nullptr);
+    GPS_CUDA(launch_pdl(k_gatedgcn_fwd<true, false>, ng.grid, ng.block, ng.smem, stream, g, (int)d, Ax, Bx, Dx, Ex, ldy,
+                        Ce, xt, stats_x, stats_e, nullptr));
   else
-    k_gatedgcn_fwd<false, false><<<ng.grid, ng.block, 0, stream>>>(g, (int)d, Ax, Bx, Dx, Ex, ldy, Ce, xt, nullptr, nullptr,
-                                                                   nullptr);
+    GPS_CUDA(launch_pdl(k_gatedgcn_fwd<false, false>, ng.grid, ng.block, 0, stream, g, (int)d, Ax, Bx, Dx, Ex, ldy, Ce,
+                        xt, nullptr, nullptr, nullptr));
   GPS_LAUNCH_CHECK();
   return GPS_OK;
 }
@@ -351,11 +362,11 @@
   NodeGeom ng;
   GPS_TRY(node_geom(g.N, d, 0, &ng));
   if (rho)
-    k_gatedgcn_bwd_dst<true><<<ng.grid, ng.block, 0, stream>>>(g, (int)d, g_xt, ldg, ehat, Bx, ldy, g_e, g_num, g_Dx, g_e_p,
-                                                               g_Dx_p, rho, g_den);
+    GPS_CUDA(launch_pdl(k_gatedgcn_bwd_dst<true>, ng.grid, ng.block, 0, stream, g, (int)d, g_xt, ldg, ehat, Bx, ldy,
+                        g_e, g_num, g_Dx, g_e_p, g_Dx_p, rho, g_den));
   else
-    k_gatedgcn_bwd_dst<false><<<ng.grid, ng.block, 0, stream>>>(g, (int)d, g_xt, ldg, ehat, Bx, ldy, g_e, g_num, g_Dx, g_e_p,
-                                                                g_Dx_p, nullptr, nullptr);
+    GPS_CUDA(launch_pdl(k_gatedgcn_bwd_dst<false>, ng.grid, ng.block, 0, stream, g, (int)d, g_xt, ldg, ehat, Bx, ldy,
+                        g_e, g_num, g_Dx, g_e_p, g_Dx_p, nullptr, nullptr));
   GPS_LAUNCH_CHECK();
   return GPS_OK;
 }
@@ -367,11 +378,11 @@
   NodeGeom ng;
   GPS_TRY(node_geom(g.N, d, 0, &ng));
   if (rho)
-    k_gatedgcn_bwd_src<true><<<ng.grid, ng.block, 0, stream>>>(g, (int)d, g_e, ehat, g_num, g_Ex, g_Bx, ldg, g_Ex_p, g_Bx_p,
-                                                               rho);
+    GPS_CUDA(launch_pdl(k_gatedgcn_bwd_src<true>, ng.grid, ng.block, 0, stream, g, (int)d, g_e, ehat, g_num, g_Ex, g_Bx,
+                        ldg, g_Ex_p, g_Bx_p, rho));
   else
-    k_gatedgcn_bwd_src<false><<<ng.grid, ng.block, 0, stream>>>(g, (int)d, g_e, ehat, g_num, g_Ex, g_Bx, ldg, g_Ex_p,
-                                                                g_Bx_p, nullptr);
+    GPS_CUDA(launch_pdl(k_gatedgcn_bwd_src<false>, ng.grid, ng.block, 0, stream, g, (int)d, g_e, ehat, g_num, g_Ex,
+                        g_Bx, ldg, g_Ex_p, g_Bx_p, nullptr));
   GPS_LAUNCH_CHECK();
   return GPS_OK;
 }
@@ -381,7 +392,7 @@
   if (g.N == 0) return GPS_OK;
   NodeGeom ng;
   GPS_TRY(node_geom(g.N, d, 0, &ng));
-  k_gine_fwd<<<ng.grid, ng.block, 0, stream>>>(g, (int)d, x, e, eps, out, outp);
+  GPS_CUDA(launch_pdl(k_gine_fwd, ng.grid, ng.block, 0, stream, g, (int)d, x, e, eps, out, outp));
   GPS_LAUNCH_CHECK();
   return GPS_OK;
 }
@@ -391,7 +402,7 @@
   if (g.N == 0) return GPS_OK;
   NodeGeom ng;
   GPS_TRY(node_geom(g.N, d, 0, &ng));
-  k_gine_bwd_dst<<<ng.grid, ng.block, 0, stream>>>(g, (int)d, x, e, g_o, g_e);
+  GPS_CUDA(launch_pdl(k_gine_bwd_dst, ng.grid, ng.block, 0, stream, g, (int)d, x, e, g_o, g_e));
   GPS_LAUNCH_CHECK();
   return GPS_OK;
 }
@@ -401,9 +412,9 @@
   if (g.N == 0) return GPS_OK;
   NodeGeom ng;
   GPS_TRY(node_geom(g.N, d, 0, &ng));
-  k_gine_bwd_src<<<ng.grid, ng.block, 0, stream>>>(g, (int)d, g_e, g_o, eps, add, g_x);
-  GPS_LAUNCH_CHECK();
-  return GPS_OK;
-}
-
-}
+  GPS_CUDA(launch_pdl(k_gine_bwd_src, ng.grid, ng.block, 0, stream, g, (int)d, g_e, g_o, eps, add, g_x));
+  GPS_LAUNCH_CHECK();
+  return GPS_OK;
+}
+
+}
```

Result: faster. 343,600 (median of 6 runs) (+1.2%).
